# fy-vision/DiGA

Hardware: AMD Instinct MI355X
Metric: 768x768 19-class crops/sec (DiGA warm-up step) (higher is better)
Workload: dtype f32; 1 GPU; configs[1]: ResNet-101 DeepLabV2 DiGA warm-up (student + EMA teacher, KL distill), synthetic GTA5-shape 768x768, batch 8 per GPU; global_batch=8, parallelism=dp1

## Files before the change

### diga_amd/_lib.py

```python
import collections
import ctypes as C
import os

import torch

from diga_amd import config

_HERE = os.path.dirname(os.path.abspath(__file__))
LIB_PATH = os.environ.get("DIGA_LIB") or os.path.join(_HERE, "libdiga_hip.so")

if not os.path.exists(LIB_PATH):
    raise ImportError(
        f"{LIB_PATH} is missing: the DiGA hot path has no CPU fallback. "
        "Build the HIP extension first: python -m diga_amd.build")

lib = C.CDLL(LIB_PATH)

P = C.c_void_p
I64 = C.c_int64
F32 = C.c_float
INT = C.c_int
SZ = C.c_size_t

SIGNATURES = {
    "diga_version": (INT, []),
    "diga_last_error_string": (C.c_char_p, []),
    "diga_loss_workspace_bytes": (SZ, [I64]),
    "diga_ce2d_fwd_bwd": (INT, [P, P, P, P, P, SZ, I64, I64, I64, I64, F32, P]),
    "diga_ohem_ce_workspace_bytes": (SZ, [I64, I64, I64]),
    "diga_ohem_ce_fwd_bwd": (INT, [P, P, P, P, P, SZ, I64, I64, I64, I64, I64, F32, I64, F32, P]),
    "diga_distill_fwd_bwd": (INT, [P, P, P, P, P, SZ, I64, I64, I64, I64, F32, F32, P]),
    "diga_scale_inplace": (INT, [P, P, I64, P]),
    "diga_upsample_loss_workspace_bytes": (SZ, [I64, I64, I64, I64]),
    "diga_upsample_ce_distill_fwd_bwd": (INT, [P, P, P, P, P, P, SZ, I64, I64, I64, I64, I64, I64, F32, F32, F32, P]),
    "diga_upsample_ce_fwd_bwd": (INT, [P, P, P, P, P, SZ, I64, I64, I64, I64, I64, I64, F32, P]),
    "diga_upsample_bilinear_ac": (INT, [P, P, I64, I64, I64, I64, I64, P]),
    "diga_ema_update_flat": (INT, [P, P, I64, F32, F32, P]),
    "diga_ema_update_multi": (INT, [P, P, P, P, P, I64, I64, F32, F32, P]),
    "diga_sgd_momentum_multi": (INT, [P, P, P, P, P, P, P, P, I64, I64, F32, F32, INT, F32, P, P]),
    "diga_nonfinite_flag_f32": (INT, [P, I64, P, P]),
    "diga_label_hist256": (INT, [P, P, I64, I64, P]),
    "diga_classmix_paste": (INT, [P, P, P, P, P, P, P, I64, I64, I64, P]),
    "diga_centroid_softmax_weights": (INT, [P, P, P, P, I64, I64, I64, I64, P]),
    "diga_upsample_argmax_consensus": (INT, [P, P, P, P, I64, I64, I64, I64, I64, I64, P]),
    "diga_class_mean_workspace_bytes": (SZ, [I64, I64]),
    "diga_class_mean_vectors": (INT, [P, P, P, P, P, P, P, SZ, I64, I64, I64, I64, I64, I64, I64, P]),
    "diga_centroid_ema_apply": (INT, [P, P, P, P, I64, I64, I64, I64, F32, INT, INT, P]),
    "diga_confusion_matrix": (INT, [P, P, P, I64, I64, P]),
    "diga_two_scale_confusion": (INT, [P, I64, I64, P, I64, I64, P, P, P, I64, I64, I64, I64, P]),
    "diga_conv2d_nhwc_f32": (INT, [P, P, P, P] + [I64] * 17 + [P, INT, P]),
    "diga_conv2d_stats_floats": (SZ, [I64, I64, I64, I64]),
    "diga_conv2d_stats_chunk_rows": (INT, [I64] * 13 + [INT]),
    "diga_conv2d_epi_chunk_rows": (INT, [I64] * 13 + [INT]),
    "diga_split_bf16": (INT, [P, P, P, I64, P]),
    "diga_conv2d_nhwc_bf16x3": (INT, [P, P, P, P, P] + [I64] * 17 + [P, INT, P]),
    "diga_make_twin": (INT, [P, I64, P, I64, I64, P]),
    "diga_split_bf16_image_bytes": (SZ, [I64, I64, I64]),
    "diga_split_bf16_image": (INT, [P, P, I64, I64, I64, P]),
    "diga_conv2d_nhwc_twin": (INT, [P, P, P, P] + [I64] * 16 + [P, INT, P]),
    "diga_conv2d_nhwc_f32_opts": (INT, [P, P, P, P] + [I64] * 17 + [P, INT, P]),
    "diga_conv2d_nhwc_bf16x3_opts": (INT, [P, P, P, P, P] + [I64] * 17 + [P, INT, P]),
    "diga_conv2d_nhwc_twin_opts": (INT, [P, P, P, P] + [I64] * 16 + [P, INT, P]),
    "diga_conv2d_wgrad_workspace_bytes": (SZ, [I64] * 7),
    "diga_conv2d_wgrad_nhwc_f32": (INT, [P, P, P, P, SZ] + [I64] * 17 + [INT, P]),
    "diga_conv2d_wgrad_twin_workspace_bytes": (SZ, [I64] * 7),
    "diga_conv2d_wgrad_twin": (INT, [P, P, P, P, SZ] + [I64] * 15 + [P]),
    "diga_weight_transpose": (INT, [P, P, I64, I64, I64, P]),
    "diga_make_triplet": (INT, [P, I64, P, I64, I64, P]),
    "diga_split_bf16x6_image_bytes": (SZ, [I64, I64, I64]),
    "diga_split_bf16x6_image": (INT, [P, P, I64, I64, I64, P]),
    "diga_conv2d_nhwc_bf16x6": (INT, [P, P, P, P] + [I64] * 16 + [P, INT, P]),
    "diga_conv2d_nhwc_bf16x6_epi": (INT, [P, P, P] + [I64] * 16 + [P, INT, P]),
    "diga_conv2d_wgrad_bf16x6_workspace_bytes": (SZ, [I64] * 7),
    "diga_conv2d_wgrad_bf16x6": (INT, [P, P, P, P, SZ] + [I64] * 15 + [P]),
    "diga_im2col_nchw": (INT, [P, P] + [I64] * 11 + [P]),
    "diga_norm_workspace_bytes": (SZ, [I64, I64, I64]),
    "diga_bn_fwd": (INT, [P, I64, P, I64, P, I64, P, P, P, P, P, P, P, I64, I64, INT, INT, INT, P, F32, F32, P, SZ, P]),
    "diga_bn_fwd_partials": (INT, [P, I64, P, I64, P, I64, P, P, P, P, P, P, P, I64, I64, INT, INT, P, F32, F32, P, I64, P, SZ, P]),
    "diga_bn_fwd_records": (INT, [P, I64, P, I64, P, I64, P, P, P, P, P, P, P, I64, I64, INT, INT, P, F32, F32, P, P, I64, P, SZ, P]),
    "diga_bn_bwd": (INT, [P, I64, P, I64, P, I64, P, P, P, P, P, I64, P, I64, I64, I64, INT, INT, P, SZ, P]),
    "diga_bn_bwd_affine": (INT, [P, I64, P, I64, P, I64, P, P, P, P, P, I64, P, P, I64, I64, INT, P, SZ, P]),
    "diga_pyramid_sum_fwd": (INT, [P, I64, I64, P, P, I64, I64, P, I64, I64, P, I64, I64, I64, I64, P]),
    "diga_pyramid_sum_bwd": (INT, [P, I64, I64, P, I64, I64, I64, I64, P]),
    "diga_pyramid_sum_fwd3": (INT, [P, I64, I64, P, P, P, P, P, I64, I64, P]),
    "diga_pyramid_sum_bwd3": (INT, [P, I64, I64, P, P, P, I64, I64, P]),
    "diga_bn_bwd_partials": (INT, [P, I64, P, I64, P, P, P, P, I64, I64, I64, INT, P, I64, P, SZ, P]),
    "diga_conv2d_nhwc_f32_epi": (INT, [P, P, P] + [I64] * 17 + [P, INT, P]),
    "diga_conv2d_winograd_workspace_bytes": (SZ, [I64] * 7),
    "diga_conv2d_winograd_tile_table_bytes": (SZ, [I64] * 5),
    "diga_conv2d_winograd_tile_table": (INT, [P] + [I64] * 5 + [P]),
    "diga_conv2d_winograd_stats_records": (SZ, [I64] * 6),
    "diga_conv2d_winograd_stats_floats": (SZ, [I64] * 6),
    "diga_conv2d_winograd_f32": (INT, [P, P, P, P, P, SZ] + [I64] * 9 + [INT, P, P, INT, P]),
    "diga_conv2d_winograd_f32_opts": (INT, [P, P, P, P, P, SZ] + [I64] * 9 + [P, P, INT, P]),
    "diga_conv2d_winograd_f32_epi": (INT, [P, P, P, P, SZ] + [I64] * 9 + [INT, P, P, INT, P]),
    "diga_conv2d_wgrad_winograd_workspace_bytes": (SZ, [I64] * 7 + [INT]),
    "diga_conv2d_wgrad_winograd_f32": (INT, [P, P, P, P, P, SZ] + [I64] * 9 + [P, P]),
    "diga_conv2d_winograd_v_floats": (SZ, [I64] * 6),
    "diga_conv2d_winograd_f32_keep": (INT, [P, P, P, P, P, P, SZ] + [I64] * 9 + [P, P, INT, P]),
    "diga_conv2d_nhwc_bf16x3_epi": (INT, [P, P, P, P] + [I64] * 17 + [P, INT, P]),
    "diga_conv2d_nhwc_twin_epi": (INT, [P, P, P] + [I64] * 16 + [P, INT, P]),
    "diga_gn_fwd": (INT, [P, I64, P, I64, P, P, P, P, P, I64, I64, I64, I64, INT, F32, P, SZ, P]),
    "diga_gn_bwd": (INT, [P, I64, P, I64, P, I64, P, P, P, P, P, I64, P, P, I64, I64, I64, I64, P, SZ, P]),
    "diga_avgpool_nhwc": (INT, [P, I64, P, I64, I64, I64, P, SZ, P]),
    "diga_colsum_nhwc": (INT, [P, I64, P, I64, I64, P, SZ, P]),
    "diga_small_linear_fwd": (INT, [P, P, P, P, I64, I64, I64, INT, P]),
    "diga_small_linear_bwd": (INT, [P, P, P, P, P, P, P, P, I64, I64, I64, INT, P]),
    "diga_channel_affine": (INT, [P, I64, P, I64, P, P, I64, I64, I64, P]),
    "diga_channel_dot": (INT, [P, I64, P, I64, P, I64, I64, I64, P, SZ, P]),
    "diga_maxpool3x3s2_fwd": (INT, [P, P, P, I64, I64, I64, I64, I64, I64, P]),
    "diga_maxpool3x3s2_bwd": (INT, [P, P, P, I64, I64, I64, I64, I64, I64, P]),
    "diga_color_aug_view": (INT, [P, P, P, P, I64, I64, I64, F32, P, P, P]),
    "diga_mit_gemm_nt": (INT, [P, I64, P, I64, P, P, I64, INT, P, I64, P, I64, INT, F32, I64, I64, I64, P]),
    "diga_mit_gemm_tn_workspace_bytes": (SZ, [I64, I64, I64]),
    "diga_mit_gemm_tn": (INT, [P, I64, P, I64, P, P, F32, INT, P, SZ, I64, I64, I64, P]),
    "diga_mit_colsum_workspace_bytes": (SZ, [I64, I64]),
    "diga_mit_colsum": (INT, [P, I64, P, F32, INT, P, SZ, I64, I64, P]),
    "diga_mit_cast_transpose": (INT, [P, P, P, I64, I64, P]),
    "diga_mit_weight_prep_multi": (INT, [P, P, I64, I64, P]),
    "diga_mit_cast_scale": (INT, [P, P, I64, F32, P]),
    "diga_mit_row_scale": (INT, [P, P, P, I64, I64, I64, P]),
    "diga_mit_layernorm_fwd": (INT, [P, I64, P, P, P, P, I64, P, P, I64, I64, F32, P]),
    "diga_mit_layernorm_bwd_workspace_bytes": (SZ, [I64, I64]),
    "diga_mit_layernorm_bwd": (INT, [P, INT, I64, F32, P, I64, P, P, P, P, I64, P, P, I64, P, P, F32, INT, P, SZ, I64, I64, P]),
    "diga_mit_dwconv_gelu_fwd": (INT, [P, P, P, P, P, I64, I64, I64, I64, P]),
    "diga_mit_dwconv_bwd_workspace_bytes": (SZ, [I64, I64, I64]),
    "diga_mit_dwconv_gelu_bwd": (INT, [P, P, P, P, P, P, P, P, F32, INT, P, SZ, I64, I64, I64, I64, P]),
    "diga_mit_im2col": (INT, [P, INT, P] + [I64] * 11 + [P]),
    "diga_mit_col2im": (INT, [P, P, INT, F32] + [I64] * 11 + [P]),
    "diga_mit_attention_fwd": (INT, [P, I64, P, I64, P, I64, P, I64, I64, I64, I64, F32, P]),
    "diga_mit_attention_bwd_workspace_bytes": (SZ, [I64, I64, I64, I64]),
    "diga_mit_attention_bwd": (INT, [P, I64, P, I64, P, P, I64, P, P, P, P, SZ, I64, I64, I64, I64, F32, P]),
    "diga_prof_enable": (INT, [INT]),
    "diga_prof_reset": (INT, []),
    "diga_prof_query": (INT, [INT, P, P]),
    "diga_prof_query_work": (INT, [INT, P]),
}

class ConvOptions(C.Structure):
    _fields_ = [("reflect_pad", INT), ("upsample_shift", INT), ("activation", INT)]


class MitWeightPrep(C.Structure):
    _fields_ = [("src", P), ("out_a", P), ("out_b", P), ("Co", INT), ("Ci", INT), ("RS", INT), ("Kp", INT), ("mode", INT),
                ("tiles_k", INT)]


class BwdEpilogue(C.Structure):
    _fields_ = [("addend", P), ("addend_ld", I64), ("mask_y", P), ("mask_ld", I64), ("x", P), ("x_ld", I64),
                ("relu_ab", P), ("mean", P), ("invstd", P), ("partials", P), ("mask_bits", P), ("mask_bits_ld", I64)]


PROF_TAGS = ["ce2d", "distill", "upsample_loss", "ema", "sgd", "classmix_hist", "classmix_paste",
             "centroid_weights", "consensus", "class_means", "centroid_apply", "conv_fwd", "conv_bwd_data",
             "conv_bwd_weight", "norm", "elementwise", "mit_gemm", "mit_wgrad", "mit_attn_fwd", "mit_attn_bwd", "mit_norm",
             "mit_dwconv", "mit_misc"]


def prof_query(tag):
    n, ms = C.c_int64(0), C.c_double(0.0)
    call("diga_prof_query", PROF_TAGS.index(tag), C.byref(n), C.byref(ms))
    return n.value, ms.value

def prof_work(tag):
    w = C.c_double(0.0)
    call("diga_prof_query_work", PROF_TAGS.index(tag), C.byref(w))
    return w.value


for _name, (_res, _args) in SIGNATURES.items():
    _fn = getattr(lib, _name)
    _fn.restype = _res
    _fn.argtypes = _args


CONV_MATH_F32, CONV_MATH_BF16X3, CONV_MATH_BF16X6 = 0, 1, 2


def set_conv_math(mode, exact=None):
    mode = {"f32": 0, "bf16x3": 1, "bf16x6": 2}.get(mode, mode)
    if mode not in (CONV_MATH_F32, CONV_MATH_BF16X3, CONV_MATH_BF16X6):
        raise ValueError(f"conv math must be 0 / 'f32', 1 / 'bf16x3' or 2 / 'bf16x6', not {mode!r}")
    if exact is not None:
        if exact and mode != CONV_MATH_F32:
            raise ValueError("exact=True belongs to the fp32 arithmetic")
        config.active().winograd_max_tile = 2 if exact else config.active().winograd_default_max_tile
    config.active().conv_math = int(mode)


def get_conv_math():
    return config.active().conv_math


def last_error():
    return lib.diga_last_error_string().decode("utf-8", "replace")


def call(name, *args):
    rc = getattr(lib, name)(*args)
    if rc != 0:
        raise RuntimeError(f"{name} failed (code {rc}): {last_error()}")


def stream():
    return C.c_void_p(torch.cuda.current_stream().cuda_stream)


def ptr(t):
    return C.c_void_p(0) if t is None else C.c_void_p(t.data_ptr())


def require_gpu(*tensors):
    for t in tensors:
        if t is not None and not t.is_cuda:
            raise RuntimeError(
                "diga_amd ops run on the GPU only (HIP kernels, no CPU fallback); got a "
                f"{t.device} tensor")


def contiguous(t, dtype=None):
    if t is None:
        return None
    if dtype is not None and t.dtype != dtype:
        t = t.to(dtype)
    return t if t.is_contiguous() else t.contiguous()


_workspaces = {}

_consumed_flags = set()

# ... 81 lines not shown
```

### diga_amd/config.py

```python
import contextlib
import dataclasses
import os
from dataclasses import dataclass


def _flag(name, default):
    v = os.environ.get(name)
    if v is None:
        return default
    return v not in ("0", "", "false", "False")


@dataclass
class StepConfig:
    teacher_stream: bool = True
    teacher_offset: str = "layer1"
    wgrad_stream: bool = True
    wgrad_hold: int = 4
    wgrad_hold_batch: int = 4
    c4_overlap: int = 2
    c4_overlap_gloo: bool = False
    step_graph: bool = False
    graph_fork_teacher: bool = True
    graph_fork_wgrad: bool = True
    centroid_exchange: str = "allgather"
    conv_math: int = 0
    winograd: bool = True
    winograd_ratio: float = 0.62
    winograd_default_max_tile: int = 6
    winograd_max_tile: int = 6
    winograd_keep_v: bool = True
    winograd_stats: bool = True
    keep_v_max_gb: float = 8.0
    keep_v_min_device_gb: float = 160.0
    conv_twin: str = "3"
    twin_only: bool = True
    twin_conv3: str = "1"
    relu_bits: bool = True
    fuse_bwd: bool = True
    junction_chain: bool = True
    ddp_bucket_mb: int = 25
    ddp_grad_views: bool = True
    ddp_overlap: bool = True
    ddp_single_rank: bool = False
    mit_loss_scale: float = 1024.0

    @classmethod
    def from_env(cls):
        e = os.environ.get
        c = cls()
        c.teacher_stream = _flag("DIGA_TEACHER_STREAM", c.teacher_stream)
        c.teacher_offset = e("DIGA_TEACHER_OFFSET", c.teacher_offset)
        c.wgrad_stream = _flag("DIGA_WGRAD_STREAM", c.wgrad_stream)
        c.wgrad_hold = int(e("DIGA_WGRAD_HOLD", c.wgrad_hold))
        c.wgrad_hold_batch = int(e("DIGA_WGRAD_HOLD_BATCH", c.wgrad_hold_batch))
        c.c4_overlap = int(e("DIGA_C4_OVERLAP", c.c4_overlap))
        c.c4_overlap_gloo = _flag("DIGA_C4_OVERLAP_GLOO", c.c4_overlap_gloo)
        c.step_graph = _flag("DIGA_STEP_GRAPH", c.step_graph)
        c.graph_fork_teacher = _flag("DIGA_GRAPH_FORK_TEACHER", c.graph_fork_teacher)
        c.graph_fork_wgrad = _flag("DIGA_GRAPH_FORK_WGRAD", c.graph_fork_wgrad)
        c.centroid_exchange = e("DIGA_CENTROID_EXCHANGE", c.centroid_exchange)
        c.conv_math = {"bf16x3": 1, "1": 1, "bf16x6": 2, "2": 2}.get(e("DIGA_CONV_MATH", ""), 0)
        c.winograd = _flag("DIGA_CONV_WINOGRAD", c.winograd)
        c.winograd_ratio = float(e("DIGA_CONV_WINOGRAD_RATIO", c.winograd_ratio))
        c.winograd_default_max_tile = c.winograd_max_tile = int(e("DIGA_CONV_WINOGRAD_TILE", c.winograd_default_max_tile))
        c.winograd_keep_v = _flag("DIGA_WINOGRAD_KEEP_V", c.winograd_keep_v)
        c.winograd_stats = _flag("DIGA_WINOGRAD_STATS", c.winograd_stats)
        c.keep_v_max_gb = float(e("DIGA_WINOGRAD_KEEP_V_MAX_GB", c.keep_v_max_gb))
        c.keep_v_min_device_gb = float(e("DIGA_WINOGRAD_KEEP_V_MIN_DEVICE_GB", c.keep_v_min_device_gb))
        c.conv_twin = e("DIGA_CONV_TWIN", c.conv_twin)
        c.twin_only = _flag("DIGA_TWIN_ONLY", c.twin_only)
        c.twin_conv3 = e("DIGA_TWIN_CONV3", c.twin_conv3)
        c.relu_bits = _flag("DIGA_RELU_BITS", c.relu_bits)
        c.fuse_bwd = _flag("DIGA_FUSE_BWD", c.fuse_bwd)
        c.junction_chain = _flag("DIGA_JUNCTION_CHAIN", c.junction_chain)
        c.ddp_bucket_mb = int(e("DIGA_DDP_BUCKET_MB", c.ddp_bucket_mb))
        c.ddp_grad_views = _flag("DIGA_DDP_GRAD_VIEWS", c.ddp_grad_views)
        c.ddp_overlap = _flag("DIGA_DDP_OVERLAP", c.ddp_overlap)
        c.ddp_single_rank = _flag("DIGA_DDP_SINGLE_RANK", c.ddp_single_rank)
        c.mit_loss_scale = float(e("DIGA_MIT_LOSS_SCALE", c.mit_loss_scale))
        c.validate()
        return c

    def validate(self):
        if self.centroid_exchange not in ("allgather", "allreduce"):
            raise ValueError(f"centroid_exchange must be 'allgather' or 'allreduce', not {self.centroid_exchange!r}")
        if self.c4_overlap not in (0, 1, 2):
            raise ValueError(f"c4_overlap must be 0, 1 or 2, not {self.c4_overlap!r}")
        if self.wgrad_hold < 0:
            raise ValueError(f"wgrad_hold must be >= 0, not {self.wgrad_hold!r}")
        if self.conv_math not in (0, 1, 2):
            raise ValueError(f"conv_math must be 0 (fp32), 1 (split bf16) or 2 (bf16x6), not {self.conv_math!r}")
        if self.winograd_max_tile not in (2, 4, 6):
            raise ValueError(f"winograd_max_tile must be 2, 4 or 6, not {self.winograd_max_tile!r}")
        return self

    def replace(self, **fields):
        return dataclasses.replace(self, **fields).validate()

    def serial_streams(self):
        return self.replace(teacher_stream=False, wgrad_stream=False, c4_overlap=0)


DEFAULTS = StepConfig.from_env()
_stack = [DEFAULTS]


def active():
    return _stack[-1]


@contextlib.contextmanager
def use(cfg):
    _stack.append(cfg)
    try:
        yield cfg
    finally:
        _stack.pop()


@contextlib.contextmanager
def override(**fields):
    with use(active().replace(**fields)) as cfg:
        yield cfg
```

### diga_amd/csrc/conv.hip

```cpp
#include <stdlib.h>
#include <string.h>

#include <algorithm>
#include <atomic>

#include "common.h"

namespace diga {

using f32x16 = __attribute__((ext_vector_type(16))) float;
using f32x4nt = __attribute__((ext_vector_type(4))) float;

__device__ __forceinline__ void store4_stream(float* p, float x, float y, float z, float w) {
#if defined(DIGA_PROBE_NOSTORE)
    if (x == 1.2345e38f) *p = y + z + w;
#elif defined(DIGA_PROBE_PLAINSTORE)
    *reinterpret_cast<float4*>(p) = make_float4(x, y, z, w);
#else
    __builtin_nontemporal_store((f32x4nt){x, y, z, w}, reinterpret_cast<f32x4nt*>(p));
#endif
}

constexpr int kBK = 32;

// ... 2029 lines not shown
            wait_next(ahead);
            nx = nx == 2 ? 0 : nx + 1;
        }
        return;
    }

    const int wm = wv >> 1, wn = wv & 1;
    f32x16 acc[2][2];
#pragma unroll
    for (int i = 0; i < 2; ++i)
#pragma unroll
        for (int j = 0; j < 2; ++j)
#pragma unroll
            for (int e = 0; e < 16; ++e) acc[i][j][e] = 0.f;
    const int li = lane & 31, lh = lane >> 5;
    int offa[2], offb[2];
#pragma unroll
    for (int i = 0; i < 2; ++i) {
        offa[i] = lh * A_ROW + (((wm * 64 + i * 32 + li) * 4) ^ (lh << 7));
        offb[i] = A_BYTES + lh * B_ROW + (((wn * 64 + i * 32 + li) * 4) ^ (lh << 7));
    }

    __builtin_amdgcn_s_barrier();
    int cur = 0;
    for (int ks = 0; ks < ksteps; ++ks) {
        const unsigned char* St = smem_b + cur * STAGE;
        float av[2][2], bv[2][2];
        auto frag = [&](int kk, int set) {
#pragma unroll
            for (int i = 0; i < 2; ++i) av[set][i] = *reinterpret_cast<const float*>(St + offa[i] + kk * A_ROW);
#pragma unroll
            for (int j = 0; j < 2; ++j) bv[set][j] = *reinterpret_cast<const float*>(St + offb[j] + kk * B_ROW);
        };
        frag(0, 0);
#pragma unroll
        for (int kk = 0; kk < kBK; kk += 2) {
            const int set = (kk >> 1) & 1;
            if (kk + 2 < kBK) frag(kk + 2, set ^ 1);
            __builtin_amdgcn_sched_group_barrier(0x100, 4, 0);
#pragma unroll
            for (int i = 0; i < 2; ++i)
#pragma unroll
                for (int j = 0; j < 2; ++j)
                    acc[i][j] = __builtin_amdgcn_mfma_f32_32x32x2f32(av[set][i], bv[set][j], acc[i][j], 0, 0, 0);
            __builtin_amdgcn_sched_group_barrier(0x008, 4, 0);
        }
        asm volatile("s_waitcnt lgkmcnt(0)" ::: "memory");
        __builtin_amdgcn_s_barrier();
        cur = cur == 2 ? 0 : cur + 1;
    }

    float* out = a.slab + (int64_t)split * a.Cout * RS * a.Cin;
#pragma unroll
    for (int j = 0; j < 2; ++j) {
        const int c = c0 + wn * 64 + j * 32 + li;
#pragma unroll
        for (int i = 0; i < 2; ++i) {
#pragma unroll
            for (int e = 0; e < 16; ++e) {
                const int k = k0 + wm * 64 + i * 32 + (e & 3) + 8 * (e >> 2) + 4 * lh;
                out[((int64_t)k * RS + tap) * a.Cin + c] = acc[i][j][e];
            }
        }
    }
}

__global__ __launch_bounds__(256) void slab_reduce_kernel(const float* __restrict__ slab, float* __restrict__ dw,
                                                          int64_t n4, int splits) {
    const int64_t i = (int64_t)blockIdx.x * 256 + threadIdx.x;
    if (i >= n4) return;
    float4 s = reinterpret_cast<const float4*>(slab)[i];
    for (int k = 1; k < splits; ++k) {
        const float4 v = reinterpret_cast<const float4*>(slab)[(int64_t)k * n4 + i];
        s.x += v.x;
        s.y += v.y;
        s.z += v.z;
        s.w += v.w;
    }
    reinterpret_cast<float4*>(dw)[i] = s;
}

__global__ __launch_bounds__(256) void weight_transpose_kernel(const float* __restrict__ w, float* __restrict__ wt,
                                                               int K, int RS, int C) {
    __shared__ float tile[32][33];
    const int tap = blockIdx.z;
    const int k0 = blockIdx.y * 32, c0 = blockIdx.x * 32;
    const int tx = threadIdx.x & 31, ty = threadIdx.x >> 5;
#pragma unroll
    for (int i = 0; i < 4; ++i) {
        const int k = k0 + ty + 8 * i, c = c0 + tx;
        tile[ty + 8 * i][tx] = (k < K && c < C) ? w[((int64_t)k * RS + tap) * C + c] : 0.f;
    }
    __syncthreads();
#pragma unroll
    for (int i = 0; i < 4; ++i) {
        const int c = c0 + ty + 8 * i, k = k0 + tx;
        if (c < C && k < K) wt[((int64_t)c * RS + tap) * K + k] = tile[tx][ty + 8 * i];
    }
}

static int check_conv_common(const char* who, int64_t Cin, int64_t in_ld, int64_t out_ld, int64_t Cout,
                             const void* in, const void* w, const void* out) {
    DIGA_REQUIRE(Cin > 0 && Cin % 32 == 0, DIGA_EINVAL, "%s: Cin=%lld must be a multiple of 32", who, (long long)Cin);
    DIGA_REQUIRE(in_ld >= Cin && in_ld % 4 == 0 && out_ld >= Cout, DIGA_EINVAL, "%s: bad leading dimensions", who);
    DIGA_REQUIRE(aligned16(in) && aligned16(w), DIGA_EALIGN, "%s: pointers must be 16-byte aligned", who);
    (void)out;
    return DIGA_OK;
}

static void set_options(ConvArgs& a, const diga_conv_options_t* o) {
    a.pad_reflect = o ? o->reflect_pad : 0;
    a.up_shift = o ? o->upsample_shift : 0;
    a.act = o ? o->activation : 0;
}

static int check_options(const diga_conv_options_t* o, const char* who) {
    if (o == nullptr) return DIGA_OK;
    DIGA_REQUIRE(o->reflect_pad >= 0 && o->reflect_pad <= 1 && o->upsample_shift >= 0 && o->upsample_shift <= 2 && o->activation >= 0 &&
                     o->activation <= 1, DIGA_EINVAL, "%s: bad options (reflect_pad 0/1, upsample_shift 0..2, activation 0/1)", who);
    return DIGA_OK;
}

static int set_bwd_epilogue(ConvArgs& a, const diga_bwd_epilogue_t* e, const char* who) {
    a.e_add = a.e_masky = a.e_x = a.e_relu_ab = a.e_mean = a.e_invstd = nullptr;
    a.e_partials = nullptr;
    a.e_maskbits = nullptr;
    a.e_add_ld = a.e_masky_ld = a.e_x_ld = a.e_maskbits_ld = 0;
    if (e == nullptr) return DIGA_OK;
    DIGA_REQUIRE(e->addend || e->mask_y || e->mask_bits || e->x, DIGA_EINVAL, "%s: empty epilogue descriptor", who);
    DIGA_REQUIRE(a.Cout % 4 == 0 && a.out_ld % 4 == 0 && aligned16(a.out) && a.bias == nullptr && a.stats == nullptr, DIGA_EINVAL,
                 "%s: a backward epilogue needs Cout %% 4 == 0, out_ld %% 4 == 0, a 16-byte aligned output, no bias, no forward statistics", who);
    DIGA_REQUIRE(!e->addend || (aligned16(e->addend) && e->addend_ld >= a.Cout && e->addend_ld % 4 == 0), DIGA_EINVAL, "%s: bad addend", who);
    DIGA_REQUIRE(!e->mask_y || (aligned16(e->mask_y) && e->mask_ld >= a.Cout && e->mask_ld % 4 == 0), DIGA_EINVAL, "%s: bad mask_y", who);
    DIGA_REQUIRE(!e->x || (aligned16(e->x) && e->x_ld >= a.Cout && e->x_ld % 4 == 0), DIGA_EINVAL, "%s: bad x", who);
    DIGA_REQUIRE((e->mask_y != nullptr) + (e->relu_ab != nullptr) + (e->mask_bits != nullptr) <= 1, DIGA_EINVAL,
                 "%s: give one of mask_y, mask_bits, relu_ab", who);
    DIGA_REQUIRE(!e->mask_bits || e->mask_bits_ld * 8 >= a.Cout, DIGA_EINVAL, "%s: bad mask_bits", who);
    DIGA_REQUIRE(!e->relu_ab || (e->x && aligned16(e->relu_ab)), DIGA_EINVAL, "%s: relu_ab needs x", who);
    DIGA_REQUIRE(!e->partials || (e->x && e->mean && e->invstd && aligned16(e->mean) && aligned16(e->invstd)), DIGA_EINVAL,
                 "%s: partials need x, mean and invstd", who);
    a.e_add = e->addend; a.e_add_ld = (int)e->addend_ld;
    a.e_masky = e->mask_y; a.e_masky_ld = (int)e->mask_ld;
    a.e_maskbits = e->mask_bits; a.e_maskbits_ld = (int)e->mask_bits_ld;
    a.e_x = e->x; a.e_x_ld = (int)e->x_ld;
    a.e_relu_ab = e->relu_ab; a.e_mean = e->mean; a.e_invstd = e->invstd; a.e_partials = e->partials;
    return DIGA_OK;
}

struct GemmArgs {
    const float* A;
    const float* W;
    float* out;
    int M, K, Cout, tiles_m, tiles_n, wb_tiles;
    int64_t wb_stride;
    int64_t a_ld, out_ld;
    const float* bias;
    float* stats;
};

__global__ __launch_bounds__(768, 3) void gemm_f32_persistent_kernel(GemmArgs g) {
    constexpr int A_BYTES = 256 * 128, B_BYTES = 128 * 128, STAGE = A_BYTES + B_BYTES;
    extern __shared__ __align__(16) unsigned char smem_b[];
    const int lane = threadIdx.x & 63, wv = threadIdx.x >> 6;
    const bool loader = wv >= 8;
    const int total = g.tiles_m * g.tiles_n;
    const int xcd = blockIdx.x & 7, slot = blockIdx.x >> 3, nslots = gridDim.x >> 3;
    const int q = total >> 3, r = total & 7;
    const int start = xcd < r ? xcd * (q + 1) : r * (q + 1) + (xcd - r) * q, len = q + (xcd < r ? 1 : 0);
    const int nmine = slot < len ? (len - slot + nslots - 1) / nslots : 0;
    if (nmine == 0) return;
    const int ksteps = g.K / 32;
    const int total_steps = nmine * ksteps;
    const int64_t rowb = g.a_ld * 4, wrowb = (int64_t)g.K * 4;

    if (loader) {
        const int lw = wv - 8;
        const int lrow = lane >> 3;
        const unsigned char* pa[8];
        const unsigned char* pb[4];
        int l_it = 0, l_cc = 0, issued = 0;
        auto set_tile = [&](int it) {
            const int t = start + slot + nslots * it;
            const int tile_n = t % g.tiles_n, tile_m = t / g.tiles_n;
            const int row0 = tile_m * 256 + lw * 64 + lrow;
            const unsigned char* ab = reinterpret_cast<const unsigned char*>(g.A) + (int64_t)row0 * rowb;
            const unsigned char* wb = reinterpret_cast<const unsigned char*>(g.W + (g.wb_tiles > 0 ? (int64_t)(tile_m / g.wb_tiles) * g.wb_stride : 0)) +
                                      (int64_t)(tile_n * 128 + lw * 32 + lrow) * wrowb;
#pragma unroll
            for (int j = 0; j < 8; ++j)
                pa[j] = row0 + 8 * j < g.M ? ab + (int64_t)(8 * j) * rowb + (((lane & 7) ^ (((8 * j + lrow) >> 1) & 7)) << 4) : nullptr;
#pragma unroll
            for (int c = 0; c < 4; ++c) pb[c] = wb + (int64_t)(8 * c) * wrowb + (((lane & 7) ^ (((8 * c + lrow) >> 1) & 7)) << 4);
        };
        auto issue = [&](int buf) {
            unsigned char* stage = smem_b + buf * STAGE;
#pragma unroll
            for (int j = 0; j < 8; ++j) {
                const unsigned char* src = pa[j] != nullptr ? pa[j] + l_cc * 128 : g_zero16;
                __builtin_amdgcn_global_load_lds((const __attribute__((address_space(1))) void*)src,
                                                 (__attribute__((address_space(3))) void*)(stage + (lw * 64 + 8 * j) * 128), 16, 0, 0);
            }
#pragma unroll
            for (int c = 0; c < 4; ++c)
                __builtin_amdgcn_global_load_lds((const __attribute__((address_space(1))) void*)(pb[c] + l_cc * 128),
                                                 (__attribute__((address_space(3))) void*)(stage + A_BYTES + (lw * 32 + 8 * c) * 128), 16, 0, 0);
            ++issued;
            if (++l_cc == ksteps) {
                l_cc = 0;
                if (++l_it < nmine) set_tile(l_it);
            }
        };
        auto wait_next = [&](bool newest_in_flight) {
            if (newest_in_flight) asm volatile("s_waitcnt vmcnt(12)" ::: "memory");
            else asm volatile("s_waitcnt vmcnt(0)" ::: "memory");
            __builtin_amdgcn_s_barrier();
        };
        set_tile(0);
        issue(0);
        if (total_steps > 1) issue(1);
        wait_next(total_steps > 1);
        int nx = 2;
        for (int gs = 0; gs < total_steps; ++gs) {
            const bool ahead = gs + 2 < total_steps;
            if (ahead) issue(nx);
            wait_next(ahead);
            nx = nx == 2 ? 0 : nx + 1;
        }
        return;
    }

    const int wm = wv >> 1, wn = wv & 1;
    f32x16 acc[2][2];
#pragma unroll
    for (int i = 0; i < 2; ++i)
#pragma unroll
        for (int j = 0; j < 2; ++j)
#pragma unroll
            for (int e = 0; e < 16; ++e) acc[i][j][e] = 0.f;
    const int li = lane & 31, lh = lane >> 5;
    const int fsw = (li >> 1) & 7;
    const int F = li * 128 + ((lh ^ fsw) << 4);
    const int FA = F + wm * 64 * 128, FB = F + A_BYTES + wn * 64 * 128;
#define DIGA_FOFF(t) ((t) << 5)

    __builtin_amdgcn_s_barrier();
    int cur = 0, it = 0, ks_in_tile = 0;
    for (int gs = 0; gs < total_steps; ++gs) {
        const int sa = cur * STAGE + FA, sb = cur * STAGE + FB;
#define As_AT(t) (smem_b + (sa ^ DIGA_FOFF(t)))
#define Bs_AT(t) (smem_b + (sb ^ DIGA_FOFF(t)))
        float4 fa[2][2], fb[2][2];
        fa[0][0] = *reinterpret_cast<const float4*>(As_AT(0));
        fa[0][1] = *reinterpret_cast<const float4*>(As_AT(0) + 32 * 128);
        fb[0][0] = *reinterpret_cast<const float4*>(Bs_AT(0));
        fb[0][1] = *reinterpret_cast<const float4*>(Bs_AT(0) + 32 * 128);
        __builtin_amdgcn_sched_group_barrier(0x100, 4, 0);
#pragma unroll
        for (int t = 0; t < 4; ++t) {
            const int p = t & 1;
            if (t + 1 < 4) {
                fa[p ^ 1][0] = *reinterpret_cast<const float4*>(As_AT(t + 1));
                fa[p ^ 1][1] = *reinterpret_cast<const float4*>(As_AT(t + 1) + 32 * 128);
                fb[p ^ 1][0] = *reinterpret_cast<const float4*>(Bs_AT(t + 1));
                fb[p ^ 1][1] = *reinterpret_cast<const float4*>(Bs_AT(t + 1) + 32 * 128);
                __builtin_amdgcn_sched_group_barrier(0x100, 4, 0);
            }
#pragma unroll
            for (int e = 0; e < 4; ++e)
#pragma unroll
                for (int i = 0; i < 2; ++i)
#pragma unroll
                    for (int j = 0; j < 2; ++j) {
                        const float av = e == 0 ? fa[p][i].x : e == 1 ? fa[p][i].y : e == 2 ? fa[p][i].z : fa[p][i].w;
                        const float bv = e == 0 ? fb[p][j].x : e == 1 ? fb[p][j].y : e == 2 ? fb[p][j].z : fb[p][j].w;
                        acc[i][j] = __builtin_amdgcn_mfma_f32_32x32x2f32(av, bv, acc[i][j], 0, 0, 0);
                    }
            __builtin_amdgcn_sched_group_barrier(0x008, 16, 0);
        }
        asm volatile("s_waitcnt lgkmcnt(0)" ::: "memory");
        __builtin_amdgcn_s_barrier();
        cur = cur == 2 ? 0 : cur + 1;
        if (++ks_in_tile == ksteps) {
            const int t = start + slot + nslots * it;
            const int tile_n = t % g.tiles_n, tile_m = t / g.tiles_n;
            const int row_w = tile_m * 256 + wm * 64;
            const int col_w = tile_n * 128 + wn * 64 + li;
            const unsigned ob = (unsigned)(row_w + 4 * lh) * (unsigned)g.out_ld + (unsigned)col_w;
#define DIGA_O_AT(r, j) (g.out + (size_t)(ob + (unsigned)(r) * (unsigned)g.out_ld + (unsigned)((j) * 32)))
            const int rows_left = g.M - (row_w + 4 * lh);
#pragma unroll
            for (int j = 0; j < 2; ++j) {
                const float bv = g.bias != nullptr ? g.bias[col_w + j * 32] : 0.f;
                const float sh = __shfl(acc[0][j][0] + bv, li, 64);
                float sd = 0.f, sd2 = 0.f;
                if (row_w + 64 <= g.M) {
#pragma unroll
                    for (int i = 0; i < 2; ++i)
#pragma unroll
                        for (int e = 0; e < 16; ++e) {
                            const int r = i * 32 + (e & 3) + 8 * (e >> 2);
                            const float v = acc[i][j][e] + bv;
                            __builtin_nontemporal_store(v, DIGA_O_AT(r, j));
                            const float d = v - sh;
                            sd += d;
                            sd2 += d * d;
                            acc[i][j][e] = 0.f;
                        }
                } else {
#pragma unroll
                    for (int i = 0; i < 2; ++i)
#pragma unroll
                        for (int e = 0; e < 16; ++e) {
                            const int r = i * 32 + (e & 3) + 8 * (e >> 2);
                            const float v = acc[i][j][e] + bv;
                            if (r < rows_left) {
                                __builtin_nontemporal_store(v, DIGA_O_AT(r, j));
                                const float d = v - sh;
                                sd += d;
                                sd2 += d * d;
                            }
                            acc[i][j][e] = 0.f;
                        }
                }
                if (g.stats != nullptr && row_w < g.M) {
                    sd += __shfl_xor(sd, 32, 64);
                    sd2 += __shfl_xor(sd2, 32, 64);
                    if (lh == 0) {
                        float* sp = g.stats + (int64_t)(row_w >> 6) * 3 * g.Cout + col_w + j * 32;
                        sp[0] = sd;
                        sp[g.Cout] = sd2;
                        sp[2 * g.Cout] = sh;
                    }
                }
            }
            ks_in_tile = 0;
            ++it;
        }
    }
}

int gemm_batched_f32_dma(const float* A, int64_t rows_per_batch, int batches, int64_t K, const float* W, int64_t Cout,
                         float* out, hipStream_t st) {
    DIGA_REQUIRE(rows_per_batch > 0 && rows_per_batch % 256 == 0 && K % 32 == 0 && Cout > 0 && Cout % 4 == 0, DIGA_EINVAL,
                 "gemm_batched_f32_dma: rows %% 256, K %% 32, Cout %% 4 required");
    const int64_t M = rows_per_batch * batches;
    DIGA_REQUIRE(M / 256 < 32768 && M < (1ll << 31), DIGA_EINVAL, "gemm_batched_f32_dma: too many rows");
    ConvArgs a;
    a.in = A; a.wgt = W; a.wgt_hi = nullptr; a.wgt_lo = nullptr; a.wgt_img = nullptr; a.bias = nullptr; a.out = out; a.stats = nullptr;
    a.N = 1; a.Hi = (int)(M / 256); a.Wi = 256; a.Cin = (int)K; a.in_ld = (int)K;
    a.Ho = a.Hi; a.Wo = 256; a.Cout = (int)Cout; a.out_ld = (int)Cout;
    a.R = 1; a.S = 1; a.sy = 1; a.sx = 1; a.oy0 = 0; a.ox0 = 0; a.ody = 1; a.odx = 1;
    a.M = (int)M; a.tiles_m = (int)ceil_div(M, 128); a.tiles_n = (int)ceil_div(Cout, 128); a.all_inside = 1;
    a.pad_reflect = 0; a.up_shift = 0; a.act = 0;
    a.e_add = a.e_masky = a.e_x = a.e_relu_ab = a.e_mean = a.e_invstd = nullptr;
    a.e_partials = nullptr; a.e_maskbits = nullptr;
    a.e_add_ld = a.e_masky_ld = a.e_x_ld = a.e_maskbits_ld = 0;
    a.wb_tiles = (int)(rows_per_batch / 256);
    a.wb_stride = Cout * K;
    const unsigned grid = (unsigned)((M / 256) * a.tiles_n);
    const size_t sh = 3 * (256 + 128) * 128;
    if (Cout % 128 == 0 && grid >= 512 && M * Cout < (1ll << 32)) {
        GemmArgs g;
        g.A = A; g.W = W; g.out = out; g.M = (int)M; g.K = (int)K; g.Cout = (int)Cout;
        g.tiles_m = (int)(M / 256); g.tiles_n = a.tiles_n; g.wb_tiles = a.wb_tiles; g.wb_stride = a.wb_stride;
        g.a_ld = K; g.out_ld = Cout; g.bias = nullptr; g.stats = nullptr;
        (void)hipFuncSetAttribute((const void*)gemm_f32_persistent_kernel, hipFuncAttributeMaxDynamicSharedMemorySize, (int)sh);
        hipLaunchKernelGGL(gemm_f32_persistent_kernel, dim3(256), dim3(768), sh, st, g);
        return DIGA_OK;
    }
    (void)hipFuncSetAttribute((const void*)conv_fwd_dma_kernel<false>, hipFuncAttributeMaxDynamicSharedMemorySize, (int)sh);
    hipLaunchKernelGGL(conv_fwd_dma_kernel<false>, dim3(grid), dim3(768), sh, st, a);
    return DIGA_OK;
}

bool pointwise_persistent_ok(int64_t M, int64_t Hi, int64_t Wi, int64_t Cin, int64_t Ho, int64_t Wo, int64_t Cout, int64_t R,
                             int64_t S, int64_t sy, int64_t sx, int64_t oy0, int64_t ox0) {
    return R == 1 && S == 1 && sy == 1 && sx == 1 && oy0 == 0 && ox0 == 0 && Hi == Ho && Wi == Wo && Cin % 32 == 0 &&
           Cout % 128 == 0 && ceil_div(M, 256) * (Cout / 128) >= 512;
}

}

using namespace diga;

static int conv2d_f32_impl(const float* in, const float* wgt, const float* bias, float* out, int64_t N,
                                    int64_t Hi, int64_t Wi, int64_t Cin, int64_t in_ld, int64_t Ho, int64_t Wo,
                                    int64_t Cout, int64_t out_ld, int64_t R, int64_t S, int64_t stride_y,
                                    int64_t stride_x, int64_t off_y0, int64_t off_x0, int64_t off_dy, int64_t off_dx,
                                    float* stats_partial, int prof_tag, void* stream, const diga_bwd_epilogue_t* epi,
                                    const diga_conv_options_t* opts = nullptr) {
    DIGA_REQUIRE(in && wgt && out, DIGA_EINVAL, "conv2d: null pointer");
    DIGA_REQUIRE(N > 0 && Hi > 0 && Wi > 0 && Ho > 0 && Wo > 0 && Cout > 0 && R > 0 && S > 0, DIGA_EINVAL, "conv2d: bad shape");
    int rc = check_conv_common("conv2d", Cin, in_ld, out_ld, Cout, in, wgt, out);
    if (rc) return rc;
    DIGA_REQUIRE(N * Hi * Wi < (1ll << 31) && N * Ho * Wo < (1ll << 31), DIGA_EINVAL, "conv2d: too many pixels for 32-bit tile indices");
    ConvArgs a;
    a.in = in; a.wgt = wgt; a.wgt_hi = nullptr; a.wgt_lo = nullptr; a.bias = bias; a.out = out; a.stats = stats_partial;
    a.N = (int)N; a.Hi = (int)Hi; a.Wi = (int)Wi; a.Cin = (int)Cin; a.in_ld = (int)in_ld;
    a.Ho = (int)Ho; a.Wo = (int)Wo; a.Cout = (int)Cout; a.out_ld = (int)out_ld;
    a.R = (int)R; a.S = (int)S; a.sy = (int)stride_y; a.sx = (int)stride_x;
    a.oy0 = (int)off_y0; a.ox0 = (int)off_x0; a.ody = (int)off_dy; a.odx = (int)off_dx;
    a.M = (int)(N * Ho * Wo);
    a.all_inside = 0;
    a.tiles_m = (int)ceil_div(a.M, 128);
    rc = check_options(opts, "conv2d");
    if (rc) return rc;
    set_options(a, opts);
    rc = set_bwd_epilogue(a, epi, "conv2d");
    if (rc) return rc;
    hipStream_t st = (hipStream_t)stream;
    ProfScope prof(prof_tag == DIGA_PROF_CONV_BWD_DATA ? DIGA_PROF_CONV_BWD_DATA : DIGA_PROF_CONV_FWD, st,
                   2.0 * (double)a.M * (double)Cout * (double)(R * S) * (double)Cin);
#define DIGA_LAUNCH_K(KERNEL_, THREADS_, SH_)                                                                          \
    do {                                                                                                               \
        (void)hipFuncSetAttribute((const void*)KERNEL_, hipFuncAttributeMaxDynamicSharedMemorySize, (int)(SH_));        \
        hipLaunchKernelGGL(KERNEL_, dim3((unsigned)(a.tiles_m * a.tiles_n)), dim3(THREADS_), (SH_), st, a);             \
    } while (0)
#define DIGA_FWD_LAUNCH(TN_, BK_)                                                                                      \
    do {                                                                                                               \
        const size_t sh = (size_t)(2 * 128 * (BK_ + 4) + 2 * 64 * TN_ * (BK_ + 4)) * sizeof(float);                     \
        if (epi != nullptr) DIGA_LAUNCH_K((conv_fwd_kernel<TN_, 32, true>), 256, sh);                                   \
        else DIGA_LAUNCH_K((conv_fwd_kernel<TN_, BK_, false>), 256, sh);                                                \
    } while (0)
    if (pointwise_persistent_ok(N * Ho * Wo, Hi, Wi, Cin, Ho, Wo, Cout, R, S, stride_y, stride_x, off_y0, off_x0) &&
        epi == nullptr && !(opts && (opts->reflect_pad || opts->upsample_shift || opts->activation))) {
        DIGA_REQUIRE((int64_t)a.M * out_ld < (1ll << 32), DIGA_EINVAL, "conv2d_nhwc_f32: output beyond 2^32 elements (the pointwise kernel "
                     "addresses it with 32-bit element offsets)");
        GemmArgs g;
        g.A = in; g.W = wgt; g.out = out; g.M = a.M; g.K = (int)Cin; g.Cout = (int)Cout;
        g.tiles_m = (int)ceil_div(a.M, 256); g.tiles_n = (int)(Cout / 128); g.wb_tiles = 0; g.wb_stride = 0;
        g.a_ld = in_ld; g.out_ld = out_ld; g.bias = bias; g.stats = stats_partial;
        const size_t shp = 3 * (256 + 128) * 128;
        (void)hipFuncSetAttribute((const void*)gemm_f32_persistent_kernel, hipFuncAttributeMaxDynamicSharedMemorySize, (int)shp);
        hipLaunchKernelGGL(gemm_f32_persistent_kernel, dim3(256), dim3(768), shp, st, g);
        return launch_status("diga_conv2d_nhwc_f32");
    }
    if (a.M >= 256 && Cout >= 256 && R * S * Cin >= 256) {
        a.tiles_n = (int)ceil_div(Cout, 128);
        const unsigned grid = (unsigned)(ceil_div(a.M, 256) * a.tiles_n);
        const size_t sh = 3 * (256 + 128) * 128;
        if (epi != nullptr) {
            (void)hipFuncSetAttribute((const void*)conv_fwd_dma_kernel<true>, hipFuncAttributeMaxDynamicSharedMemorySize, (int)sh);
            hipLaunchKernelGGL(conv_fwd_dma_kernel<true>, dim3(grid), dim3(768), sh, st, a);
        } else {
            (void)hipFuncSetAttribute((const void*)conv_fwd_dma_kernel<false>, hipFuncAttributeMaxDynamicSharedMemorySize, (int)sh);
            hipLaunchKernelGGL(conv_fwd_dma_kernel<false>, dim3(grid), dim3(768), sh, st, a);
        }
    } else if (Cout > 64) {
        a.tiles_n = (int)ceil_div(Cout, 128);
        DIGA_FWD_LAUNCH(2, 32);
    } else {
        a.tiles_n = 1;
        DIGA_FWD_LAUNCH(1, 32);
    }
#undef DIGA_FWD_LAUNCH
    return launch_status("diga_conv2d_nhwc_f32");
}


extern "C" int diga_conv2d_nhwc_f32(const float* in, const float* wgt, const float* bias, float* out, int64_t N,
                                    int64_t Hi, int64_t Wi, int64_t Cin, int64_t in_ld, int64_t Ho, int64_t Wo,
                                    int64_t Cout, int64_t out_ld, int64_t R, int64_t S, int64_t stride_y,
                                    int64_t stride_x, int64_t off_y0, int64_t off_x0, int64_t off_dy, int64_t off_dx,
                                    float* stats_partial, int prof_tag, void* stream) {
    return conv2d_f32_impl(in, wgt, bias, out, N, Hi, Wi, Cin, in_ld, Ho, Wo, Cout, out_ld, R, S, stride_y, stride_x, off_y0, off_x0,
                           off_dy, off_dx, stats_partial, prof_tag, stream, nullptr);
}

extern "C" int diga_conv2d_nhwc_f32_epi(const float* in, const float* wgt, float* out, int64_t N, int64_t Hi, int64_t Wi,
                                        int64_t Cin, int64_t in_ld, int64_t Ho, int64_t Wo, int64_t Cout, int64_t out_ld,
                                        int64_t R, int64_t S, int64_t stride_y, int64_t stride_x, int64_t off_y0,
                                        int64_t off_x0, int64_t off_dy, int64_t off_dx, const diga_bwd_epilogue_t* epi,
                                        int prof_tag, void* stream) {
    DIGA_REQUIRE(epi != nullptr, DIGA_EINVAL, "conv2d_epi: null epilogue descriptor");
    return conv2d_f32_impl(in, wgt, nullptr, out, N, Hi, Wi, Cin, in_ld, Ho, Wo, Cout, out_ld, R, S, stride_y, stride_x, off_y0,
                           off_x0, off_dy, off_dx, nullptr, prof_tag, stream, epi);
}

extern "C" int diga_split_bf16(const float* x, uint16_t* hi, uint16_t* lo, int64_t n, void* stream) {
    DIGA_REQUIRE(x && hi && lo && n > 0 && n % 4 == 0, DIGA_EINVAL, "split_bf16: n must be a positive multiple of 4");
    DIGA_REQUIRE(aligned16(x) && ((uintptr_t)hi & 7u) == 0 && ((uintptr_t)lo & 7u) == 0, DIGA_EALIGN, "split_bf16: alignment");
    int64_t blocks = ceil_div(n / 4, 256);
    if (blocks > 4096) blocks = 4096;
    hipLaunchKernelGGL(split_bf16_kernel, dim3((unsigned)blocks), dim3(256), 0, (hipStream_t)stream, x, hi, lo, n / 4);
    return launch_status("diga_split_bf16");
}

static int conv2d_bf16x3_impl(const float* in, const uint16_t* wgt_hi, const uint16_t* wgt_lo, const float* bias,
                                       float* out, int64_t N, int64_t Hi, int64_t Wi, int64_t Cin, int64_t in_ld,
                                       int64_t Ho, int64_t Wo, int64_t Cout, int64_t out_ld, int64_t R, int64_t S,
                                       int64_t stride_y, int64_t stride_x, int64_t off_y0, int64_t off_x0, int64_t off_dy,
                                       int64_t off_dx, float* stats_partial, int prof_tag, void* stream,
                                       const diga_bwd_epilogue_t* epi, const diga_conv_options_t* opts = nullptr) {
    DIGA_REQUIRE(in && wgt_hi && wgt_lo && out, DIGA_EINVAL, "conv2d_bf16x3: null pointer");
    DIGA_REQUIRE(N > 0 && Hi > 0 && Wi > 0 && Ho > 0 && Wo > 0 && Cout > 0 && R > 0 && S > 0, DIGA_EINVAL, "conv2d_bf16x3: bad shape");
    int rc = check_conv_common("conv2d_bf16x3", Cin, in_ld, out_ld, Cout, in, in, out);
    if (rc) return rc;
    DIGA_REQUIRE(((uintptr_t)wgt_hi & 7u) == 0 && ((uintptr_t)wgt_lo & 7u) == 0, DIGA_EALIGN, "conv2d_bf16x3: weight alignment");
    DIGA_REQUIRE(N * Hi * Wi < (1ll << 31) && N * Ho * Wo < (1ll << 31), DIGA_EINVAL, "conv2d_bf16x3: too many pixels");
    ConvArgs a;
    a.in = in; a.wgt = nullptr; a.wgt_hi = wgt_hi; a.wgt_lo = wgt_lo; a.wgt_img = nullptr; a.bias = bias; a.out = out; a.stats = stats_partial;
    a.N = (int)N; a.Hi = (int)Hi; a.Wi = (int)Wi; a.Cin = (int)Cin; a.in_ld = (int)in_ld;
    a.Ho = (int)Ho; a.Wo = (int)Wo; a.Cout = (int)Cout; a.out_ld = (int)out_ld;
    a.R = (int)R; a.S = (int)S; a.sy = (int)stride_y; a.sx = (int)stride_x;
    a.oy0 = (int)off_y0; a.ox0 = (int)off_x0; a.ody = (int)off_dy; a.odx = (int)off_dx;
    a.M = (int)(N * Ho * Wo);
    a.tiles_m = (int)ceil_div(a.M, 128);
    {
        const int64_t y_lo = off_y0 + std::min<int64_t>(0, (R - 1) * off_dy), y_hi = (Ho - 1) * stride_y + off_y0 + std::max<int64_t>(0, (R - 1) * off_dy);
        const int64_t x_lo = off_x0 + std::min<int64_t>(0, (S - 1) * off_dx), x_hi = (Wo - 1) * stride_x + off_x0 + std::max<int64_t>(0, (S - 1) * off_dx);
        a.all_inside = y_lo >= 0 && y_hi < Hi && x_lo >= 0 && x_hi < Wi;
    }
    rc = check_options(opts, "conv2d_bf16x3");
    if (rc) return rc;
    set_options(a, opts);
    if (a.pad_reflect || a.up_shift) a.all_inside = 0;
    rc = set_bwd_epilogue(a, epi, "conv2d_bf16x3");
    if (rc) return rc;
    hipStream_t st = (hipStream_t)stream;
    ProfScope prof(prof_tag == DIGA_PROF_CONV_BWD_DATA ? DIGA_PROF_CONV_BWD_DATA : DIGA_PROF_CONV_FWD, st,
                   2.0 * (double)a.M * (double)Cout * (double)(R * S) * (double)Cin);
    const int tn = Cout > 64 ? 2 : 1;
    a.tiles_n = (int)ceil_div(Cout, 64 * tn);
    const bool fits32 = N * Hi * Wi * in_ld < (1ll << 31) && Cout * R * S * Cin < (1ll << 31);
    DIGA_REQUIRE(fits32 || !(a.pad_reflect || a.up_shift), DIGA_EINVAL,
                 "conv2d_bf16x3: reflect padding / fused upsampling are implemented by the 256-row kernel only");
    if (fits32) {
        a.tiles_m = (int)ceil_div(a.M, 256);
        const size_t loop = (size_t)2 * 256 * 64 + (size_t)2 * 64 * tn * 64, stage = (size_t)128 * (64 * tn + 4) * sizeof(float);
        const size_t sh = loop > stage ? loop : stage;
#ifdef DIGA_PROBE_STAMP
        if (tn == 2 && a.stats != nullptr) {
            (void)hipFuncSetAttribute((const void*)conv_fwd_x3w_kernel<2, true>, hipFuncAttributeMaxDynamicSharedMemorySize, (int)sh);
            hipLaunchKernelGGL((conv_fwd_x3w_kernel<2, true>), dim3((unsigned)(a.tiles_m * a.tiles_n)), dim3(256), sh, st, a);
        } else
#endif
        if (tn == 2) {
            if (epi != nullptr) DIGA_LAUNCH_K((conv_fwd_x3w_kernel<2, false, true>), 256, sh);
            else DIGA_LAUNCH_K((conv_fwd_x3w_kernel<2, false, false>), 256, sh);
        } else {
            if (epi != nullptr) DIGA_LAUNCH_K((conv_fwd_x3w_kernel<1, false, true>), 256, sh);
            else DIGA_LAUNCH_K((conv_fwd_x3w_kernel<1, false, false>), 256, sh);
        }
    } else if (tn == 2) {
        const size_t sh = (size_t)2 * (2 * 128 * kRowB + 2 * 128 * kRowB);
        if (epi != nullptr) DIGA_LAUNCH_K((conv_fwd_x3p_kernel<2, true>), 256, sh);
        else DIGA_LAUNCH_K((conv_fwd_x3p_kernel<2, false>), 256, sh);
    } else {
        const size_t sh = (size_t)2 * (2 * 128 * kRowB + 2 * 64 * kRowB);
        if (epi != nullptr) DIGA_LAUNCH_K((conv_fwd_x3p_kernel<1, true>), 256, sh);
        else DIGA_LAUNCH_K((conv_fwd_x3p_kernel<1, false>), 256, sh);
    }
    return launch_status("diga_conv2d_nhwc_bf16x3");
}

extern "C" int diga_conv2d_nhwc_bf16x3(const float* in, const uint16_t* wgt_hi, const uint16_t* wgt_lo, const float* bias,
                                       float* out, int64_t N, int64_t Hi, int64_t Wi, int64_t Cin, int64_t in_ld,
                                       int64_t Ho, int64_t Wo, int64_t Cout, int64_t out_ld, int64_t R, int64_t S,
                                       int64_t stride_y, int64_t stride_x, int64_t off_y0, int64_t off_x0, int64_t off_dy,
                                       int64_t off_dx, float* stats_partial, int prof_tag, void* stream) {
    return conv2d_bf16x3_impl(in, wgt_hi, wgt_lo, bias, out, N, Hi, Wi, Cin, in_ld, Ho, Wo, Cout, out_ld, R, S, stride_y, stride_x,
                              off_y0, off_x0, off_dy, off_dx, stats_partial, prof_tag, stream, nullptr);
}

extern "C" int diga_conv2d_nhwc_bf16x3_epi(const float* in, const uint16_t* wgt_hi, const uint16_t* wgt_lo, float* out, int64_t N,
                                           int64_t Hi, int64_t Wi, int64_t Cin, int64_t in_ld, int64_t Ho, int64_t Wo,
                                           int64_t Cout, int64_t out_ld, int64_t R, int64_t S, int64_t stride_y,
                                           int64_t stride_x, int64_t off_y0, int64_t off_x0, int64_t off_dy, int64_t off_dx,
                                           const diga_bwd_epilogue_t* epi, int prof_tag, void* stream) {
    DIGA_REQUIRE(epi != nullptr, DIGA_EINVAL, "conv2d_bf16x3_epi: null epilogue descriptor");
    return conv2d_bf16x3_impl(in, wgt_hi, wgt_lo, nullptr, out, N, Hi, Wi, Cin, in_ld, Ho, Wo, Cout, out_ld, R, S, stride_y, stride_x,
                              off_y0, off_x0, off_dy, off_dx, nullptr, prof_tag, stream, epi);
}

static int64_t image_bn(int64_t K) { return K > 64 ? 128 : 64; }

extern "C" int diga_make_twin(const float* x, int64_t ld, void* twin, int64_t M, int64_t C, void* stream) {
    DIGA_REQUIRE(x && twin && M > 0 && C > 0 && C % 8 == 0 && ld >= C && ld % 4 == 0, DIGA_EINVAL, "make_twin: C must be a multiple of 8");
    DIGA_REQUIRE(aligned16(x) && aligned16(twin), DIGA_EALIGN, "make_twin: pointers must be 16-byte aligned");
    int64_t blocks = ceil_div(M * (C / 8), 256);
    if (blocks > 16384) blocks = 16384;
    ProfScope prof(DIGA_PROF_ELEMENTWISE, (hipStream_t)stream, (double)M * C * 8.0);
    hipLaunchKernelGGL(make_twin_kernel, dim3((unsigned)blocks), dim3(256), 0, (hipStream_t)stream, x, ld, (unsigned char*)twin, M,
                       (int)(C / 8));
    return launch_status("diga_make_twin");
}

// ... 446 lines not shown
```

### diga_amd/csrc/norm.hip

```cpp
#include <initializer_list>

#include "common.h"

namespace diga {

constexpr int kNormThreads = 256;

using nf4 = __attribute__((ext_vector_type(4))) float;
using nu2 = __attribute__((ext_vector_type(2))) unsigned int;
__device__ __forceinline__ void st4s(float* p, float4 v) { __builtin_nontemporal_store((nf4){v.x, v.y, v.z, v.w}, reinterpret_cast<nf4*>(p)); }
__device__ __forceinline__ void st2s(unsigned char* p, uint2 v) { __builtin_nontemporal_store((nu2){v.x, v.y}, reinterpret_cast<nu2*>(p)); }
__device__ __forceinline__ float4 ld4s(const float* p) { const nf4 v = __builtin_nontemporal_load(reinterpret_cast<const nf4*>(p)); return make_float4(v.x, v.y, v.z, v.w); }

struct ColGeom {
    int64_t rows_per_seg;
    int nseg, C, chunk_rows, nchunk;
};

struct NoPrep {
    __device__ __forceinline__ void operator()(int) const {}
};

template <int NV, class F, class P = NoPrep>
__device__ __forceinline__ void chunk_walk(const ColGeom& g, int seg, int chunk, float* __restrict__ out, F&& f, P&& prep = NoPrep()) {
    __shared__ float red[kNormThreads][4];
    const int tq = g.C >> 2;
    const int64_t r0 = (int64_t)seg * g.rows_per_seg + (int64_t)chunk * g.chunk_rows;
    int64_t r1 = r0 + g.chunk_rows;
    const int64_t seg_end = (int64_t)(seg + 1) * g.rows_per_seg;
    if (r1 > seg_end) r1 = seg_end;
    if (tq >= kNormThreads) {
        for (int q = threadIdx.x; q < tq; q += kNormThreads) {
            float acc[NV][4];
#pragma unroll
            for (int v = 0; v < NV; ++v)
#pragma unroll
                for (int e = 0; e < 4; ++e) acc[v][e] = 0.f;
            prep(q * 4);
#pragma unroll 8
            for (int64_t r = r0; r < r1; ++r) f(r, r0, q * 4, acc);
#pragma unroll
            for (int v = 0; v < NV; ++v)
#pragma unroll
                for (int e = 0; e < 4; ++e) out[(int64_t)v * g.C + q * 4 + e] = acc[v][e];
        }
    } else {
        const int lanes = kNormThreads / tq;
        const int q = threadIdx.x % tq, rl = threadIdx.x / tq;
        float acc[NV][4];
#pragma unroll
        for (int v = 0; v < NV; ++v)
#pragma unroll
            for (int e = 0; e < 4; ++e) acc[v][e] = 0.f;
        if (rl < lanes) {
            prep(q * 4);
            int64_t r = r0 + rl;
            for (; r + 7 * (int64_t)lanes < r1; r += 8 * (int64_t)lanes) {
#pragma unroll
                for (int u = 0; u < 8; ++u) f(r + u * (int64_t)lanes, r0, q * 4, acc);
            }
            for (; r < r1; r += lanes) f(r, r0, q * 4, acc);
        }
#pragma unroll
        for (int v = 0; v < NV; ++v) {
            __syncthreads();
#pragma unroll
            for (int e = 0; e < 4; ++e) red[threadIdx.x][e] = acc[v][e];
            __syncthreads();
            if (threadIdx.x < tq) {
                float s[4] = {0.f, 0.f, 0.f, 0.f};
                for (int l = 0; l < lanes; ++l)
#pragma unroll
                    for (int e = 0; e < 4; ++e) s[e] += red[l * tq + threadIdx.x][e];
#pragma unroll
                for (int e = 0; e < 4; ++e) out[(int64_t)v * g.C + threadIdx.x * 4 + e] = s[e];
            }
        }
    }
}

__global__ __launch_bounds__(kNormThreads) void colstats_partial_kernel(const float* __restrict__ x, int64_t ld,
                                                                         ColGeom g, float* __restrict__ partial) {
    const int chunk = blockIdx.x, seg = blockIdx.y;
    float* out = partial + ((int64_t)seg * g.nchunk + chunk) * 3 * g.C;
    const int64_t r0 = (int64_t)seg * g.rows_per_seg + (int64_t)chunk * g.chunk_rows;
    float4 s = make_float4(0.f, 0.f, 0.f, 0.f);
    chunk_walk<2>(g, seg, chunk, out, [&](int64_t r, int64_t, int c, float (&acc)[2][4]) {
        const float4 v = *reinterpret_cast<const float4*>(x + r * ld + c);
        const float d0 = v.x - s.x, d1 = v.y - s.y, d2 = v.z - s.z, d3 = v.w - s.w;
        acc[0][0] += d0; acc[0][1] += d1; acc[0][2] += d2; acc[0][3] += d3;
        acc[1][0] += d0 * d0; acc[1][1] += d1 * d1; acc[1][2] += d2 * d2; acc[1][3] += d3 * d3;
    }, [&](int c) { s = *reinterpret_cast<const float4*>(x + r0 * ld + c); });
    for (int c = threadIdx.x; c < g.C; c += kNormThreads) out[2 * g.C + c] = x[r0 * ld + c];
}

__device__ __forceinline__ int64_t chunk_count(const ColGeom& g, int chunk) {
    const int64_t a = (int64_t)chunk * g.chunk_rows;
    int64_t b = a + g.chunk_rows;
    if (b > g.rows_per_seg) b = g.rows_per_seg;
    return b - a;
}

__device__ __forceinline__ void merge_channel(const float* __restrict__ partial, const ColGeom& g, int seg, int c,
                                              double& n, double& mean, double& m2) {
    n = 0.0; mean = 0.0; m2 = 0.0;
    for (int k = 0; k < g.nchunk; ++k) {
        const float* p = partial + ((int64_t)seg * g.nchunk + k) * 3 * g.C;
        const double nb = (double)chunk_count(g, k);
        const double sd = p[c], sd2 = p[g.C + c], sh = p[2 * g.C + c];
        const double mb = sh + sd / nb, m2b = sd2 - sd * sd / nb;
        const double tot = n + nb, delta = mb - mean;
        mean += delta * nb / tot;
        m2 += m2b + delta * delta * n * nb / tot;
        n = tot;
    }
}


__global__ void bn_eval_ab_kernel(const float* __restrict__ gamma, const float* __restrict__ beta,
                                  const float* __restrict__ running_mean, const float* __restrict__ running_var,
                                  float* __restrict__ save_mean, float* __restrict__ save_invstd, float* __restrict__ ab,
                                  int C, float eps) {
    const int c = blockIdx.x * blockDim.x + threadIdx.x;
    if (c >= C) return;
    const float invstd = 1.f / sqrtf(running_var[c] + eps);
    save_mean[c] = running_mean[c];
    save_invstd[c] = invstd;
    const float a = invstd * gamma[c];
    ab[c] = a;
    ab[C + c] = beta[c] - running_mean[c] * a;
}

__global__ void gn_finalize_kernel(const float* __restrict__ partial, ColGeom g, int G, const float* __restrict__ gamma,
                                   const float* __restrict__ beta, const float* __restrict__ chan_scale,
                                   float* __restrict__ save_mean, float* __restrict__ save_invstd, float* __restrict__ ab,
                                   float eps) {
    const int idx = blockIdx.x * blockDim.x + threadIdx.x;
    if (idx >= g.nseg * G) return;
    const int n_img = idx / G, grp = idx - n_img * G;
    const int cpg = g.C / G;
    double n = 0.0, mean = 0.0, m2 = 0.0;
    for (int j = 0; j < cpg; ++j) {
        double nb, mb, m2b;
        merge_channel(partial, g, n_img, grp * cpg + j, nb, mb, m2b);
        const double tot = n + nb, delta = mb - mean;
        mean += delta * nb / tot;
        m2 += m2b + delta * delta * n * nb / tot;
        n = tot;
    }
    const float var = (float)(m2 / n);
    const float invstd = 1.f / sqrtf(var + eps);
    const float mu = (float)mean;
    save_mean[idx] = mu;
    save_invstd[idx] = invstd;
    const int64_t NC = (int64_t)g.nseg * g.C;
    for (int j = 0; j < cpg; ++j) {
        const int c = grp * cpg + j;
        const float s = chan_scale ? chan_scale[(int64_t)n_img * g.C + c] : 1.f;
        const float a = invstd * gamma[c];
        ab[(int64_t)n_img * g.C + c] = a * s;
        ab[NC + (int64_t)n_img * g.C + c] = (beta[c] - mu * a) * s;
    }
}

__device__ __forceinline__ void norm_split4(const float4 v, uint2& hi, uint2& lo) {
    typedef __bf16 bf2 __attribute__((ext_vector_type(2)));
    typedef float f2 __attribute__((ext_vector_type(2)));
    hi.x = __builtin_bit_cast(uint32_t, __builtin_convertvector((f2){v.x, v.y}, bf2));
    hi.y = __builtin_bit_cast(uint32_t, __builtin_convertvector((f2){v.z, v.w}, bf2));
    const float h0 = __uint_as_float(hi.x << 16), h1 = __uint_as_float(hi.x & 0xffff0000u);
    const float h2 = __uint_as_float(hi.y << 16), h3 = __uint_as_float(hi.y & 0xffff0000u);
    lo.x = __builtin_bit_cast(uint32_t, __builtin_convertvector((f2){v.x - h0, v.y - h1}, bf2));
    lo.y = __builtin_bit_cast(uint32_t, __builtin_convertvector((f2){v.z - h2, v.w - h3}, bf2));
}

template <bool RES, bool RELU, bool BITS, bool TWIN, bool SEG>
__global__ __launch_bounds__(256) void affine_apply_kernel(const float* __restrict__ x, int64_t ld_x, float* __restrict__ y,
                                                           int64_t ld_y, const float* __restrict__ res, int64_t ld_r,
                                                           const float* __restrict__ a, const float* __restrict__ b,
                                                           int64_t ab_seg_stride, int64_t rows_per_seg, int64_t rows,
                                                           int C, unsigned char* __restrict__ relu_bits) {
    const int tq = C >> 2;
    const int tpr = tq < 256 ? tq : 256;
    const int rpb = 256 / tpr;
    const int q0 = threadIdx.x % tpr, rl = threadIdx.x / tpr;
    if (rl >= rpb) return;
    const int nrows = (int)rows, rps = (int)rows_per_seg;
    const int rstep = gridDim.x * rpb;
    for (int q = q0; q < tq; q += tpr) {
        const int c = q * 4;
        float4 av = *reinterpret_cast<const float4*>(a + c);
        float4 bv = b != nullptr ? *reinterpret_cast<const float4*>(b + c) : make_float4(0.f, 0.f, 0.f, 0.f);
        int cur_seg = 0;
        for (int r = blockIdx.x * rpb + rl; r < nrows; r += rstep) {
            if (SEG) {
                const int seg = r / rps;
                if (seg != cur_seg) {
                    cur_seg = seg;
                    av = *reinterpret_cast<const float4*>(a + (int64_t)seg * ab_seg_stride + c);
                    if (b != nullptr) bv = *reinterpret_cast<const float4*>(b + (int64_t)seg * ab_seg_stride + c);
                }
            }
            const float4 xv = ld4s(x + (int64_t)r * ld_x + c);
            float4 o;
            o.x = __builtin_fmaf(xv.x, av.x, bv.x); o.y = __builtin_fmaf(xv.y, av.y, bv.y);
            o.z = __builtin_fmaf(xv.z, av.z, bv.z); o.w = __builtin_fmaf(xv.w, av.w, bv.w);
            if (RES) {
                const float4 rv = ld4s(res + (int64_t)r * ld_r + c);
                o.x += rv.x; o.y += rv.y; o.z += rv.z; o.w += rv.w;
            }
            if (RELU) {
                if (BITS) {
                    unsigned v = ((o.x > 0.f ? 1u : 0u) | (o.y > 0.f ? 2u : 0u) | (o.z > 0.f ? 4u : 0u) | (o.w > 0.f ? 8u : 0u))
                                 << (4 * (threadIdx.x & 7));
                    v |= (unsigned)__builtin_amdgcn_update_dpp(0, (int)v, 0xB1, 0xf, 0xf, true);
                    v |= (unsigned)__builtin_amdgcn_update_dpp(0, (int)v, 0x4E, 0xf, 0xf, true);
                    v |= (unsigned)__builtin_amdgcn_update_dpp(0, (int)v, 0x141, 0xf, 0xf, true);
                    if ((threadIdx.x & 7) == 0)
                        *reinterpret_cast<unsigned*>(relu_bits + (int64_t)r * (C >> 3) + (c >> 3)) = v;
                }
                o.x = fmaxf(o.x, 0.f); o.y = fmaxf(o.y, 0.f); o.z = fmaxf(o.z, 0.f); o.w = fmaxf(o.w, 0.f);
            }
            if (TWIN) {
                uint2 hi, lo;
                norm_split4(o, hi, lo);
                unsigned char* tw = reinterpret_cast<unsigned char*>(y) + ((int64_t)r * (C >> 3) + (c >> 3)) * 32 + ((c >> 2) & 1) * 8;
                st2s(tw, hi);
                st2s(tw + 16, lo);
            } else {
                st4s(y + (int64_t)r * ld_y + c, o);
            }
        }
    }
}

template <bool RES, bool RELU, bool BITS, bool TWIN>
static void launch_affine_seg(dim3 grid, hipStream_t st, const float* x, int64_t ld_x, float* y, int64_t ld_y, const float* res, int64_t ld_r,
                              const float* a, const float* b, int64_t ab_seg_stride, int64_t rows_per_seg, int64_t rows, int C,
                              unsigned char* relu_bits) {
    if (ab_seg_stride != 0)
        hipLaunchKernelGGL((affine_apply_kernel<RES, RELU, BITS, TWIN, true>), grid, dim3(256), 0, st, x, ld_x, y, ld_y, res, ld_r, a, b, ab_seg_stride,
                           rows_per_seg, rows, C, relu_bits);
    else
        hipLaunchKernelGGL((affine_apply_kernel<RES, RELU, BITS, TWIN, false>), grid, dim3(256), 0, st, x, ld_x, y, ld_y, res, ld_r, a, b, ab_seg_stride,
                           rows_per_seg, rows, C, relu_bits);
}
static void launch_affine(dim3 grid, hipStream_t st, const float* x, int64_t ld_x, float* y, int64_t ld_y, const float* res, int64_t ld_r,
                          const float* a, const float* b, int64_t ab_seg_stride, int64_t rows_per_seg, int64_t rows, int C, int relu,
                          int twin_out, unsigned char* relu_bits = nullptr) {
#define DIGA_AFF(RES, RELU, BITS, TWIN) \
    launch_affine_seg<RES, RELU, BITS, TWIN>(grid, st, x, ld_x, y, ld_y, res, ld_r, a, b, ab_seg_stride, rows_per_seg, rows, C, relu_bits)
    const bool bits = relu && relu_bits != nullptr;
    if (res != nullptr) {
        if (relu) {
            if (bits) { if (twin_out) DIGA_AFF(true, true, true, true); else DIGA_AFF(true, true, true, false); }
            else { if (twin_out) DIGA_AFF(true, true, false, true); else DIGA_AFF(true, true, false, false); }
        } else { if (twin_out) DIGA_AFF(true, false, false, true); else DIGA_AFF(true, false, false, false); }
    } else {
        if (relu) {
            if (bits) { if (twin_out) DIGA_AFF(false, true, true, true); else DIGA_AFF(false, true, true, false); }
            else { if (twin_out) DIGA_AFF(false, true, false, true); else DIGA_AFF(false, true, false, false); }
        } else { if (twin_out) DIGA_AFF(false, false, false, true); else DIGA_AFF(false, false, false, false); }
    }
#undef DIGA_AFF
}

__global__ __launch_bounds__(kNormThreads) void bwd_partial_kernel(const float* __restrict__ dy, int64_t ld_dy,
                                                                    const float* __restrict__ x, int64_t ld_x,
                                                                    const float* __restrict__ y, int64_t ld_y,
                                                                    const float* __restrict__ mean,
                                                                    const float* __restrict__ invstd, int st_seg_stride,
                                                                    int cdiv, ColGeom g, float* __restrict__ partial,
                                                                    const float* __restrict__ relu_ab) {
    const int chunk = blockIdx.x, seg = blockIdx.y;
    float* out = partial + ((int64_t)seg * g.nchunk + chunk) * 2 * g.C;
    float mu[4] = {0.f, 0.f, 0.f, 0.f}, is[4] = {1.f, 1.f, 1.f, 1.f}, ra[4] = {0.f, 0.f, 0.f, 0.f}, rb[4] = {0.f, 0.f, 0.f, 0.f};
    chunk_walk<2>(g, seg, chunk, out, [&](int64_t r, int64_t, int c, float (&acc)[2][4]) {
        const float4 gv = *reinterpret_cast<const float4*>(dy + r * ld_dy + c);
        const float4 xv = *reinterpret_cast<const float4*>(x + r * ld_x + c);
        float gg[4] = {gv.x, gv.y, gv.z, gv.w};
        const float xx[4] = {xv.x, xv.y, xv.z, xv.w};
        if (y != nullptr) {
            const float4 yv = *reinterpret_cast<const float4*>(y + r * ld_y + c);
            const float yy[4] = {yv.x, yv.y, yv.z, yv.w};
#pragma unroll
            for (int e = 0; e < 4; ++e) gg[e] = yy[e] > 0.f ? gg[e] : 0.f;
        } else if (relu_ab != nullptr) {
#pragma unroll
            for (int e = 0; e < 4; ++e) gg[e] = __builtin_fmaf(xx[e], ra[e], rb[e]) > 0.f ? gg[e] : 0.f;
        }
#pragma unroll
        for (int e = 0; e < 4; ++e) {
            const float xh = (xx[e] - mu[e]) * is[e];
            acc[0][e] += gg[e];
            acc[1][e] += gg[e] * xh;
        }
    }, [&](int c) {
#pragma unroll
        for (int e = 0; e < 4; ++e) {
            const int si = seg * st_seg_stride + (c + e) / cdiv;
            mu[e] = mean != nullptr ? mean[si] : 0.f;
            is[e] = mean != nullptr ? invstd[si] : 1.f;
            ra[e] = relu_ab != nullptr ? relu_ab[c + e] : 0.f;
            rb[e] = relu_ab != nullptr ? relu_ab[g.C + c + e] : 0.f;
        }
    });
}


__global__ void gn_bwd_finalize_kernel(const float* __restrict__ partial, ColGeom g, int G, const float* __restrict__ gamma,
                                       const float* __restrict__ chan_scale, const float* __restrict__ invstd,
                                       float* __restrict__ kk, float* __restrict__ chan_sums ) {
    const int idx = blockIdx.x * blockDim.x + threadIdx.x;
    if (idx >= g.nseg * G) return;
    const int n_img = idx / G, grp = idx - n_img * G;
    const int cpg = g.C / G;
    const int64_t NC = (int64_t)g.nseg * g.C;
    double c1 = 0.0, c2 = 0.0;
    for (int j = 0; j < cpg; ++j) {
        const int c = grp * cpg + j;
        double s1 = 0.0, s2 = 0.0;
        for (int k = 0; k < g.nchunk; ++k) {
            const float* p = partial + ((int64_t)n_img * g.nchunk + k) * 2 * g.C;
            s1 += (double)p[c];
            s2 += (double)p[g.C + c];
        }
        const double sc = chan_scale ? (double)chan_scale[(int64_t)n_img * g.C + c] : 1.0;
        s1 *= sc;
        s2 *= sc;
        chan_sums[(int64_t)n_img * g.C + c] = (float)s1;
        chan_sums[NC + (int64_t)n_img * g.C + c] = (float)s2;
        c1 += (double)gamma[c] * s1;
        c2 += (double)gamma[c] * s2;
    }
    const double cnt = (double)g.rows_per_seg * cpg;
    const float is = invstd[idx];
    for (int j = 0; j < cpg; ++j) {
        const int c = grp * cpg + j;
        const float sc = chan_scale ? chan_scale[(int64_t)n_img * g.C + c] : 1.f;
        kk[(int64_t)n_img * g.C + c] = sc * gamma[c] * is;
        kk[NC + (int64_t)n_img * g.C + c] = (float)(is * (c1 / cnt));
        kk[2 * NC + (int64_t)n_img * g.C + c] = (float)(is * (c2 / cnt));
    }
}

__global__ void gn_param_grad_kernel(const float* __restrict__ chan_sums, int N, int C, float* __restrict__ dgamma,
                                     float* __restrict__ dbeta) {
    const int c = blockIdx.x * blockDim.x + threadIdx.x;
    if (c >= C) return;
    float b = 0.f, gm = 0.f;
    for (int n = 0; n < N; ++n) {
        b += chan_sums[(int64_t)n * C + c];
        gm += chan_sums[(int64_t)N * C + (int64_t)n * C + c];
    }
    dbeta[c] = b;
    dgamma[c] = gm;
}

template <int MASK, bool DRES, bool TWIN, bool SEG>
__global__ __launch_bounds__(256) void bwd_apply_kernel(const float* __restrict__ dy, int64_t ld_dy,
                                                        const float* __restrict__ x, int64_t ld_x,
                                                        const float* __restrict__ y, int64_t ld_y,
                                                        const float* __restrict__ mean, const float* __restrict__ invstd,
                                                        int st_seg_stride, int cdiv, const float* __restrict__ kk,
                                                        int64_t kk_seg_stride, int64_t kk_plane, float* __restrict__ dx,
                                                        int64_t ld_dx, float* __restrict__ dres, int64_t ld_dr,
                                                        int64_t rows_per_seg, int64_t rows, int C,
                                                        const float* __restrict__ relu_ab) {
    const int tq = C >> 2;
    const int tpr = tq < 256 ? tq : 256;
    const int rpb = 256 / tpr;
    const int q0 = threadIdx.x % tpr, rl = threadIdx.x / tpr;
    if (rl >= rpb) return;
    const int nrows = (int)rows, rps = (int)rows_per_seg;
    const int rstep = gridDim.x * rpb;
    for (int q = q0; q < tq; q += tpr) {
        const int c = q * 4;
        float k1a[4], k2a[4], k3a[4], mu[4], is[4];
        float ra[4] = {0.f, 0.f, 0.f, 0.f}, rb[4] = {0.f, 0.f, 0.f, 0.f};
        if (MASK == 2) {
#pragma unroll
            for (int e = 0; e < 4; ++e) {
                ra[e] = relu_ab[c + e];
                rb[e] = relu_ab[C + c + e];
            }
        }
        auto load_coeff = [&](int seg) {
            const float* kb = kk + (int64_t)seg * kk_seg_stride + c;
            const float4 k1 = *reinterpret_cast<const float4*>(kb);
            const float4 k2 = *reinterpret_cast<const float4*>(kb + kk_plane);
            const float4 k3 = *reinterpret_cast<const float4*>(kb + 2 * kk_plane);
            k1a[0] = k1.x; k1a[1] = k1.y; k1a[2] = k1.z; k1a[3] = k1.w;
            k2a[0] = k2.x; k2a[1] = k2.y; k2a[2] = k2.z; k2a[3] = k2.w;
            k3a[0] = k3.x; k3a[1] = k3.y; k3a[2] = k3.z; k3a[3] = k3.w;
#pragma unroll
            for (int e = 0; e < 4; ++e) {
                const int si = seg * st_seg_stride + (c + e) / cdiv;
                mu[e] = mean[si];
                is[e] = invstd[si];
            }
        };
        load_coeff(0);
        int cur_seg = 0;
        for (int r = blockIdx.x * rpb + rl; r < nrows; r += rstep) {
            if (SEG) {
                const int seg = r / rps;
                if (seg != cur_seg) {
                    cur_seg = seg;
                    load_coeff(seg);
                }
            }
            const float4 gv = ld4s(dy + (int64_t)r * ld_dy + c);
            const float4 xv = ld4s(x + (int64_t)r * ld_x + c);
            float gg[4] = {gv.x, gv.y, gv.z, gv.w};
            const float xx[4] = {xv.x, xv.y, xv.z, xv.w};
            if (MASK == 1) {
                const float4 yv = ld4s(y + (int64_t)r * ld_y + c);
// ... 397 lines not shown
            s1 += (double)p[c];
            s2 += (double)p[g.C + c];
        }
    for (int o = cpg; o < 64; o <<= 1) {
        s1 += __shfl_xor(s1, o, 64);
        s2 += __shfl_xor(s2, o, 64);
    }
    const double sc = chan_scale ? (double)chan_scale[(int64_t)n_img * g.C + c] : 1.0;
    s1 *= sc;
    s2 *= sc;
    const int64_t NC = (int64_t)g.nseg * g.C;
    if (lane < cpg) {
        chan_sums[(int64_t)n_img * g.C + c] = (float)s1;
        chan_sums[NC + (int64_t)n_img * g.C + c] = (float)s2;
    }
    double c1 = lane < cpg ? (double)gamma[c] * s1 : 0.0;
    double c2 = lane < cpg ? (double)gamma[c] * s2 : 0.0;
    c1 = wave_sum_f64(c1);
    c2 = wave_sum_f64(c2);
    const double cnt = (double)g.rows_per_seg * cpg;
    const float is = invstd[idx];
    if (lane < cpg) {
        kk[(int64_t)n_img * g.C + c] = (float)sc * gamma[c] * is;
        kk[NC + (int64_t)n_img * g.C + c] = (float)(is * (c1 / cnt));
        kk[2 * NC + (int64_t)n_img * g.C + c] = (float)(is * (c2 / cnt));
    }
}

static ColGeom make_geom(int64_t rows_per_seg, int64_t nseg, int64_t C) {
    ColGeom g;
    g.rows_per_seg = rows_per_seg;
    g.nseg = (int)nseg;
    g.C = (int)C;
    int64_t want = ceil_div(512, nseg);
    int64_t chunk = ceil_div(rows_per_seg, want);
    if (chunk < 64) chunk = 64;
    if (chunk > rows_per_seg) chunk = rows_per_seg;
    g.chunk_rows = (int)chunk;
    g.nchunk = (int)ceil_div(rows_per_seg, chunk);
    return g;
}

static unsigned ew_blocks(int64_t work) {
    int64_t b = ceil_div(work, 256);
    if (b > 8192) b = 8192;
    if (b < 1) b = 1;
    return (unsigned)b;
}

static int check_norm(const char* who, int64_t C, std::initializer_list<int64_t> lds, std::initializer_list<const void*> ptrs) {
    DIGA_REQUIRE(C > 0 && C % 4 == 0, DIGA_EINVAL, "%s: C=%lld must be a positive multiple of 4", who, (long long)C);
    for (int64_t ld : lds) DIGA_REQUIRE(ld >= C && ld % 4 == 0, DIGA_EINVAL, "%s: leading dimension %lld invalid", who, (long long)ld);
    for (const void* p : ptrs) DIGA_REQUIRE(p == nullptr || aligned16(p), DIGA_EALIGN, "%s: pointers must be 16-byte aligned", who);
    return DIGA_OK;
}

__device__ __forceinline__ float act_apply(float v, int act) { return act == 1 ? fmaxf(v, 0.f) : act == 2 ? 1.f / (1.f + expf(-v)) : v; }

__global__ __launch_bounds__(256) void small_linear_fwd_kernel(const float* __restrict__ x, const float* __restrict__ w,
                                                               const float* __restrict__ b, float* __restrict__ y, int N, int K, int O,
                                                               int act) {
    const int wave = (int)(((int64_t)blockIdx.x * 256 + threadIdx.x) >> 6), lane = threadIdx.x & 63;
    if (wave >= N * O) return;
    const int n = wave / O, o = wave - n * O;
    const float* xr = x + (int64_t)n * K;
    const float* wr = w + (int64_t)o * K;
    float acc = 0.f;
    for (int k = lane; k < K; k += 64) acc = __builtin_fmaf(xr[k], wr[k], acc);
    acc = wave_sum(acc);
    if (lane == 0) y[(int64_t)n * O + o] = act_apply(acc + (b != nullptr ? b[o] : 0.f), act);
}

__global__ __launch_bounds__(256) void small_linear_dz_kernel(const float* __restrict__ dy, const float* __restrict__ y,
                                                              float* __restrict__ dz, float* __restrict__ db, int N, int O, int act) {
    const int o = blockIdx.x * 256 + threadIdx.x;
    if (o >= O) return;
    float s = 0.f;
    for (int n = 0; n < N; ++n) {
        const float yv = y[(int64_t)n * O + o], g = dy[(int64_t)n * O + o];
        const float d = act == 1 ? (yv > 0.f ? g : 0.f) : act == 2 ? g * yv * (1.f - yv) : g;
        dz[(int64_t)n * O + o] = d;
        s += d;
    }
    if (db != nullptr) db[o] = s;
}

__global__ __launch_bounds__(256) void small_linear_dw_kernel(const float* __restrict__ dz, const float* __restrict__ x,
                                                              float* __restrict__ dw, int N, int K, int O) {
    const int64_t idx = (int64_t)blockIdx.x * 256 + threadIdx.x;
    if (idx >= (int64_t)O * K) return;
    const int o = (int)(idx / K), k = (int)(idx - (int64_t)o * K);
    float s = 0.f;
    for (int n = 0; n < N; ++n) s = __builtin_fmaf(dz[(int64_t)n * O + o], x[(int64_t)n * K + k], s);
    dw[idx] = s;
}

__global__ __launch_bounds__(256) void small_linear_dx_kernel(const float* __restrict__ dz, const float* __restrict__ w,
                                                              float* __restrict__ dx, int N, int K, int O) {
    const int64_t idx = (int64_t)blockIdx.x * 256 + threadIdx.x;
    if (idx >= (int64_t)N * K) return;
    const int n = (int)(idx / K), k = (int)(idx - (int64_t)n * K);
    float s = 0.f;
    for (int o = 0; o < O; ++o) s = __builtin_fmaf(dz[(int64_t)n * O + o], w[(int64_t)o * K + k], s);
    dx[idx] = s;
}

}

using namespace diga;

extern "C" size_t diga_norm_workspace_bytes(int64_t rows_per_seg, int64_t nseg, int64_t C) {
    if (rows_per_seg <= 0 || nseg <= 0 || C <= 0) return 0;
    const ColGeom g = make_geom(rows_per_seg, nseg, C);
    return ((size_t)nseg * g.nchunk * 3 * C + (size_t)5 * nseg * C + 64) * sizeof(float);
}

extern "C" int diga_bn_fwd(const float* x, int64_t ld_x, float* y, int64_t ld_y, const float* residual, int64_t ld_r,
                           const float* gamma, const float* beta, float* running_mean, float* running_var,
                           float* save_mean, float* save_invstd, float* save_ab, int64_t M, int64_t C, int training,
                           int relu, int y_twin, unsigned char* relu_bits, float momentum, float eps, void* workspace,
                           size_t workspace_bytes, void* stream) {
    DIGA_REQUIRE(!relu_bits || (relu && C % 32 == 0), DIGA_EINVAL, "bn_fwd: relu_bits needs relu and C % 32 == 0");
    DIGA_REQUIRE(!y_twin || (C % 8 == 0 && ld_y == C), DIGA_EINVAL, "bn_fwd: twin output needs C % 8 == 0 and a dense y");
    DIGA_REQUIRE(x && gamma && beta && save_mean && save_invstd && workspace && M > 0, DIGA_EINVAL, "bn_fwd: bad argument");
    DIGA_REQUIRE(y || (save_ab && !y_twin), DIGA_EINVAL, "bn_fwd: y = null (statistics and coefficients only; residual / relu_bits are then the consumer's) needs save_ab");
    DIGA_REQUIRE(training || (running_mean && running_var), DIGA_EINVAL, "bn_fwd: eval mode needs running statistics");
    int rc = check_norm("bn_fwd", C, {ld_x, y ? ld_y : C, residual ? ld_r : C}, {x, y ? (const void*)y : (const void*)x, residual});
    if (rc) return rc;
    DIGA_REQUIRE(workspace_bytes >= diga_norm_workspace_bytes(M, 1, C), DIGA_EWORKSPACE, "bn_fwd: workspace too small");
    hipStream_t st = (hipStream_t)stream;
    ProfScope prof(DIGA_PROF_NORM, st, (double)M * C * (8.0 + (training ? 4.0 : 0.0) + (residual ? 4.0 : 0.0)));
    const ColGeom g = make_geom(M, 1, C);
    float* partial = (float*)workspace;
    float* ab = save_ab != nullptr ? save_ab : partial + (size_t)g.nchunk * 3 * C;
    if (training) {
        hipLaunchKernelGGL(colstats_partial_kernel, dim3(g.nchunk, 1), dim3(kNormThreads), 0, st, x, ld_x, g, partial);
        hipLaunchKernelGGL(bn_finalize2_kernel, dim3((unsigned)ceil_div(C, kFinCh)), dim3(256), 0, st, partial, g, gamma, beta,
                           running_mean, running_var, save_mean, save_invstd, ab, momentum, eps);
    } else {
        hipLaunchKernelGGL(bn_eval_ab_kernel, dim3((unsigned)ceil_div(C, 128)), dim3(128), 0, st, gamma, beta, running_mean,
                           running_var, save_mean, save_invstd, ab, (int)C, eps);
    }
    if (y != nullptr)
        launch_affine(dim3(ew_blocks(M * C / 4)), st, x, ld_x, y, ld_y, residual, ld_r, ab,
                           ab + C, (int64_t)0, M, M, (int)C, relu, y_twin, relu_bits);
    return launch_status("diga_bn_fwd");
}

static int bn_fwd_from_partials(const char* who, const float* x, int64_t ld_x, float* y, int64_t ld_y, const float* residual,
                                int64_t ld_r, const float* gamma, const float* beta, float* running_mean,
                                float* running_var, float* save_mean, float* save_invstd, float* save_ab, int64_t M,
                                int64_t C, int relu, int y_twin, unsigned char* relu_bits, float momentum, float eps,
                                const float* partial, int64_t chunk_rows, const float* counts, int64_t n_records,
                                void* workspace, size_t workspace_bytes, void* stream) {
    DIGA_REQUIRE(!relu_bits || (relu && C % 32 == 0), DIGA_EINVAL, "%s: relu_bits needs relu and C %% 32 == 0", who);
    DIGA_REQUIRE(x && gamma && beta && save_mean && save_invstd && partial && workspace && M > 0, DIGA_EINVAL, "%s: bad argument", who);
    DIGA_REQUIRE(counts ? (n_records > 0 && n_records < (1 << 30)) : chunk_rows > 0, DIGA_EINVAL, "%s: bad chunk_rows / record count", who);
    DIGA_REQUIRE(y || (save_ab && !y_twin), DIGA_EINVAL, "%s: y = null (statistics and coefficients only) needs save_ab", who);
    int rc = check_norm(who, C, {ld_x, y ? ld_y : C, residual ? ld_r : C}, {x, y ? (const void*)y : (const void*)x, residual});
    if (rc) return rc;
    hipStream_t st = (hipStream_t)stream;
    ProfScope prof(DIGA_PROF_NORM, st, (double)M * C * (8.0 + (residual ? 4.0 : 0.0)));
    ColGeom g;
    g.rows_per_seg = M;
    g.nseg = 1;
    g.C = (int)C;
    g.chunk_rows = counts ? 1 : (int)chunk_rows;
    g.nchunk = counts ? (int)n_records : (int)ceil_div(M, chunk_rows);
    const int group = g.nchunk > 128 ? (int)ceil_div(g.nchunk, 96) : 1;
    const int ngroup = (int)ceil_div(g.nchunk, group);
    const size_t need = ((group > 1 ? (size_t)ngroup * 3 * C + (counts ? ngroup : 0) : 0) + (size_t)2 * C) * sizeof(float);
    DIGA_REQUIRE(workspace_bytes >= need, DIGA_EWORKSPACE, "%s: workspace too small (%zu < %zu)", who, workspace_bytes, need);
    float* ab = save_ab != nullptr ? save_ab : (float*)workspace;
    if (group > 1) {
        float* merged = (float*)workspace + 2 * C;
        float* mcounts = counts ? merged + (size_t)ngroup * 3 * C : nullptr;
        hipLaunchKernelGGL(merge_partials_kernel, dim3(ngroup, (unsigned)ceil_div(C, 64)), dim3(256), 0, st, partial, g, group,
                           merged, counts, mcounts);
        partial = merged;
        counts = mcounts;
        g.chunk_rows = counts ? 1 : (int)(chunk_rows * group);
        g.nchunk = ngroup;
    }
    hipLaunchKernelGGL(bn_finalize2_kernel, dim3((unsigned)ceil_div(C, kFinCh)), dim3(256), 0, st, partial, g, gamma, beta,
                       running_mean, running_var, save_mean, save_invstd, ab, momentum, eps, counts);
    if (y != nullptr)
        launch_affine(dim3(ew_blocks(M * C / 4)), st, x, ld_x, y, ld_y, residual, ld_r, ab,
                           ab + C, (int64_t)0, M, M, (int)C, relu, y_twin, relu_bits);
    return launch_status(who);
}

extern "C" int diga_bn_fwd_partials(const float* x, int64_t ld_x, float* y, int64_t ld_y, const float* residual,
                                    int64_t ld_r, const float* gamma, const float* beta, float* running_mean,
                                    float* running_var, float* save_mean, float* save_invstd, float* save_ab, int64_t M,
                                    int64_t C, int relu, int y_twin, unsigned char* relu_bits, float momentum, float eps,
                                    const float* partial, int64_t chunk_rows,
                                    void* workspace, size_t workspace_bytes, void* stream) {
    return bn_fwd_from_partials("diga_bn_fwd_partials", x, ld_x, y, ld_y, residual, ld_r, gamma, beta, running_mean, running_var, save_mean,
                                save_invstd, save_ab, M, C, relu, y_twin, relu_bits, momentum, eps, partial, chunk_rows, nullptr, 0,
                                workspace, workspace_bytes, stream);
}

extern "C" int diga_bn_fwd_records(const float* x, int64_t ld_x, float* y, int64_t ld_y, const float* residual,
                                   int64_t ld_r, const float* gamma, const float* beta, float* running_mean,
                                   float* running_var, float* save_mean, float* save_invstd, float* save_ab, int64_t M,
                                   int64_t C, int relu, int y_twin, unsigned char* relu_bits, float momentum, float eps,
                                   const float* partial, const float* counts, int64_t n_records,
                                   void* workspace, size_t workspace_bytes, void* stream) {
    DIGA_REQUIRE(counts != nullptr, DIGA_EINVAL, "diga_bn_fwd_records: null counts");
    return bn_fwd_from_partials("diga_bn_fwd_records", x, ld_x, y, ld_y, residual, ld_r, gamma, beta, running_mean, running_var, save_mean,
                                save_invstd, save_ab, M, C, relu, y_twin, relu_bits, momentum, eps, partial, 0, counts, n_records,
                                workspace, workspace_bytes, stream);
}

static int bn_bwd_impl(const float* dy, int64_t ld_dy, const float* x, int64_t ld_x, const float* y, int64_t ld_y,
                           const float* relu_ab, const float* gamma, const float* save_mean, const float* save_invstd,
                           float* dx, int64_t ld_dx,
                           float* dres, int64_t ld_dr, int64_t M, int64_t C, int training, int dx_twin, void* workspace,
                           size_t workspace_bytes, void* stream, float* dgamma, float* dbeta) {
    DIGA_REQUIRE(!dx_twin || (C % 8 == 0 && ld_dx == C), DIGA_EINVAL, "bn_bwd: twin output needs C % 8 == 0 and a dense dx");
    DIGA_REQUIRE(dy && x && gamma && save_mean && save_invstd && dx && workspace && M > 0, DIGA_EINVAL, "bn_bwd: bad argument");
    int rc = check_norm("bn_bwd", C, {ld_dy, ld_x, y ? ld_y : C, ld_dx, dres ? ld_dr : C}, {dy, x, y, dx, dres});
    if (rc) return rc;
    DIGA_REQUIRE(workspace_bytes >= diga_norm_workspace_bytes(M, 1, C), DIGA_EWORKSPACE, "bn_bwd: workspace too small");
    hipStream_t st = (hipStream_t)stream;
    ProfScope prof(DIGA_PROF_NORM, st,
                   (double)M * C * ((training ? 8.0 + (y ? 4.0 : 0.0) : 0.0) + 12.0 + (y ? 4.0 : 0.0) + (dres ? 4.0 : 0.0)));
    const ColGeom g = make_geom(M, 1, C);
    float* partial = (float*)workspace;
    float* kk = partial + (size_t)g.nchunk * 3 * C;
    DIGA_REQUIRE(!(y && relu_ab), DIGA_EINVAL, "bn_bwd: pass y or relu_ab, not both");
    if (training || dgamma)
        hipLaunchKernelGGL(bwd_partial_kernel, dim3(g.nchunk, 1), dim3(kNormThreads), 0, st, dy, ld_dy, x, ld_x, y, ld_y,
                           save_mean, save_invstd, 0, 1, g, partial, relu_ab);
    hipLaunchKernelGGL(bn_bwd_finalize2_kernel, dim3((unsigned)ceil_div(C, kFinCh)), dim3(256), 0, st, partial, g, gamma,
                       save_invstd, kk, training, dgamma, dbeta);
    launch_bwd_apply(dim3(ew_blocks(M * C / 4)), st, dy, ld_dy, x, ld_x, y, ld_y, save_mean,
                       save_invstd, 0, 1, kk, (int64_t)0, (int64_t)C, dx, ld_dx, dres, ld_dr, M, M, (int)C, relu_ab, dx_twin);
    return launch_status(dgamma ? "diga_bn_bwd_affine" : "diga_bn_bwd");
}

extern "C" int diga_bn_bwd(const float* dy, int64_t ld_dy, const float* x, int64_t ld_x, const float* y, int64_t ld_y,
                           const float* relu_ab, const float* gamma, const float* save_mean, const float* save_invstd,
                           float* dx, int64_t ld_dx,
                           float* dres, int64_t ld_dr, int64_t M, int64_t C, int training, int dx_twin, void* workspace,
                           size_t workspace_bytes, void* stream) {
    return bn_bwd_impl(dy, ld_dy, x, ld_x, y, ld_y, relu_ab, gamma, save_mean, save_invstd, dx, ld_dx, dres, ld_dr, M, C, training,
                       dx_twin, workspace, workspace_bytes, stream, nullptr, nullptr);
}

extern "C" int diga_bn_bwd_affine(const float* dy, int64_t ld_dy, const float* x, int64_t ld_x, const float* y, int64_t ld_y,
                                  const float* relu_ab, const float* gamma, const float* save_mean, const float* save_invstd,
                                  float* dx, int64_t ld_dx, float* dgamma, float* dbeta, int64_t M, int64_t C, int training,
                                  void* workspace, size_t workspace_bytes, void* stream) {
    DIGA_REQUIRE(dgamma && dbeta, DIGA_EINVAL, "bn_bwd_affine: dgamma and dbeta are required");
    return bn_bwd_impl(dy, ld_dy, x, ld_x, y, ld_y, relu_ab, gamma, save_mean, save_invstd, dx, ld_dx, nullptr, 0, M, C, training ? 1 : 0, 0,
                       workspace, workspace_bytes, stream, dgamma, dbeta);
}

extern "C" int diga_bn_bwd_partials(const float* g, int64_t ld_g, const float* x, int64_t ld_x, const float* gamma,
                                    const float* save_mean, const float* save_invstd, float* dx, int64_t ld_dx, int64_t M,
                                    int64_t C, int dx_twin, const float* partial, int64_t chunk_rows, void* workspace,
                                    size_t workspace_bytes, void* stream) {
    DIGA_REQUIRE(!dx_twin || (C % 8 == 0 && ld_dx == C), DIGA_EINVAL, "bn_bwd_partials: twin output needs C % 8 == 0 and a dense dx");
    DIGA_REQUIRE(g && x && gamma && save_mean && save_invstd && dx && partial && workspace && M > 0 && chunk_rows > 0, DIGA_EINVAL,
                 "bn_bwd_partials: bad argument");
    int rc = check_norm("bn_bwd_partials", C, {ld_g, ld_x, ld_dx}, {g, x, dx});
    if (rc) return rc;
    DIGA_REQUIRE(workspace_bytes >= (size_t)(3 + 64) * C * sizeof(float), DIGA_EWORKSPACE, "bn_bwd_partials: workspace too small");
    hipStream_t st = (hipStream_t)stream;
    ProfScope prof(DIGA_PROF_NORM, st, (double)M * C * 12.0);
    ColGeom geo;
    geo.rows_per_seg = M;
    geo.nseg = 1;
    geo.C = (int)C;
    geo.chunk_rows = (int)chunk_rows;
    geo.nchunk = (int)ceil_div(M, chunk_rows);
    float* kk = (float*)workspace;
    if (geo.nchunk > 64) {
        constexpr int kParts = 32;
        float* folded = kk + 3 * C;
        hipLaunchKernelGGL(colsum_fold_kernel, dim3((unsigned)ceil_div(2 * C, 64), kParts), dim3(256), 0, st, partial, geo.nchunk,
                           (int)(2 * C), kParts, folded);
        partial = folded;
        geo.nchunk = kParts;
        geo.chunk_rows = (int)ceil_div(M, kParts);
    }
    hipLaunchKernelGGL(bn_bwd_finalize2_kernel, dim3((unsigned)ceil_div(C, kFinCh)), dim3(256), 0, st, partial, geo, gamma,
                       save_invstd, kk, 1);
    launch_bwd_apply(dim3(ew_blocks(M * C / 4)), st, g, ld_g, x, ld_x, (const float*)nullptr,
                       (int64_t)0, save_mean, save_invstd, 0, 1, kk, (int64_t)0, (int64_t)C, dx, ld_dx, (float*)nullptr,
                       (int64_t)0, M, M, (int)C, (const float*)nullptr, dx_twin);
    return launch_status("diga_bn_bwd_partials");
}

extern "C" int diga_gn_fwd(const float* x, int64_t ld_x, float* y, int64_t ld_y, const float* gamma, const float* beta,
                           const float* chan_scale, float* save_mean, float* save_invstd, int64_t N, int64_t HW, int64_t C,
                           int64_t G, int relu, float eps, void* workspace, size_t workspace_bytes, void* stream) {
    DIGA_REQUIRE(x && y && gamma && beta && save_mean && save_invstd && workspace && N > 0 && HW > 0, DIGA_EINVAL, "gn_fwd: bad argument");
    DIGA_REQUIRE(G > 0 && C % G == 0, DIGA_EINVAL, "gn_fwd: C must be divisible by the group count");
    int rc = check_norm("gn_fwd", C, {ld_x, ld_y}, {x, y});
    if (rc) return rc;
    DIGA_REQUIRE(workspace_bytes >= diga_norm_workspace_bytes(HW, N, C), DIGA_EWORKSPACE, "gn_fwd: workspace too small");
    hipStream_t st = (hipStream_t)stream;
    ProfScope prof(DIGA_PROF_NORM, st, (double)N * HW * C * 12.0);
    const ColGeom g = make_geom(HW, N, C);
    float* partial = (float*)workspace;
    float* ab = partial + (size_t)N * g.nchunk * 3 * C;
    hipLaunchKernelGGL(colstats_partial_kernel, dim3(g.nchunk, (unsigned)N), dim3(kNormThreads), 0, st, x, ld_x, g, partial);
    const int cpg_f = (int)(C / G);
    if (cpg_f <= 64 && (cpg_f & (cpg_f - 1)) == 0)
        hipLaunchKernelGGL(gn_finalize2_kernel, dim3((unsigned)ceil_div(N * G, 4)), dim3(256), 0, st, partial, g, (int)G, gamma,
                           beta, chan_scale, save_mean, save_invstd, ab, eps);
    else
        hipLaunchKernelGGL(gn_finalize_kernel, dim3((unsigned)ceil_div(N * G, 64)), dim3(64), 0, st, partial, g, (int)G, gamma,
                           beta, chan_scale, save_mean, save_invstd, ab, eps);
    launch_affine(dim3(ew_blocks(N * HW * C / 4)), st, x, ld_x, y, ld_y,
                       (const float*)nullptr, (int64_t)0, ab, ab + N * C, C, HW, N * HW, (int)C, relu, 0);
    return launch_status("diga_gn_fwd");
}

extern "C" int diga_gn_bwd(const float* dy, int64_t ld_dy, const float* x, int64_t ld_x, const float* y, int64_t ld_y,
                           const float* gamma, const float* chan_scale, const float* save_mean, const float* save_invstd,
                           float* dx, int64_t ld_dx, float* dgamma, float* dbeta, int64_t N, int64_t HW, int64_t C,
                           int64_t G, void* workspace, size_t workspace_bytes, void* stream) {
    DIGA_REQUIRE(dy && x && gamma && save_mean && save_invstd && dx && dgamma && dbeta && workspace && N > 0 && HW > 0,
                 DIGA_EINVAL, "gn_bwd: bad argument");
    DIGA_REQUIRE(G > 0 && C % G == 0, DIGA_EINVAL, "gn_bwd: C must be divisible by the group count");
    int rc = check_norm("gn_bwd", C, {ld_dy, ld_x, y ? ld_y : C, ld_dx}, {dy, x, y, dx});
    if (rc) return rc;
    DIGA_REQUIRE(workspace_bytes >= diga_norm_workspace_bytes(HW, N, C), DIGA_EWORKSPACE, "gn_bwd: workspace too small");
    hipStream_t st = (hipStream_t)stream;
    ProfScope prof(DIGA_PROF_NORM, st, (double)N * HW * C * (20.0 + (y ? 8.0 : 0.0)));
    const ColGeom g = make_geom(HW, N, C);
    const int cpg = (int)(C / G);
    float* partial = (float*)workspace;
    float* kk = partial + (size_t)N * g.nchunk * 3 * C;
    float* chan_sums = kk + (size_t)3 * N * C;
    hipLaunchKernelGGL(bwd_partial_kernel, dim3(g.nchunk, (unsigned)N), dim3(kNormThreads), 0, st, dy, ld_dy, x, ld_x, y, ld_y,
                       save_mean, save_invstd, (int)G, cpg, g, partial, (const float*)nullptr);
    if (cpg <= 64 && (cpg & (cpg - 1)) == 0)
        hipLaunchKernelGGL(gn_bwd_finalize2_kernel, dim3((unsigned)ceil_div(N * G, 4)), dim3(256), 0, st, partial, g, (int)G,
                           gamma, chan_scale, save_invstd, kk, chan_sums);
    else
        hipLaunchKernelGGL(gn_bwd_finalize_kernel, dim3((unsigned)ceil_div(N * G, 64)), dim3(64), 0, st, partial, g, (int)G,
                           gamma, chan_scale, save_invstd, kk, chan_sums);
    hipLaunchKernelGGL(gn_param_grad_kernel, dim3((unsigned)ceil_div(C, 128)), dim3(128), 0, st, chan_sums, (int)N, (int)C,
                       dgamma, dbeta);
    launch_bwd_apply(dim3(ew_blocks(N * HW * C / 4)), st, dy, ld_dy, x, ld_x, y, ld_y,
                       save_mean, save_invstd, (int)G, cpg, kk, C, N * C, dx, ld_dx, (float*)nullptr, (int64_t)0, HW, N * HW,
                       (int)C, (const float*)nullptr, 0);
    return launch_status("diga_gn_bwd");
}
// ... 167 lines not shown
```

### diga_amd/csrc/winograd.hip

```cpp
#include "common.h"

namespace diga {

int gemm_batched_f32_dma(const float* A, int64_t rows_per_batch, int batches, int64_t K, const float* W, int64_t Cout,
                         float* out, hipStream_t st);
size_t wgrad_batched_slab_bytes(int64_t rows, int batches, int64_t Cout, int64_t Cin);
int wgrad_batched_f32_dma(const float* Z, const float* V, float* dU, float* slab, int64_t rows, int batches, int64_t Cout,
                          int64_t Cin, hipStream_t st);

namespace wino {

struct WinoGeom {
    int N, H, W, d;
    int m;
    int tys, txs;
    int64_t T, Tp;
};

int phase_tiles(int len, int d, int m) {
    int s = 0;
    for (int a = 0; a < d; ++a) {
        const int n = len > a ? (len - a + d - 1) / d : 0;
        s += (n + m - 1) / m;
    }
    return s;
}

WinoGeom make_wino(int64_t N, int64_t H, int64_t W, int64_t d, int64_t m) {
    WinoGeom g;
    g.N = (int)N; g.H = (int)H; g.W = (int)W; g.d = (int)d; g.m = (int)m;
    g.tys = phase_tiles((int)H, (int)d, (int)m);
    g.txs = phase_tiles((int)W, (int)d, (int)m);
    g.T = N * g.tys * g.txs;
    g.Tp = ceil_div(g.T, 256) * 256;
    return g;
}
static inline int products(int64_t m) { return (int)((m + 2) * (m + 2)); }
static inline bool tile_ok(int64_t m) { return m == 2 || m == 4 || m == 6; }

__global__ __launch_bounds__(256) void wino_tiles_kernel(int4* __restrict__ tab, WinoGeom g) {
    const int64_t t = (int64_t)blockIdx.x * 256 + threadIdx.x;
    if (t >= g.Tp) return;
    if (t >= g.T) {
        tab[t] = make_int4(-1, 0, 0, 0);
        return;
    }
    const int timg = g.tys * g.txs;
    const int n = (int)(t / timg), r = (int)(t - (int64_t)n * timg);
    constexpr int kBand = 1;
    const int band = r / (kBand * g.txs), rem = r - band * kBand * g.txs;
    const int rows_in_band = min(kBand, g.tys - kBand * band);
    int Cc = rem / rows_in_band, R = kBand * band + (rem - Cc * rows_in_band);
    int a = 0, b = 0;
    for (; a < g.d; ++a) {
        const int cnt = g.H > a ? (g.H - a + g.d - 1) / g.d : 0;
        const int tl = (cnt + g.m - 1) / g.m;
        if (R < tl) break;
        R -= tl;
    }
    for (; b < g.d; ++b) {
        const int cnt = g.W > b ? (g.W - b + g.d - 1) / g.d : 0;
        const int tl = (cnt + g.m - 1) / g.m;
        if (Cc < tl) break;
        Cc -= tl;
    }
    tab[t] = make_int4(n, a + g.m * R * g.d, b + g.m * Cc * g.d, 0);
}

using f32x4nt = __attribute__((ext_vector_type(4))) float;
__device__ __forceinline__ void nt_store4(float* p, float4 v) {
    __builtin_nontemporal_store((f32x4nt){v.x, v.y, v.z, v.w}, reinterpret_cast<f32x4nt*>(p));
}
__device__ __forceinline__ float4 nt_load4(const float* p) {
    const f32x4nt v = __builtin_nontemporal_load(reinterpret_cast<const f32x4nt*>(p));
    return make_float4(v.x, v.y, v.z, v.w);
}
__device__ __forceinline__ float4 f4add(float4 a, float4 b) { return make_float4(a.x + b.x, a.y + b.y, a.z + b.z, a.w + b.w); }
__device__ __forceinline__ float4 f4sub(float4 a, float4 b) { return make_float4(a.x - b.x, a.y - b.y, a.z - b.z, a.w - b.w); }
__device__ __forceinline__ float4 f4half(float4 a) { return make_float4(0.5f * a.x, 0.5f * a.y, 0.5f * a.z, 0.5f * a.w); }

__global__ __launch_bounds__(256) void wino_weight_kernel(const float* __restrict__ w, float* __restrict__ U, int Cout, int Cin,
                                                          int flip) {
    const int64_t idx = (int64_t)blockIdx.x * 256 + threadIdx.x;
    const int c4n = Cin / 4;
    if (idx >= (int64_t)Cout * c4n) return;
    const int co = (int)(idx / c4n), c = (int)(idx - (int64_t)co * c4n) * 4;
    float4 g[3][3];
#pragma unroll
    for (int r = 0; r < 3; ++r)
#pragma unroll
        for (int s = 0; s < 3; ++s) {
            const int rr = flip ? 2 - r : r, ss = flip ? 2 - s : s;
            g[r][s] = *reinterpret_cast<const float4*>(w + ((int64_t)co * 9 + rr * 3 + ss) * Cin + c);
        }
    float4 t[4][3];
#pragma unroll
    for (int s = 0; s < 3; ++s) {
        const float4 sum = f4add(g[0][s], g[2][s]);
        t[0][s] = g[0][s];
        t[1][s] = f4half(f4add(sum, g[1][s]));
        t[2][s] = f4half(f4sub(sum, g[1][s]));
        t[3][s] = g[2][s];
    }
    const int64_t plane = (int64_t)Cout * Cin;
    float* o = U + (int64_t)co * Cin + c;
#pragma unroll
    for (int i = 0; i < 4; ++i) {
        const float4 sum = f4add(t[i][0], t[i][2]);
        *reinterpret_cast<float4*>(o + (4 * i + 0) * plane) = t[i][0];
        *reinterpret_cast<float4*>(o + (4 * i + 1) * plane) = f4half(f4add(sum, t[i][1]));
        *reinterpret_cast<float4*>(o + (4 * i + 2) * plane) = f4half(f4sub(sum, t[i][1]));
        *reinterpret_cast<float4*>(o + (4 * i + 3) * plane) = t[i][2];
    }
}

__global__ __launch_bounds__(256) void wino_input_kernel(const float* __restrict__ x, int64_t ld, const int4* __restrict__ tab,
                                                         float* __restrict__ V, int64_t Tp, int C, int H, int W, int d) {
    const int c4n = C / 4;
    const int64_t idx = (int64_t)blockIdx.x * 256 + threadIdx.x;
    if (idx >= Tp * c4n) return;
    const int64_t t = idx / c4n;
    const int c = (int)(idx - t * c4n) * 4;
    const int4 e = tab[t];
    const float4 z = make_float4(0.f, 0.f, 0.f, 0.f);
    const int img = max(e.x, 0);
    float4 p[4][4];
#pragma unroll
    for (int i = 0; i < 4; ++i) {
        const int y = e.y + (i - 1) * d;
        const bool yok = e.x >= 0 && (unsigned)y < (unsigned)H;
        const int yc = min(max(y, 0), H - 1);
#pragma unroll
        for (int j = 0; j < 4; ++j) {
            const int xx = e.z + (j - 1) * d;
            const bool ok = yok && (unsigned)xx < (unsigned)W;
            const float4 v = *reinterpret_cast<const float4*>(x + ((int64_t)(img * H + yc) * W + min(max(xx, 0), W - 1)) * ld + c);
            p[i][j] = ok ? v : z;
        }
    }
    float4 m[4][4];
#pragma unroll
    for (int j = 0; j < 4; ++j) {
        m[0][j] = f4sub(p[0][j], p[2][j]);
        m[1][j] = f4add(p[1][j], p[2][j]);
        m[2][j] = f4sub(p[2][j], p[1][j]);
        m[3][j] = f4sub(p[1][j], p[3][j]);
    }
    float* o = V + t * C + c;
    const int64_t plane = Tp * C;
#pragma unroll
    for (int i = 0; i < 4; ++i) {
        nt_store4(o + (4 * i + 0) * plane, f4sub(m[i][0], m[i][2]));
        nt_store4(o + (4 * i + 1) * plane, f4add(m[i][1], m[i][2]));
        nt_store4(o + (4 * i + 2) * plane, f4sub(m[i][2], m[i][1]));
        nt_store4(o + (4 * i + 3) * plane, f4sub(m[i][1], m[i][3]));
    }
}

// ... 670 lines not shown
}
struct WinoStatsPlan {
    int tpb, CG, TL;
    int64_t blocks, records;
};
template <int M>
static WinoStatsPlan stats_plan_m(const WinoGeom& g, int64_t Cout) {
    using VT = typename Vec<M>::Out;
    constexpr int VW = sizeof(VT) / 4;
    WinoStatsPlan p;
    const int64_t groups = Cout / VW;
    p.CG = groups >= 256 ? 256 : groups >= 128 ? 128 : 64;
    p.TL = 256 / p.CG;
    p.tpb = 4 * p.TL;
    p.blocks = ceil_div(g.T, p.tpb);
    p.records = p.blocks * p.TL;
    return p;
}
static WinoStatsPlan stats_plan(const WinoGeom& g, int64_t Cout) {
    return g.m == 6 ? stats_plan_m<6>(g, Cout) : stats_plan_m<4>(g, Cout);
}
template <int M>
static void launch_output_stats_m(const float* Mb, const int4* tab, const float* bias, float* out, int64_t out_ld, const WinoGeom& g,
                                  int64_t Cout, float* stats, hipStream_t st) {
    using VT = typename Vec<M>::Out;
    constexpr int VW = sizeof(VT) / 4;
    const WinoStatsPlan p = stats_plan_m<M>(g, Cout);
    float* counts = stats + p.records * 3 * Cout;
    hipLaunchKernelGGL((winoM_output_stats_kernel<M, VT>), dim3((unsigned)p.blocks, (unsigned)ceil_div(Cout, (int64_t)p.CG * VW)), dim3(256), 0, st,
                       Mb, tab, bias, out, out_ld, g.T, g.Tp, (int)Cout, g.H, g.W, g.d, p.tpb, p.CG, stats, counts);
}

constexpr int kEpiTileLanes = 2;
template <int M, bool ADD, int MASK>
static void launch_output_epi2_sums(const float* Mb, const int4* tab, float* out, int64_t out_ld, const WinoGeom& g, int64_t Cout, int64_t G,
                                    int tpb, const WinoEpi& ep, hipStream_t st) {
    using VT = typename Vec<M>::Out;
    constexpr int VW = sizeof(VT) / 4;
    constexpr int TL = kEpiTileLanes;
    const dim3 grid((unsigned)G, (unsigned)ceil_div(Cout, (256 / TL) * VW));
    if (ep.partials != nullptr)
        hipLaunchKernelGGL((winoM_output_epi2_kernel<M, VT, TL, ADD, MASK, true>), grid, dim3(256), 0, st, Mb, tab, out, out_ld, g.T, g.Tp,
                           (int)Cout, g.H, g.W, g.d, tpb, ep);
    else
        hipLaunchKernelGGL((winoM_output_epi2_kernel<M, VT, TL, ADD, MASK, false>), grid, dim3(256), 0, st, Mb, tab, out, out_ld, g.T, g.Tp,
                           (int)Cout, g.H, g.W, g.d, tpb, ep);
}
template <int M, bool ADD>
static void launch_output_epi2_mask(const float* Mb, const int4* tab, float* out, int64_t out_ld, const WinoGeom& g, int64_t Cout, int64_t G,
                                    int tpb, const WinoEpi& ep, hipStream_t st) {
    if (ep.masky != nullptr) launch_output_epi2_sums<M, ADD, 1>(Mb, tab, out, out_ld, g, Cout, G, tpb, ep, st);
    else if (ep.maskbits != nullptr) launch_output_epi2_sums<M, ADD, 2>(Mb, tab, out, out_ld, g, Cout, G, tpb, ep, st);
    else if (ep.relu_ab != nullptr) launch_output_epi2_sums<M, ADD, 3>(Mb, tab, out, out_ld, g, Cout, G, tpb, ep, st);
    else launch_output_epi2_sums<M, ADD, 0>(Mb, tab, out, out_ld, g, Cout, G, tpb, ep, st);
}
template <int M>
static void launch_output_epi2_m(const float* Mb, const int4* tab, float* out, int64_t out_ld, const WinoGeom& g, int64_t Cout, int64_t G,
                                 int tpb, const WinoEpi& ep, hipStream_t st) {
    if (ep.add != nullptr) launch_output_epi2_mask<M, true>(Mb, tab, out, out_ld, g, Cout, G, tpb, ep, st);
    else launch_output_epi2_mask<M, false>(Mb, tab, out, out_ld, g, Cout, G, tpb, ep, st);
}

template <int M>
static void launch_dy_m(const float* dy, int64_t dy_ld, const int4* tab, float* Z, const WinoGeom& g, int64_t Cout, hipStream_t st) {
    using VT = typename Vec<M>::Dy;
    constexpr int VW = sizeof(VT) / 4;
    hipLaunchKernelGGL((winoM_dy_kernel<M, VT>), dim3((unsigned)ceil_div(g.Tp * (Cout / VW), 256)), dim3(256), 0, st, dy, dy_ld, tab, Z, g.Tp,
                       (int)Cout, g.H, g.W, g.d);
}
template <int M>
static void launch_dw_m(const float* dU, float* dw, int64_t Cout, int64_t Cin, hipStream_t st) {
    hipLaunchKernelGGL((winoM_dw_kernel<M, float2>), dim3((unsigned)ceil_div(Cout * (Cin / 2), 256)), dim3(256), 0, st, dU, dw, (int)Cout, (int)Cin);
}

struct WinoWgradLayout {
    size_t tab, V, Z, dU, slab, total;
};
WinoWgradLayout wino_wgrad_layout(const WinoGeom& g, int64_t Cin, int64_t Cout, bool with_v) {
    WinoWgradLayout l;
    size_t o = 0;
    l.tab = o; o += (size_t)g.Tp * sizeof(int4);
    l.V = o; o += with_v ? (size_t)products(g.m) * g.Tp * Cin * sizeof(float) : 0;
    l.Z = o; o += (size_t)products(g.m) * g.Tp * Cout * sizeof(float);
    l.dU = o; o += (size_t)products(g.m) * Cout * Cin * sizeof(float);
    l.slab = o; o += wgrad_batched_slab_bytes(g.Tp, products(g.m), Cout, Cin);
    l.total = o + 64;
    return l;
}

struct WinoLayout {
    size_t tab, U, V, M, total;
};
WinoLayout wino_layout(const WinoGeom& g, int64_t Cin, int64_t Cout) {
    WinoLayout l;
    size_t o = 0;
    l.tab = o; o += (size_t)g.Tp * sizeof(int4);
    l.U = o; o += (size_t)products(g.m) * Cout * Cin * sizeof(float);
    l.V = o; o += (size_t)products(g.m) * g.Tp * Cin * sizeof(float);
    l.M = o; o += (size_t)products(g.m) * g.Tp * Cout * sizeof(float);
    l.total = o + 64;
    return l;
}

}
}

using namespace diga;
using namespace diga::wino;

extern "C" size_t diga_conv2d_winograd_workspace_bytes(int64_t N, int64_t H, int64_t W, int64_t Cin, int64_t Cout, int64_t dilation, int64_t tile) {
    if (N <= 0 || H <= 0 || W <= 0 || Cin <= 0 || Cout <= 0 || dilation <= 0 || !tile_ok(tile)) return 0;
    return wino_layout(make_wino(N, H, W, dilation, tile), Cin, Cout).total;
}

static int winograd_impl(const float* in, const float* wgt, const float* bias, float* out, void* workspace,
                         size_t workspace_bytes, int64_t N, int64_t H, int64_t W, int64_t Cin, int64_t in_ld,
                         int64_t Cout, int64_t out_ld, int64_t dilation, int64_t tile, int flip, const diga_bwd_epilogue_t* epi, int prof_tag,
                         void* stream, float* v_keep = nullptr, float* stats = nullptr,
                         const void* tile_table = nullptr, int reflect = 0) {
    DIGA_REQUIRE(!reflect || (tile != 2 && !flip && !epi && dilation < H && dilation < W), DIGA_EINVAL,
                 "conv2d_winograd: reflection padding comes with the forward of 4x4 / 6x6 tiles (pad < H, W)");
    DIGA_REQUIRE(in && wgt && out && workspace, DIGA_EINVAL, "conv2d_winograd: null pointer");
    DIGA_REQUIRE(N > 0 && H > 0 && W > 0 && dilation > 0 && dilation < 4096, DIGA_EINVAL, "conv2d_winograd: bad shape");
    DIGA_REQUIRE(tile_ok(tile), DIGA_EINVAL, "conv2d_winograd: tile must be 2, 4 or 6 (F(2x2,3x3) / F(4x4,3x3) / F(6x6,3x3))");
    DIGA_REQUIRE(Cin % 32 == 0 && Cout % 4 == 0 && Cout > 64 && in_ld >= Cin && in_ld % 4 == 0 && out_ld >= Cout && out_ld % 4 == 0,
                 DIGA_EINVAL, "conv2d_winograd: Cin %% 32, Cout %% 4 (> 64) and leading dimensions %% 4 required");
    DIGA_REQUIRE(aligned16(in) && aligned16(wgt) && aligned16(out) && aligned16(workspace) && (!bias || aligned16(bias)), DIGA_EALIGN,
                 "conv2d_winograd: pointers must be 16-byte aligned");
    DIGA_REQUIRE(N * H * W < (1ll << 31), DIGA_EINVAL, "conv2d_winograd: too many pixels");
    const WinoGeom g = make_wino(N, H, W, dilation, tile);
    const int P = products(tile);
    DIGA_REQUIRE(P * g.Tp / 256 < 32768, DIGA_EINVAL, "conv2d_winograd: too many tiles for one launch");
    const WinoLayout l = wino_layout(g, Cin, Cout);
    DIGA_REQUIRE(workspace_bytes >= l.total, DIGA_EWORKSPACE, "conv2d_winograd: workspace too small (%zu < %zu)", workspace_bytes, l.total);
    DIGA_REQUIRE(!stats || (epi == nullptr && tile != 2 && aligned16(stats)), DIGA_EINVAL,
                 "conv2d_winograd: statistics come with the forward output transform of 4x4 / 6x6 tiles (16-byte aligned buffer)");
    DIGA_REQUIRE(!tile_table || aligned16(tile_table), DIGA_EALIGN, "conv2d_winograd: tile_table must be 16-byte aligned");
    char* ws = static_cast<char*>(workspace);
    const int4* tab = tile_table != nullptr ? static_cast<const int4*>(tile_table) : reinterpret_cast<const int4*>(ws + l.tab);
    float* U = reinterpret_cast<float*>(ws + l.U);
    float* V = v_keep != nullptr ? v_keep : reinterpret_cast<float*>(ws + l.V);
    float* Mb = reinterpret_cast<float*>(ws + l.M);
    hipStream_t st = (hipStream_t)stream;
    ProfScope prof(prof_tag == DIGA_PROF_CONV_BWD_DATA ? DIGA_PROF_CONV_BWD_DATA : DIGA_PROF_CONV_FWD, st,
                   2.0 * (double)(N * H * W) * (double)Cout * 9.0 * (double)Cin);
    if (tile_table == nullptr)
        hipLaunchKernelGGL(wino_tiles_kernel, dim3((unsigned)ceil_div(g.Tp, 256)), dim3(256), 0, st, reinterpret_cast<int4*>(ws + l.tab), g);
    if (tile == 6) launch_weight_m<6>(wgt, U, Cout, Cin, flip, st);
    else if (tile == 4) launch_weight_m<4>(wgt, U, Cout, Cin, flip, st);
    else
        hipLaunchKernelGGL(wino_weight_kernel, dim3((unsigned)ceil_div(Cout * (Cin / 4), 256)), dim3(256), 0, st, wgt, U, (int)Cout, (int)Cin,
                           flip);
    launch_input(tile, in, in_ld, tab, V, g.Tp, Cin, H, W, dilation, st, reflect);
    int rc = gemm_batched_f32_dma(V, g.Tp, P, Cin, U, Cout, Mb, st);
    if (rc) return rc;
    if (epi == nullptr && stats != nullptr) {
        if (tile == 6) launch_output_stats_m<6>(Mb, tab, bias, out, out_ld, g, Cout, stats, st);
        else launch_output_stats_m<4>(Mb, tab, bias, out, out_ld, g, Cout, stats, st);
    } else if (epi == nullptr) {
        if (tile == 6) launch_output_m<6>(Mb, tab, bias, out, out_ld, g, Cout, st);
        else if (tile == 4) launch_output_m<4>(Mb, tab, bias, out, out_ld, g, Cout, st);
        else
            hipLaunchKernelGGL(wino_output_kernel, dim3((unsigned)ceil_div(g.T * (Cout / 4), 256)), dim3(256), 0, st, Mb, tab, bias, out,
                               out_ld, g.T, g.Tp, (int)Cout, (int)H, (int)W, (int)dilation);
    } else {
        WinoEpi ep;
        ep.add = epi->addend; ep.add_ld = epi->addend_ld;
        ep.masky = epi->mask_y; ep.masky_ld = epi->mask_ld;
        ep.maskbits = epi->mask_bits; ep.maskbits_ld = epi->mask_bits_ld;
        ep.x = epi->x; ep.x_ld = epi->x_ld;
        ep.relu_ab = epi->relu_ab; ep.mean = epi->mean; ep.invstd = epi->invstd; ep.partials = epi->partials;
        const int64_t G = ceil_div(N * H * W, 128);
        const int tpb = (int)ceil_div(g.T, G);
        if (tile == 6) launch_output_epi2_m<6>(Mb, tab, out, out_ld, g, Cout, G, tpb, ep, st);
        else if (tile == 4) launch_output_epi2_m<4>(Mb, tab, out, out_ld, g, Cout, G, tpb, ep, st);
        else
            hipLaunchKernelGGL(wino_output_epi_kernel, dim3((unsigned)G, (unsigned)ceil_div(Cout, 256)), dim3(256), 0, st, Mb, tab, out,
                               out_ld, g.T, g.Tp, (int)Cout, (int)H, (int)W, (int)dilation, tpb, ep);
    }
    return launch_status("diga_conv2d_winograd_f32");
}

extern "C" size_t diga_conv2d_winograd_tile_table_bytes(int64_t N, int64_t H, int64_t W, int64_t dilation, int64_t tile) {
    if (N <= 0 || H <= 0 || W <= 0 || dilation <= 0 || !tile_ok(tile)) return 0;
    return (size_t)make_wino(N, H, W, dilation, tile).Tp * sizeof(int4);
}

extern "C" int diga_conv2d_winograd_tile_table(void* table, int64_t N, int64_t H, int64_t W, int64_t dilation, int64_t tile, void* stream) {
    DIGA_REQUIRE(table && aligned16(table), DIGA_EINVAL, "conv2d_winograd_tile_table: null / unaligned table");
    DIGA_REQUIRE(N > 0 && H > 0 && W > 0 && dilation > 0 && dilation < 4096 && tile_ok(tile) && N * H * W < (1ll << 31), DIGA_EINVAL,
                 "conv2d_winograd_tile_table: bad shape / tile");
    const WinoGeom g = make_wino(N, H, W, dilation, tile);
    hipLaunchKernelGGL(wino_tiles_kernel, dim3((unsigned)ceil_div(g.Tp, 256)), dim3(256), 0, (hipStream_t)stream, static_cast<int4*>(table), g);
    return launch_status("diga_conv2d_winograd_tile_table");
}

extern "C" size_t diga_conv2d_winograd_stats_records(int64_t N, int64_t H, int64_t W, int64_t Cout, int64_t dilation, int64_t tile) {
    if (N <= 0 || H <= 0 || W <= 0 || Cout <= 0 || dilation <= 0 || (tile != 4 && tile != 6)) return 0;
    return (size_t)stats_plan(make_wino(N, H, W, dilation, tile), Cout).records;
}

extern "C" size_t diga_conv2d_winograd_stats_floats(int64_t N, int64_t H, int64_t W, int64_t Cout, int64_t dilation, int64_t tile) {
    const size_t r = diga_conv2d_winograd_stats_records(N, H, W, Cout, dilation, tile);
    return r * 3 * (size_t)Cout + r;
}

extern "C" int diga_conv2d_winograd_f32(const float* in, const float* wgt, const float* bias, float* out, void* workspace,
                                        size_t workspace_bytes, int64_t N, int64_t H, int64_t W, int64_t Cin, int64_t in_ld,
                                        int64_t Cout, int64_t out_ld, int64_t dilation, int64_t tile, int flip, float* stats_partial,
                                        const void* tile_table, int prof_tag, void* stream) {
    return winograd_impl(in, wgt, bias, out, workspace, workspace_bytes, N, H, W, Cin, in_ld, Cout, out_ld, dilation, tile, flip, nullptr,
                         prof_tag, stream, nullptr, stats_partial, tile_table);
}

extern "C" int diga_conv2d_winograd_f32_opts(const float* in, const float* wgt, const float* bias, float* out, void* workspace,
                                             size_t workspace_bytes, int64_t N, int64_t H, int64_t W, int64_t Cin, int64_t in_ld,
                                             int64_t Cout, int64_t out_ld, int64_t dilation, int64_t tile, const diga_conv_options_t* opts,
                                             const void* tile_table, int prof_tag, void* stream) {
    DIGA_REQUIRE(opts != nullptr, DIGA_EINVAL, "conv2d_winograd_opts: null options");
    DIGA_REQUIRE(opts->upsample_shift == 0 && opts->activation == 0, DIGA_EINVAL,
                 "conv2d_winograd_opts: only reflect_pad is folded on the Winograd path (upsampling / tanh: the direct `_opts` kernels)");
    return winograd_impl(in, wgt, bias, out, workspace, workspace_bytes, N, H, W, Cin, in_ld, Cout, out_ld, dilation, tile, 0, nullptr,
                         prof_tag, stream, nullptr, nullptr, tile_table, opts->reflect_pad ? 1 : 0);
}

extern "C" size_t diga_conv2d_winograd_v_floats(int64_t N, int64_t H, int64_t W, int64_t Cin, int64_t dilation, int64_t tile) {
    if (N <= 0 || H <= 0 || W <= 0 || Cin <= 0 || dilation <= 0 || !tile_ok(tile)) return 0;
    return (size_t)products(tile) * make_wino(N, H, W, dilation, tile).Tp * Cin;
}

extern "C" int diga_conv2d_winograd_f32_keep(const float* in, const float* wgt, const float* bias, float* out, float* v_keep,
                                             void* workspace, size_t workspace_bytes, int64_t N, int64_t H, int64_t W, int64_t Cin,
                                             int64_t in_ld, int64_t Cout, int64_t out_ld, int64_t dilation, int64_t tile,
                                             float* stats_partial, const void* tile_table, int prof_tag, void* stream) {
    DIGA_REQUIRE(v_keep != nullptr && aligned16(v_keep), DIGA_EINVAL, "conv2d_winograd_keep: v_keep must be a 16-byte aligned buffer");
    return winograd_impl(in, wgt, bias, out, workspace, workspace_bytes, N, H, W, Cin, in_ld, Cout, out_ld, dilation, tile, 0, nullptr,
                         prof_tag, stream, v_keep, stats_partial, tile_table);
}

extern "C" int diga_conv2d_winograd_f32_epi(const float* in, const float* wgt, float* out, void* workspace, size_t workspace_bytes,
                                            int64_t N, int64_t H, int64_t W, int64_t Cin, int64_t in_ld, int64_t Cout,
                                            int64_t out_ld, int64_t dilation, int64_t tile, int flip, const diga_bwd_epilogue_t* e,
                                            const void* tile_table, int prof_tag, void* stream) {
    DIGA_REQUIRE(e != nullptr, DIGA_EINVAL, "conv2d_winograd_epi: null epilogue descriptor");
    DIGA_REQUIRE(e->addend || e->mask_y || e->mask_bits || e->x, DIGA_EINVAL, "conv2d_winograd_epi: empty epilogue descriptor");
    DIGA_REQUIRE(!e->addend || (aligned16(e->addend) && e->addend_ld >= Cout && e->addend_ld % 4 == 0), DIGA_EINVAL, "conv2d_winograd_epi: bad addend");
    DIGA_REQUIRE(!e->mask_y || (aligned16(e->mask_y) && e->mask_ld >= Cout && e->mask_ld % 4 == 0), DIGA_EINVAL, "conv2d_winograd_epi: bad mask_y");
    DIGA_REQUIRE(!e->x || (aligned16(e->x) && e->x_ld >= Cout && e->x_ld % 4 == 0), DIGA_EINVAL, "conv2d_winograd_epi: bad x");
    DIGA_REQUIRE((e->mask_y != nullptr) + (e->relu_ab != nullptr) + (e->mask_bits != nullptr) <= 1, DIGA_EINVAL,
                 "conv2d_winograd_epi: give one of mask_y, mask_bits, relu_ab");
    DIGA_REQUIRE(!e->mask_bits || e->mask_bits_ld * 8 >= Cout, DIGA_EINVAL, "conv2d_winograd_epi: bad mask_bits");
    DIGA_REQUIRE(!e->relu_ab || (e->x && aligned16(e->relu_ab)), DIGA_EINVAL, "conv2d_winograd_epi: relu_ab needs x");
    DIGA_REQUIRE(!e->partials || (e->x && e->mean && e->invstd && aligned16(e->mean) && aligned16(e->invstd)), DIGA_EINVAL,
                 "conv2d_winograd_epi: partials need x, mean and invstd");
    return winograd_impl(in, wgt, nullptr, out, workspace, workspace_bytes, N, H, W, Cin, in_ld, Cout, out_ld, dilation, tile, flip, e, prof_tag,
                         stream, nullptr, nullptr, tile_table);
}

extern "C" size_t diga_conv2d_wgrad_winograd_workspace_bytes(int64_t N, int64_t H, int64_t W, int64_t Cin, int64_t Cout,
                                                             int64_t dilation, int64_t tile, int v_kept) {
    if (N <= 0 || H <= 0 || W <= 0 || Cin <= 0 || Cout <= 0 || dilation <= 0 || Cout % 256 != 0 || Cin % 128 != 0 || !tile_ok(tile)) return 0;
    return wino_wgrad_layout(make_wino(N, H, W, dilation, tile), Cin, Cout, v_kept == 0).total;
}

static int wgrad_winograd_impl(const float* dy, const float* x, const float* v_kept, float* dw, void* workspace,
                               size_t workspace_bytes, int64_t N, int64_t H, int64_t W, int64_t Cin, int64_t x_ld,
                               int64_t Cout, int64_t dy_ld, int64_t dilation, int64_t tile, const void* tile_table, void* stream) {
    DIGA_REQUIRE(!tile_table || aligned16(tile_table), DIGA_EALIGN, "conv2d_wgrad_winograd: tile_table must be 16-byte aligned");
    DIGA_REQUIRE(dy && (x || v_kept) && dw && workspace, DIGA_EINVAL, "conv2d_wgrad_winograd: null pointer");
    DIGA_REQUIRE(!v_kept || aligned16(v_kept), DIGA_EALIGN, "conv2d_wgrad_winograd: v_kept must be 16-byte aligned");
    DIGA_REQUIRE(N > 0 && H > 0 && W > 0 && dilation > 0 && dilation < 4096 && N * H * W < (1ll << 31) && tile_ok(tile),
                 DIGA_EINVAL, "conv2d_wgrad_winograd: bad shape / tile");
    DIGA_REQUIRE(Cout % 256 == 0 && Cin % 128 == 0 && x_ld >= Cin && x_ld % 4 == 0 && dy_ld >= Cout && dy_ld % 4 == 0, DIGA_EINVAL,
                 "conv2d_wgrad_winograd: Cout %% 256, Cin %% 128 and leading dimensions %% 4 required");
    DIGA_REQUIRE(aligned16(dy) && (!x || aligned16(x)) && aligned16(dw) && aligned16(workspace), DIGA_EALIGN,
                 "conv2d_wgrad_winograd: pointers must be 16-byte aligned");
    const WinoGeom g = make_wino(N, H, W, dilation, tile);
    const WinoWgradLayout l = wino_wgrad_layout(g, Cin, Cout, v_kept == nullptr);
    DIGA_REQUIRE(workspace_bytes >= l.total, DIGA_EWORKSPACE, "conv2d_wgrad_winograd: workspace too small (%zu < %zu)", workspace_bytes,
                 l.total);
    char* ws = static_cast<char*>(workspace);
    const int4* tab = tile_table != nullptr ? static_cast<const int4*>(tile_table) : reinterpret_cast<const int4*>(ws + l.tab);
    const float* V = v_kept != nullptr ? v_kept : reinterpret_cast<float*>(ws + l.V);
    float* Z = reinterpret_cast<float*>(ws + l.Z);
    float* dU = reinterpret_cast<float*>(ws + l.dU);
    float* slab = reinterpret_cast<float*>(ws + l.slab);
    hipStream_t st = (hipStream_t)stream;
    ProfScope prof(DIGA_PROF_CONV_BWD_WEIGHT, st, 2.0 * (double)(N * H * W) * (double)Cout * 9.0 * (double)Cin);
    if (tile_table == nullptr)
        hipLaunchKernelGGL(wino_tiles_kernel, dim3((unsigned)ceil_div(g.Tp, 256)), dim3(256), 0, st, reinterpret_cast<int4*>(ws + l.tab), g);
    if (v_kept == nullptr)
        launch_input(tile, x, x_ld, tab, reinterpret_cast<float*>(ws + l.V), g.Tp, Cin, H, W, dilation, st);
    if (tile == 6) launch_dy_m<6>(dy, dy_ld, tab, Z, g, Cout, st);
    else if (tile == 4) launch_dy_m<4>(dy, dy_ld, tab, Z, g, Cout, st);
    else
        hipLaunchKernelGGL(wino_dy_kernel, dim3((unsigned)ceil_div(g.Tp * (Cout / 4), 256)), dim3(256), 0, st, dy, dy_ld, tab, Z, g.Tp,
                           (int)Cout, (int)H, (int)W, (int)dilation);
    int rc = wgrad_batched_f32_dma(Z, V, dU, slab, g.Tp, products(tile), Cout, Cin, st);
    if (rc) return rc;
    if (tile == 6) launch_dw_m<6>(dU, dw, Cout, Cin, st);
    else if (tile == 4) launch_dw_m<4>(dU, dw, Cout, Cin, st);
    else
        hipLaunchKernelGGL(wino_dw_kernel, dim3((unsigned)ceil_div(Cout * (Cin / 4), 256)), dim3(256), 0, st, dU, dw, (int)Cout, (int)Cin);
    return launch_status("diga_conv2d_wgrad_winograd_f32");
}

extern "C" int diga_conv2d_wgrad_winograd_f32(const float* dy, const float* x, const float* v_kept, float* dw, void* workspace,
// ... 7 lines not shown
```

### diga_amd/model/norm.py

```python
import torch
import torch.nn as nn

from diga_amd import _lib, config


def nhwc(x):
    t = x.permute(0, 2, 3, 1)
    if t.dtype != torch.float32:
        t = t.float()
    return t if t.is_contiguous() else t.contiguous()


def rows_ld(t):
    n, h, w, c = t.shape
    ld = t.stride(2)
    if t.stride(3) == 1 and ld >= c and t.stride(1) == w * ld and t.stride(0) == h * w * ld and ld % 4 == 0 \
            and t.data_ptr() % 16 == 0:
        return ld
    return None


def as_rows(t):
    ld = rows_ld(t)
    if ld is None:
        t = t.contiguous()
        ld = t.shape[3]
    return t, ld


def alias_slice(buf, lo, hi):
    n, h, w, c = buf.shape
    return torch.empty(0, dtype=buf.dtype, device=buf.device).set_(
        buf.untyped_storage(), buf.storage_offset() + lo, (n, h, w, hi - lo), (h * w * c, w * c, c, 1))


def _ws(rows_per_seg, nseg, c, device):
    return _lib.workspace(_lib.lib.diga_norm_workspace_bytes(rows_per_seg, nseg, c), device, "norm")


class _BnFn(torch.autograd.Function):

    @staticmethod
    def forward(ctx, x, residual, weight, bias, running_mean, running_var, training, relu, momentum, eps,
                partials=None, twin_out=False, dx_twin=False, box=None, res_box=None):
        _lib.require_gpu(x)
        xn = nhwc(x.detach())
        n, h, w, c = xn.shape
        m = n * h * w
        rn = None if residual is None else nhwc(residual.detach())
        y = torch.empty_like(xn)
        save_mean = torch.empty(c, dtype=torch.float32, device=xn.device)
        save_invstd = torch.empty_like(save_mean)
        save_ab = torch.empty(2 * c, dtype=torch.float32, device=xn.device) if (relu and residual is None) else None
        ws = _ws(m, 1, c, xn.device)
        bits = None
        if (box is not None and relu and residual is not None and c % 32 == 0 and _relu_bits_enabled()):
            bits = torch.empty((m, c // 8), dtype=torch.uint8, device=xn.device)
        if partials is not None and training and isinstance(partials[1], tuple):
            recs = int(partials[1][1])
            wsr = _lib.workspace(max(_lib.lib.diga_norm_workspace_bytes(m, 1, c), (96 * 3 * c + 2 * c + 128) * 4), xn.device, "norm_rec")
            _lib.call("diga_bn_fwd_records", _lib.ptr(xn), c, _lib.ptr(y), c, _lib.ptr(rn), c, _lib.ptr(weight),
                      _lib.ptr(bias), _lib.ptr(running_mean), _lib.ptr(running_var), _lib.ptr(save_mean),
                      _lib.ptr(save_invstd), _lib.ptr(save_ab), m, c, 1 if relu else 0, 1 if twin_out else 0,
                      _lib.ptr(bits), float(momentum), float(eps), _lib.ptr(partials[0]),
                      _lib.C.c_void_p(partials[0].data_ptr() + recs * 3 * c * 4), recs, _lib.ptr(wsr), wsr.numel(), _lib.stream())
        elif partials is not None and training:
            _lib.call("diga_bn_fwd_partials", _lib.ptr(xn), c, _lib.ptr(y), c, _lib.ptr(rn), c, _lib.ptr(weight),
                      _lib.ptr(bias), _lib.ptr(running_mean), _lib.ptr(running_var), _lib.ptr(save_mean),
                      _lib.ptr(save_invstd), _lib.ptr(save_ab), m, c, 1 if relu else 0, 1 if twin_out else 0,
                      _lib.ptr(bits),
                      float(momentum), float(eps), _lib.ptr(partials[0]), int(partials[1]), _lib.ptr(ws), ws.numel(),
                      _lib.stream())
        else:
            _lib.call("diga_bn_fwd", _lib.ptr(xn), c, _lib.ptr(y), c, _lib.ptr(rn), c, _lib.ptr(weight), _lib.ptr(bias),
                      _lib.ptr(running_mean), _lib.ptr(running_var), _lib.ptr(save_mean), _lib.ptr(save_invstd),
                      _lib.ptr(save_ab), m, c, 1 if training else 0, 1 if relu else 0, 1 if twin_out else 0,
                      _lib.ptr(bits),
                      float(momentum), float(eps), _lib.ptr(ws), ws.numel(), _lib.stream())
        ctx.save_for_backward(xn, y if (relu and save_ab is None) else None, weight, save_mean, save_invstd, save_ab)
        ctx.flags = (training, residual is not None)
        ctx.dx_twin = bool(dx_twin and c % 8 == 0)
        ctx.box, ctx.res_box = box, res_box
        if box is not None:
            box.update(x=xn, mean=save_mean, invstd=save_invstd, relu_ab=save_ab, has_res=residual is not None, rows=m, C=c,
                       mask_bits=bits)
        return y.permute(0, 3, 1, 2)

    @staticmethod
    def backward(ctx, gy):
        xn, y, weight, save_mean, save_invstd, save_ab = ctx.saved_tensors
        training, has_res = ctx.flags
        n, h, w, c = xn.shape
        m = n * h * w
        g, ld_g = as_rows(gy.permute(0, 2, 3, 1))
        dx = torch.empty_like(xn)
        dgamma = dbeta = None
        if ctx.needs_input_grad[2] or ctx.needs_input_grad[3]:
            if has_res or ctx.box is not None:
                raise RuntimeError("DigaTrainableBatchNorm2d: no residual input / fused backward epilogue with a trainable affine pair")
            dgamma, dbeta = torch.empty(c, dtype=torch.float32, device=xn.device), torch.empty(c, dtype=torch.float32, device=xn.device)
            ws = _ws(m, 1, c, xn.device)
            _lib.call("diga_bn_bwd_affine", _lib.ptr(g), ld_g, _lib.ptr(xn), c, _lib.ptr(y), c, _lib.ptr(save_ab), _lib.ptr(weight),
                      _lib.ptr(save_mean), _lib.ptr(save_invstd), _lib.ptr(dx), c, _lib.ptr(dgamma), _lib.ptr(dbeta), m, c,
                      1 if training else 0, _lib.ptr(ws), ws.numel(), _lib.stream())
            return (dx.permute(0, 3, 1, 2), None, dgamma if ctx.needs_input_grad[2] else None, dbeta if ctx.needs_input_grad[3] else None,
                    None, None, None, None, None, None, None, None, None, None, None)
        pre = ctx.box.pop("premasked", None) if ctx.box is not None else None
        if pre is not None and pre[0] == g.data_ptr() and pre[2]._version == pre[4] and ld_g == c and training:
            ws = _lib.workspace(67 * c * 4, xn.device, "norm_kk")
            _lib.call("diga_bn_bwd_partials", _lib.ptr(g), ld_g, _lib.ptr(xn), c, _lib.ptr(weight), _lib.ptr(save_mean),
                      _lib.ptr(save_invstd), _lib.ptr(dx), c, m, c, 1 if ctx.dx_twin else 0, _lib.ptr(pre[1]), int(pre[5]),
                      _lib.ptr(ws), ws.numel(), _lib.stream())
            dres = g if has_res else None
        else:
            dres = torch.empty_like(xn) if has_res else None
            ws = _ws(m, 1, c, xn.device)
            _lib.call("diga_bn_bwd", _lib.ptr(g), ld_g, _lib.ptr(xn), c, _lib.ptr(y), c, _lib.ptr(save_ab), _lib.ptr(weight),
                      _lib.ptr(save_mean), _lib.ptr(save_invstd), _lib.ptr(dx), c, _lib.ptr(dres), c, m, c,
                      1 if training else 0, 1 if ctx.dx_twin else 0, _lib.ptr(ws), ws.numel(), _lib.stream())
        if dres is not None and ctx.res_box is not None and not ctx.res_box.get("consumed"):
            ctx.res_box["dres"] = dres
            dres = None
        return (dx.permute(0, 3, 1, 2), None if dres is None else dres.permute(0, 3, 1, 2),
                dgamma, dbeta, None, None, None, None, None, None, None, None, None, None, None)


class DigaBatchNorm2d(nn.BatchNorm2d):

    def forward(self, x, residual=None, relu=False, twin_out=False, dx_twin=False):
        if self.weight.requires_grad or self.bias.requires_grad:
            raise RuntimeError("DigaBatchNorm2d implements the frozen-affine BN of the DiGA path; "
                               "set requires_grad=False on weight and bias")
        training = self.training or self.running_mean is None
        if getattr(self, "_nbt_external", False):
            self._nbt_external = False
        elif self.training and self.num_batches_tracked is not None:
            self.num_batches_tracked.add_(1)
        twin_out = bool(twin_out and relu and residual is None and x.shape[1] % 8 == 0)
        box = res_box = None
        if training and relu and torch.is_grad_enabled() and x.requires_grad and fuse_backward_enabled():
            box = {}
            if residual is not None:
                rb = getattr(residual, "_diga_bn_box", None)
                if rb is not None and rb.get("consumer_ready") and "res_claimed" not in rb:
                    rb["res_claimed"] = True
                    res_box = rb
        y = _BnFn.apply(x, residual, self.weight, self.bias, self.running_mean, self.running_var, training, relu,
                        self.momentum, self.eps, getattr(x, "_diga_bn_partials", None), twin_out, bool(dx_twin), box, res_box)
        if twin_out:
            y._diga_is_twin = True
        if box is not None:
            y._diga_bn_box = box
        return y


class DigaTrainableBatchNorm2d(DigaBatchNorm2d):

    def forward(self, x, relu=False):
        training = self.training or self.running_mean is None
        if getattr(self, "_nbt_external", False):
            self._nbt_external = False
        elif self.training and self.num_batches_tracked is not None:
            self.num_batches_tracked.add_(1)
        return _BnFn.apply(x, None, self.weight, self.bias, self.running_mean, self.running_var, training, relu, self.momentum, self.eps,
                           getattr(x, "_diga_bn_partials", None), False, False, None, None)


def bump_batches_tracked(model):
    bns = [m for m in model.modules() if isinstance(m, DigaBatchNorm2d) and m.num_batches_tracked is not None]
    if not bns:
        return
    flat = getattr(model, "_nbt_flat", None)
    ok = (flat is not None and len(bns) == flat.numel() and flat.device == bns[0].num_batches_tracked.device
          and all(b.num_batches_tracked.data_ptr() == flat.data_ptr() + 8 * i for i, b in enumerate(bns)))
    if not ok:
        flat = torch.stack([b.num_batches_tracked.detach().reshape(()) for b in bns]).contiguous()
        for i, b in enumerate(bns):
            b.num_batches_tracked = flat[i]
        object.__setattr__(model, "_nbt_flat", flat)
        object.__setattr__(model, "_nbt_inc", None)
    state = tuple(b.training for b in bns)
    inc = getattr(model, "_nbt_inc", None)
    if inc is None or inc[0] != state:
        inc = (state, torch.tensor([1 if t else 0 for t in state], dtype=torch.int64).to(flat.device))
        object.__setattr__(model, "_nbt_inc", inc)
    for b in bns:
        b._nbt_external = True
    if all(state):
        flat.add_(1)
    else:
        flat.add_(inc[1])


def _relu_bits_enabled():
    return config.active().relu_bits


def fuse_backward_enabled():
    return config.active().fuse_bwd


class _GnFn(torch.autograd.Function):
    @staticmethod
    def forward(ctx, x, weight, bias, groups, eps, relu, chan_scale, out):
        _lib.require_gpu(x)
        xn = nhwc(x.detach())
        n, h, w, c = xn.shape
        y = torch.empty_like(xn) if out is None else out
        y_, ld_y = (y, c) if out is None else (out, rows_ld(out))
        if ld_y is None:
            raise ValueError("GroupNorm output slice must be a channel slice of a contiguous NHWC tensor")
        save_mean = torch.empty(n * groups, dtype=torch.float32, device=xn.device)
        save_invstd = torch.empty_like(save_mean)
        cs = None if chan_scale is None else chan_scale.detach().float().contiguous()
        ws = _ws(h * w, n, c, xn.device)
        _lib.call("diga_gn_fwd", _lib.ptr(xn), c, _lib.ptr(y_), ld_y, _lib.ptr(weight.detach()), _lib.ptr(bias.detach()),
                  _lib.ptr(cs), _lib.ptr(save_mean), _lib.ptr(save_invstd), n, h * w, c, groups, 1 if relu else 0,
                  float(eps), _lib.ptr(ws), ws.numel(), _lib.stream())
        ctx.save_for_backward(xn, y_ if relu else None, weight, cs, save_mean, save_invstd)
        ctx.groups = groups
        return y_.permute(0, 3, 1, 2)

    @staticmethod
    def backward(ctx, gy):
        xn, y, weight, cs, save_mean, save_invstd = ctx.saved_tensors
        n, h, w, c = xn.shape
        g, ld_g = as_rows(gy.permute(0, 2, 3, 1))
        ld_y = rows_ld(y) if y is not None else c
        dx = torch.empty_like(xn)
        dgamma = torch.empty(c, dtype=torch.float32, device=xn.device)
        dbeta = torch.empty_like(dgamma)
        ws = _ws(h * w, n, c, xn.device)
        _lib.call("diga_gn_bwd", _lib.ptr(g), ld_g, _lib.ptr(xn), c, _lib.ptr(y), ld_y, _lib.ptr(weight.detach()),
                  _lib.ptr(cs), _lib.ptr(save_mean), _lib.ptr(save_invstd), _lib.ptr(dx), c, _lib.ptr(dgamma),
                  _lib.ptr(dbeta), n, h * w, c, ctx.groups, _lib.ptr(ws), ws.numel(), _lib.stream())
        return dx.permute(0, 3, 1, 2), dgamma, dbeta, None, None, None, None, None


class DigaGroupNorm(nn.GroupNorm):

    def forward(self, x, relu=False, chan_scale=None, out=None):
        return _GnFn.apply(x, self.weight, self.bias, self.num_groups, self.eps, relu, chan_scale, out)


class _AssembleFn(torch.autograd.Function):

    @staticmethod
    def forward(ctx, buf, width, *slices):
        ctx.width = width
        ctx.k = len(slices)
        return buf.permute(0, 3, 1, 2)

    @staticmethod
    def backward(ctx, g):
        gn = g.permute(0, 2, 3, 1)
        if not gn.is_contiguous():
            gn = gn.contiguous()
        outs = [alias_slice(gn, i * ctx.width, (i + 1) * ctx.width).permute(0, 3, 1, 2) for i in range(ctx.k)]
        return (None, None, *outs)


def assemble(buf, width, slices):
    return _AssembleFn.apply(buf, width, *slices)


class _AvgPoolFn(torch.autograd.Function):
    @staticmethod
    def forward(ctx, x):
        xn = nhwc(x.detach())
        n, h, w, c = xn.shape
        out = torch.empty((n, c), dtype=torch.float32, device=xn.device)
        ws = _ws(h * w, n, c, xn.device)
        _lib.call("diga_avgpool_nhwc", _lib.ptr(xn), c, _lib.ptr(out), n, h * w, c, _lib.ptr(ws), ws.numel(), _lib.stream())
        ctx.shape = (n, h, w, c)
        return out

    @staticmethod
    def backward(ctx, g):
        n, h, w, c = ctx.shape
        return (g / float(h * w))[:, :, None, None].expand(n, c, h, w)


class _ChannelGateFn(torch.autograd.Function):
    @staticmethod
    def forward(ctx, x, gate):
        xn = nhwc(x.detach())
        n, h, w, c = xn.shape
        gt = gate.detach().float().contiguous()
        y = torch.empty_like(xn)
        _lib.call("diga_channel_affine", _lib.ptr(xn), c, _lib.ptr(y), c, _lib.ptr(gt), None, n, h * w, c, _lib.stream())
        ctx.save_for_backward(xn, gt)
        return y.permute(0, 3, 1, 2)

    @staticmethod
    def backward(ctx, gy):
        xn, gt = ctx.saved_tensors
        n, h, w, c = xn.shape
        g, ld_g = as_rows(gy.permute(0, 2, 3, 1))
        dx = torch.empty_like(xn)
        _lib.call("diga_channel_affine", _lib.ptr(g), ld_g, _lib.ptr(dx), c, _lib.ptr(gt), None, n, h * w, c, _lib.stream())
        dgate = torch.empty((n, c), dtype=torch.float32, device=xn.device)
        ws = _ws(h * w, n, c, xn.device)
        _lib.call("diga_channel_dot", _lib.ptr(g), ld_g, _lib.ptr(xn), c, _lib.ptr(dgate), n, h * w, c, _lib.ptr(ws),
                  ws.numel(), _lib.stream())
        return dx.permute(0, 3, 1, 2), dgate


class _SmallLinearFn(torch.autograd.Function):

    @staticmethod
    def forward(ctx, x, weight, bias, act):
        _lib.require_gpu(x, weight)
        xc, wc = x.detach().float().contiguous(), weight.detach().float().contiguous()
        bc = None if bias is None else bias.detach().float().contiguous()
        n, k = xc.shape
        o = wc.shape[0]
        y = torch.empty((n, o), dtype=torch.float32, device=xc.device)
        _lib.call("diga_small_linear_fwd", _lib.ptr(xc), _lib.ptr(wc), _lib.ptr(bc), _lib.ptr(y), n, k, o, act, _lib.stream())
        ctx.save_for_backward(xc, wc, y)
        ctx.act, ctx.has_bias = act, bias is not None
        return y

    @staticmethod
    def backward(ctx, gy):
        xc, wc, y = ctx.saved_tensors
        n, k = xc.shape
        o = wc.shape[0]
        g = gy.float().contiguous()
        dz = torch.empty_like(y)
        dx = torch.empty_like(xc) if ctx.needs_input_grad[0] else None
        dw = torch.empty_like(wc) if ctx.needs_input_grad[1] else None
        db = torch.empty(o, dtype=torch.float32, device=xc.device) if (ctx.has_bias and ctx.needs_input_grad[2]) else None
        _lib.call("diga_small_linear_bwd", _lib.ptr(xc), _lib.ptr(wc), _lib.ptr(y), _lib.ptr(g), _lib.ptr(dz), _lib.ptr(dx), _lib.ptr(dw),
                  _lib.ptr(db), n, k, o, ctx.act, _lib.stream())
        return dx, dw, db, None


def small_linear(x, linear, act):
    return _SmallLinearFn.apply(x, linear.weight, linear.bias, act)


def global_avg_pool(x):
    return _AvgPoolFn.apply(x)


def channel_gate(x, gate):
    return _ChannelGateFn.apply(x, gate)


class _MaxPoolFn(torch.autograd.Function):
# ... 37 lines not shown
```

### diga_amd/model/seg_model_noaux.py

```python
from dataclasses import dataclass
from typing import Tuple

import torch
import torch.nn as nn

from diga_amd import config
from diga_amd.model import norm as dn
from diga_amd.model.conv import DigaConv2d, takes_twin_only_input


@dataclass(frozen=True)
class Arch:
    layers: Tuple[int, ...] = (3, 4, 23, 3)
    planes: Tuple[int, ...] = (64, 128, 256, 512)
    strides: Tuple[int, ...] = (1, 2, 1, 1)
    dilations: Tuple[int, ...] = (1, 1, 2, 4)
    stem: int = 64
    expansion: int = 4
    aspp_dilations: Tuple[int, ...] = (6, 12, 18, 24)
    aspp_width: int = 256
    gn_groups: int = 32
    se_reduction: int = 16
    n_classes: int = 19
    droprate: float = 0.1


RESNET101 = Arch()
TINY = Arch(layers=(1, 1, 2, 1), planes=(16, 32, 64, 128), stem=16)


def _frozen_bn(channels):
    bn = dn.DigaBatchNorm2d(channels, affine=True)
    for p in bn.parameters():
        p.requires_grad = False
    return bn


class Bottleneck(nn.Module):
    expansion = 4

    def __init__(self, inplanes, planes, stride=1, dilation=1, downsample=None):
        super().__init__()
        self.conv1 = DigaConv2d(inplanes, planes, 1, stride=stride, bias=False)
        self.bn1 = _frozen_bn(planes)
        self.conv2 = DigaConv2d(planes, planes, 3, stride=1, padding=dilation, dilation=dilation, bias=False)
        self.bn2 = _frozen_bn(planes)
        self.conv3 = DigaConv2d(planes, planes * self.expansion, 1, bias=False)
        self.bn3 = _frozen_bn(planes * self.expansion)
        self.relu = nn.ReLU(inplace=True)
        self.downsample = downsample
        self.stride = stride
        for conv in (self.conv1, self.conv2, self.conv3) + ((downsample[0],) if downsample is not None else ()):
            conv.emit_bn_stats = True

    def forward(self, x):
        grad = torch.is_grad_enabled()
        chain = None
        if self.downsample is not None:
            box = getattr(x, "_diga_bn_box", None)
            if (grad and x.requires_grad and dn.fuse_backward_enabled() and tuple(self.conv1.stride) == (1, 1)
                    and tuple(self.downsample[0].stride) == (1, 1) and config.active().junction_chain):
                chain = {"remaining": 2, "acc": None, "box": box}
            elif box is not None:
                x._diga_bn_box = None
        tw2 = takes_twin_only_input(self.conv2)
        c3 = config.active().twin_conv3
        tw3 = (grad or c3 != "2") and c3 != "0" and takes_twin_only_input(self.conv3, pointwise_ok=True)
        y1 = self.conv1(x, chain=chain)
        y = self.bn1(y1, relu=True, twin_out=tw2)
        y = self.bn2(self.conv2(y, twin_grad=tw2 and grad), relu=True, twin_out=tw3, dx_twin=tw2 and grad)
        if self.downsample is None:
            skip = x
        elif chain is not None:
            skip = self.downsample[1](self.downsample[0](x, chain=chain))
        else:
            skip = self.downsample(x)
        return self.bn3(self.conv3(y, twin_grad=tw3), residual=skip, relu=True, dx_twin=tw3)


class SEBlock(nn.Module):
    def __init__(self, inplanes, r=16):
        super().__init__()
        self.global_pool = nn.AdaptiveAvgPool2d((1, 1))
        self.se = nn.Sequential(nn.Linear(inplanes, inplanes // r), nn.ReLU(inplace=True),
                                nn.Linear(inplanes // r, inplanes), nn.Sigmoid())

    def forward(self, x):
        hidden = dn.small_linear(dn.global_avg_pool(x), self.se[0], 1)
        for hook in self.se[1]._forward_hooks.values():
            hook(self.se[1], (hidden,), hidden)
        return dn.channel_gate(x, dn.small_linear(hidden, self.se[2], 2))


class Classifier_Module2(nn.Module):

    def __init__(self, inplanes, dilation_series, padding_series, num_classes, droprate=0.1, use_se=True,
                 width=256, groups=32, se_reduction=16):
        super().__init__()
        self.width = width

        def branch(k, d, p):
            return nn.Sequential(DigaConv2d(inplanes, width, k, stride=1, padding=p, dilation=d, bias=True),
                                 dn.DigaGroupNorm(groups, width), nn.ReLU(inplace=True))

        self.conv2d_list = nn.ModuleList([branch(1, 1, 0)] +
                                         [branch(3, d, p) for d, p in zip(dilation_series, padding_series)])
        for seq in self.conv2d_list:
            seq[0].share_twin = True
        cat = width * (len(dilation_series) + 1)
        tail = [DigaConv2d(cat, width, 3, stride=1, padding=1, bias=True), dn.DigaGroupNorm(groups, width)]
        self.bottleneck = nn.Sequential(*([SEBlock(cat, se_reduction)] if use_se else []), *tail)
        self.head = nn.Sequential(nn.Dropout2d(droprate), DigaConv2d(width, num_classes, 1, bias=False))
        nn.init.zeros_(self.bottleneck[-2].bias)

    def _drop_scale(self, n, c, device):
        drop = self.head[0]
        if not drop.training or drop.p <= 0.0:
            return None
        keep = (torch.rand((n, c), device=device) >= drop.p).to(torch.float32)
        return keep / (1.0 - drop.p)

    def forward(self, x, get_feat=True):
        n, _, h, w = x.shape
        nb = len(self.conv2d_list)
        buf = torch.empty((n, h, w, self.width * nb), dtype=torch.float32, device=x.device)
        slices = []
        chain = None
        if torch.is_grad_enabled() and x.requires_grad and dn.fuse_backward_enabled():
            chain = {"remaining": nb, "acc": None, "box": getattr(x, "_diga_bn_box", None)}
        for b, (conv, gn, _) in enumerate(self.conv2d_list):
            dst = dn.alias_slice(buf, b * self.width, (b + 1) * self.width)
            slices.append(gn(conv(x, chain=chain), relu=True, out=dst))
        y = dn.assemble(buf, self.width, slices)
        mods = list(self.bottleneck)
        if len(mods) == 3:
            y = mods[0](y)
        y = mods[-2](y)
        feat = mods[-1](y, chan_scale=self._drop_scale(n, self.width, x.device))
        out = self.head[1](feat)
        return {'feat': feat, 'out': out} if get_feat else out


class ResNetMulti(nn.Module):
    def __init__(self, block, layers, num_classes, bn_clr=False, arch=RESNET101):
        super().__init__()
        self.bn_clr = bn_clr
        self.inplanes = arch.stem
        self.conv1 = DigaConv2d(3, arch.stem, 7, stride=2, padding=3, bias=False)
        self.bn1 = _frozen_bn(arch.stem)
        self.conv1.emit_bn_stats = True
        self.relu = nn.ReLU(inplace=True)
        self.maxpool = dn.DigaMaxPool3x3s2()
        stages = [self._make_layer(block, arch.planes[i], layers[i], arch.strides[i], arch.dilations[i])
                  for i in range(4)]
        self.layer1, self.layer2, self.layer3, self.layer4 = stages
        self.layer5 = Classifier_Module2(self.inplanes, list(arch.aspp_dilations), list(arch.aspp_dilations),
                                         num_classes, arch.droprate, True, arch.aspp_width, arch.gn_groups,
                                         arch.se_reduction)
        if bn_clr:
            self.bn_pretrain = dn.DigaBatchNorm2d(self.inplanes, affine=True)
            for p in self.bn_pretrain.parameters():
                p.requires_grad = False
        for m in self.modules():
            if isinstance(m, nn.Conv2d):
                m.weight.data.normal_(0, 0.01)
            elif isinstance(m, nn.BatchNorm2d):
                m.weight.data.fill_(1)
                m.bias.data.zero_()

    def _make_layer(self, block, planes, blocks, stride=1, dilation=1):
        down = None
        if stride != 1 or self.inplanes != planes * block.expansion or dilation in (2, 4):
            down = nn.Sequential(DigaConv2d(self.inplanes, planes * block.expansion, 1, stride=stride, bias=False),
                                 _frozen_bn(planes * block.expansion))
        seq = [block(self.inplanes, planes, stride, dilation=dilation, downsample=down)]
        self.inplanes = planes * block.expansion
        seq += [block(self.inplanes, planes, dilation=dilation) for _ in range(1, blocks)]
        return nn.Sequential(*seq)

    def stem(self, x):
        return self.maxpool(self.bn1(self.conv1(x), relu=True))

    def forward(self, x):
        if self.training:
            dn.bump_batches_tracked(self)
        x = self.layer4(self.layer3(self.layer2(self.layer1(self.stem(x)))))
        if self.bn_clr:
            x = self.bn_pretrain(x)
        return self.layer5(x)


def DeeplabMulti(pretrained=True, num_classes=19, initialization=None, bn_clr=False, arch=RESNET101):
    model = ResNetMulti(Bottleneck, list(arch.layers), num_classes, bn_clr=bn_clr, arch=arch)
    if pretrained and initialization is not None:
        saved = torch.load(initialization, map_location="cpu")
        saved = saved.get('state_dict', saved)
        own = model.state_dict()
        own.update({k: v for k, v in saved.items() if k in own and v.shape == own[k].shape})
        model.load_state_dict(own)
    return model
```

### include/diga_hip.h

```cpp
#ifndef DIGA_HIP_H
#define DIGA_HIP_H

#include <stddef.h>
#include <stdint.h>

#ifdef __cplusplus
extern "C" {
#endif
#if defined(__GNUC__)
#pragma GCC visibility push(default)
#endif

#define DIGA_ABI_VERSION 1

#define DIGA_OK 0
#define DIGA_EINVAL (-1)
#define DIGA_EALIGN (-2)
#define DIGA_EWORKSPACE (-3)

#define DIGA_IGNORE_LABEL 255

int diga_version(void);
const char* diga_last_error_string(void);

// ... 91 lines not shown
                         int64_t off_dy, int64_t off_dx, float* stats_partial, int prof_tag, void* stream);

size_t diga_conv2d_stats_floats(int64_t N, int64_t Ho, int64_t Wo, int64_t Cout);
int diga_conv2d_stats_chunk_rows(int64_t N, int64_t Hi, int64_t Wi, int64_t Cin, int64_t Ho, int64_t Wo, int64_t Cout, int64_t R,
                                 int64_t S, int64_t stride_y, int64_t stride_x, int64_t off_y0, int64_t off_x0, int math);
int diga_conv2d_epi_chunk_rows(int64_t N, int64_t Hi, int64_t Wi, int64_t Cin, int64_t Ho, int64_t Wo, int64_t Cout, int64_t R,
                               int64_t S, int64_t stride_y, int64_t stride_x, int64_t off_y0, int64_t off_x0, int math);

typedef struct {
    const float* addend;
    int64_t addend_ld;
    const float* mask_y;
    int64_t mask_ld;
    const float* x;
    int64_t x_ld;
    const float* relu_ab;
    const float* mean;
    const float* invstd;
    float* partials;
    const unsigned char* mask_bits;
    int64_t mask_bits_ld;
} diga_bwd_epilogue_t;

int diga_conv2d_nhwc_f32_epi(const float* in, const float* wgt, float* out, int64_t N, int64_t Hi, int64_t Wi, int64_t Cin,
                             int64_t in_ld, int64_t Ho, int64_t Wo, int64_t Cout, int64_t out_ld, int64_t R, int64_t S,
                             int64_t stride_y, int64_t stride_x, int64_t off_y0, int64_t off_x0, int64_t off_dy,
                             int64_t off_dx, const diga_bwd_epilogue_t* epi, int prof_tag, void* stream);
int diga_conv2d_nhwc_bf16x3_epi(const float* in, const uint16_t* wgt_hi, const uint16_t* wgt_lo, float* out, int64_t N,
                                int64_t Hi, int64_t Wi, int64_t Cin, int64_t in_ld, int64_t Ho, int64_t Wo, int64_t Cout,
                                int64_t out_ld, int64_t R, int64_t S, int64_t stride_y, int64_t stride_x, int64_t off_y0,
                                int64_t off_x0, int64_t off_dy, int64_t off_dx, const diga_bwd_epilogue_t* epi, int prof_tag,
                                void* stream);
int diga_conv2d_nhwc_twin_epi(const void* in_twin, const void* wgt_img, float* out, int64_t N, int64_t Hi, int64_t Wi,
                              int64_t Cin, int64_t Ho, int64_t Wo, int64_t Cout, int64_t out_ld, int64_t R, int64_t S,
                              int64_t stride_y, int64_t stride_x, int64_t off_y0, int64_t off_x0, int64_t off_dy,
                              int64_t off_dx, const diga_bwd_epilogue_t* epi, int prof_tag, void* stream);

typedef struct diga_conv_options {
    int reflect_pad;
    int upsample_shift;
    int activation;
} diga_conv_options_t;

#define DIGA_CONV_MATH_F32 0
#define DIGA_CONV_MATH_BF16X3 1
#define DIGA_CONV_MATH_BF16X6 2

int diga_split_bf16(const float* x, uint16_t* hi, uint16_t* lo, int64_t n, void* stream);
int diga_conv2d_nhwc_bf16x3(const float* in, const uint16_t* wgt_hi, const uint16_t* wgt_lo, const float* bias, float* out,
                            int64_t N, int64_t Hi, int64_t Wi, int64_t Cin, int64_t in_ld,
                            int64_t Ho, int64_t Wo, int64_t Cout, int64_t out_ld, int64_t R, int64_t S,
                            int64_t stride_y, int64_t stride_x, int64_t off_y0, int64_t off_x0,
                            int64_t off_dy, int64_t off_dx, float* stats_partial, int prof_tag, void* stream);

int diga_make_twin(const float* x, int64_t ld, void* twin, int64_t M, int64_t C, void* stream);
size_t diga_split_bf16_image_bytes(int64_t Cout, int64_t RS, int64_t Cin);
int diga_split_bf16_image(const float* w, void* img, int64_t Cout, int64_t RS, int64_t Cin, void* stream);
int diga_conv2d_nhwc_twin(const void* in_twin, const void* wgt_img, const float* bias, float* out, int64_t N, int64_t Hi,
                          int64_t Wi, int64_t Cin, int64_t Ho, int64_t Wo, int64_t Cout, int64_t out_ld, int64_t R, int64_t S,
                          int64_t stride_y, int64_t stride_x, int64_t off_y0, int64_t off_x0, int64_t off_dy, int64_t off_dx,
                          float* stats_partial, int prof_tag, void* stream);

size_t diga_conv2d_winograd_workspace_bytes(int64_t N, int64_t H, int64_t W, int64_t Cin, int64_t Cout, int64_t dilation, int64_t tile);
size_t diga_conv2d_winograd_tile_table_bytes(int64_t N, int64_t H, int64_t W, int64_t dilation, int64_t tile);
int diga_conv2d_winograd_tile_table(void* table, int64_t N, int64_t H, int64_t W, int64_t dilation, int64_t tile, void* stream);
size_t diga_conv2d_winograd_stats_records(int64_t N, int64_t H, int64_t W, int64_t Cout, int64_t dilation, int64_t tile);
size_t diga_conv2d_winograd_stats_floats(int64_t N, int64_t H, int64_t W, int64_t Cout, int64_t dilation, int64_t tile);
int diga_conv2d_winograd_f32(const float* in, const float* wgt, const float* bias, float* out, void* workspace,
                             size_t workspace_bytes, int64_t N, int64_t H, int64_t W, int64_t Cin, int64_t in_ld, int64_t Cout,
                             int64_t out_ld, int64_t dilation, int64_t tile, int flip, float* stats_partial, const void* tile_table,
                             int prof_tag, void* stream);
int diga_conv2d_winograd_f32_opts(const float* in, const float* wgt, const float* bias, float* out, void* workspace,
                                  size_t workspace_bytes, int64_t N, int64_t H, int64_t W, int64_t Cin, int64_t in_ld, int64_t Cout,
                                  int64_t out_ld, int64_t dilation, int64_t tile, const diga_conv_options_t* opts, const void* tile_table,
                                  int prof_tag, void* stream);
int diga_conv2d_winograd_f32_epi(const float* in, const float* wgt, float* out, void* workspace, size_t workspace_bytes, int64_t N,
                                 int64_t H, int64_t W, int64_t Cin, int64_t in_ld, int64_t Cout, int64_t out_ld, int64_t dilation,
                                 int64_t tile, int flip, const diga_bwd_epilogue_t* epi, const void* tile_table, int prof_tag,
                                 void* stream);
size_t diga_conv2d_wgrad_winograd_workspace_bytes(int64_t N, int64_t H, int64_t W, int64_t Cin, int64_t Cout, int64_t dilation,
                                                  int64_t tile, int v_kept );
int diga_conv2d_wgrad_winograd_f32(const float* dy, const float* x, const float* v_kept, float* dw, void* workspace,
                                   size_t workspace_bytes, int64_t N, int64_t H, int64_t W, int64_t Cin, int64_t x_ld, int64_t Cout,
                                   int64_t dy_ld, int64_t dilation, int64_t tile, const void* tile_table, void* stream);
size_t diga_conv2d_winograd_v_floats(int64_t N, int64_t H, int64_t W, int64_t Cin, int64_t dilation, int64_t tile);
int diga_conv2d_winograd_f32_keep(const float* in, const float* wgt, const float* bias, float* out, float* v_keep, void* workspace,
                                  size_t workspace_bytes, int64_t N, int64_t H, int64_t W, int64_t Cin, int64_t in_ld, int64_t Cout,
                                  int64_t out_ld, int64_t dilation, int64_t tile, float* stats_partial, const void* tile_table, int prof_tag,
                                  void* stream);

int diga_conv2d_nhwc_f32_opts(const float* in, const float* wgt, const float* bias, float* out, int64_t N, int64_t Hi, int64_t Wi,
                              int64_t Cin, int64_t in_ld, int64_t Ho, int64_t Wo, int64_t Cout, int64_t out_ld, int64_t R, int64_t S,
                              int64_t stride_y, int64_t stride_x, int64_t off_y0, int64_t off_x0, int64_t off_dy, int64_t off_dx,
                              const diga_conv_options_t* opts, int prof_tag, void* stream);
int diga_conv2d_nhwc_bf16x3_opts(const float* in, const uint16_t* wgt_hi, const uint16_t* wgt_lo, const float* bias, float* out,
                                 int64_t N, int64_t Hi, int64_t Wi, int64_t Cin, int64_t in_ld, int64_t Ho, int64_t Wo, int64_t Cout,
                                 int64_t out_ld, int64_t R, int64_t S, int64_t stride_y, int64_t stride_x, int64_t off_y0,
                                 int64_t off_x0, int64_t off_dy, int64_t off_dx, const diga_conv_options_t* opts, int prof_tag,
                                 void* stream);
int diga_conv2d_nhwc_twin_opts(const void* in_twin, const void* wgt_img, const float* bias, float* out, int64_t N, int64_t Hi,
                               int64_t Wi, int64_t Cin, int64_t Ho, int64_t Wo, int64_t Cout, int64_t out_ld, int64_t R, int64_t S,
                               int64_t stride_y, int64_t stride_x, int64_t off_y0, int64_t off_x0, int64_t off_dy, int64_t off_dx,
                               const diga_conv_options_t* opts, int prof_tag, void* stream);

size_t diga_conv2d_wgrad_workspace_bytes(int64_t N, int64_t Ho, int64_t Wo, int64_t Cout, int64_t Cin,
                                         int64_t R, int64_t S);
int diga_conv2d_wgrad_nhwc_f32(const float* dy, const float* x, float* dw, void* workspace, size_t workspace_bytes,
                               int64_t N, int64_t Hi, int64_t Wi, int64_t Cin, int64_t x_ld,
                               int64_t Ho, int64_t Wo, int64_t Cout, int64_t dy_ld, int64_t R, int64_t S,
                               int64_t stride_y, int64_t stride_x, int64_t off_y0, int64_t off_x0,
                               int64_t off_dy, int64_t off_dx, int math, void* stream);

size_t diga_conv2d_wgrad_twin_workspace_bytes(int64_t N, int64_t Ho, int64_t Wo, int64_t Cout, int64_t Cin, int64_t R, int64_t S);
int diga_conv2d_wgrad_twin(const void* dy_twin, const void* x_twin, float* dw, void* workspace, size_t workspace_bytes,
                           int64_t N, int64_t Hi, int64_t Wi, int64_t Cin, int64_t Ho, int64_t Wo, int64_t Cout, int64_t R,
                           int64_t S, int64_t stride_y, int64_t stride_x, int64_t off_y0, int64_t off_x0, int64_t off_dy,
                           int64_t off_dx, void* stream);

int diga_make_triplet(const float* x, int64_t ld, void* triplet, int64_t M, int64_t C, void* stream);
size_t diga_split_bf16x6_image_bytes(int64_t Cout, int64_t RS, int64_t Cin);
int diga_split_bf16x6_image(const float* w, void* img, int64_t Cout, int64_t RS, int64_t Cin, void* stream);
int diga_conv2d_nhwc_bf16x6(const void* in_triplet, const void* wgt_img, const float* bias, float* out, int64_t N, int64_t Hi,
                            int64_t Wi, int64_t Cin, int64_t Ho, int64_t Wo, int64_t Cout, int64_t out_ld, int64_t R, int64_t S,
                            int64_t stride_y, int64_t stride_x, int64_t off_y0, int64_t off_x0, int64_t off_dy, int64_t off_dx,
                            float* stats_partial, int prof_tag, void* stream);
int diga_conv2d_nhwc_bf16x6_epi(const void* in_triplet, const void* wgt_img, float* out, int64_t N, int64_t Hi, int64_t Wi,
                                int64_t Cin, int64_t Ho, int64_t Wo, int64_t Cout, int64_t out_ld, int64_t R, int64_t S,
                                int64_t stride_y, int64_t stride_x, int64_t off_y0, int64_t off_x0, int64_t off_dy, int64_t off_dx,
                                const diga_bwd_epilogue_t* epi, int prof_tag, void* stream);
size_t diga_conv2d_wgrad_bf16x6_workspace_bytes(int64_t N, int64_t Ho, int64_t Wo, int64_t Cout, int64_t Cin, int64_t R, int64_t S);
int diga_conv2d_wgrad_bf16x6(const void* dy_triplet, const void* x_triplet, float* dw, void* workspace, size_t workspace_bytes,
                             int64_t N, int64_t Hi, int64_t Wi, int64_t Cin, int64_t Ho, int64_t Wo, int64_t Cout, int64_t R,
                             int64_t S, int64_t stride_y, int64_t stride_x, int64_t off_y0, int64_t off_x0, int64_t off_dy,
                             int64_t off_dx, void* stream);

int diga_im2col_nchw(const float* x, float* out, int64_t N, int64_t C, int64_t H, int64_t W, int64_t R, int64_t S,
                     int64_t stride, int64_t pad, int64_t Ho, int64_t Wo, int64_t Kpad, void* stream);

int diga_weight_transpose(const float* w, float* wt, int64_t K, int64_t RS, int64_t C, void* stream);

size_t diga_norm_workspace_bytes(int64_t rows_per_segment, int64_t n_segments, int64_t C);

int diga_bn_fwd(const float* x, int64_t ld_x, float* y, int64_t ld_y, const float* residual, int64_t ld_r,
                const float* gamma, const float* beta, float* running_mean, float* running_var,
                float* save_mean, float* save_invstd, float* save_ab, int64_t M, int64_t C, int training, int relu,
                int y_twin, unsigned char* relu_bits, float momentum, float eps, void* workspace, size_t workspace_bytes,
                void* stream);

int diga_bn_fwd_partials(const float* x, int64_t ld_x, float* y, int64_t ld_y, const float* residual, int64_t ld_r,
                         const float* gamma, const float* beta, float* running_mean, float* running_var,
                         float* save_mean, float* save_invstd, float* save_ab, int64_t M, int64_t C, int relu,
                         int y_twin, unsigned char* relu_bits, float momentum, float eps, const float* partial,
                         int64_t chunk_rows, void* workspace, size_t workspace_bytes, void* stream);

int diga_bn_fwd_records(const float* x, int64_t ld_x, float* y, int64_t ld_y, const float* residual, int64_t ld_r,
                        const float* gamma, const float* beta, float* running_mean, float* running_var,
                        float* save_mean, float* save_invstd, float* save_ab, int64_t M, int64_t C, int relu,
                        int y_twin, unsigned char* relu_bits, float momentum, float eps, const float* partial,
                        const float* counts, int64_t n_records, void* workspace, size_t workspace_bytes, void* stream);

int diga_bn_bwd(const float* dy, int64_t ld_dy, const float* x, int64_t ld_x, const float* y, int64_t ld_y,
                const float* relu_ab, const float* gamma, const float* save_mean, const float* save_invstd, float* dx,
                int64_t ld_dx, float* dres, int64_t ld_dr, int64_t M, int64_t C, int training, int dx_twin, void* workspace,
                size_t workspace_bytes, void* stream);

int diga_bn_bwd_affine(const float* dy, int64_t ld_dy, const float* x, int64_t ld_x, const float* y, int64_t ld_y,
                       const float* relu_ab, const float* gamma, const float* save_mean, const float* save_invstd, float* dx,
                       int64_t ld_dx, float* dgamma, float* dbeta, int64_t M, int64_t C, int training, void* workspace,
                       size_t workspace_bytes, void* stream);

int diga_bn_bwd_partials(const float* g, int64_t ld_g, const float* x, int64_t ld_x, const float* gamma,
                         const float* save_mean, const float* save_invstd, float* dx, int64_t ld_dx, int64_t M, int64_t C,
                         int dx_twin, const float* partial, int64_t chunk_rows, void* workspace, size_t workspace_bytes,
                         void* stream);

int diga_gn_fwd(const float* x, int64_t ld_x, float* y, int64_t ld_y, const float* gamma, const float* beta,
                const float* chan_scale, float* save_mean, float* save_invstd, int64_t N, int64_t HW, int64_t C,
                int64_t G, int relu, float eps, void* workspace, size_t workspace_bytes, void* stream);
int diga_gn_bwd(const float* dy, int64_t ld_dy, const float* x, int64_t ld_x, const float* y, int64_t ld_y,
                const float* gamma, const float* chan_scale, const float* save_mean, const float* save_invstd,
                float* dx, int64_t ld_dx, float* dgamma, float* dbeta, int64_t N, int64_t HW, int64_t C, int64_t G,
                void* workspace, size_t workspace_bytes, void* stream);

int diga_avgpool_nhwc(const float* x, int64_t ld_x, float* out, int64_t N, int64_t HW, int64_t C, void* workspace,
                      size_t workspace_bytes, void* stream);
int diga_channel_affine(const float* x, int64_t ld_x, float* y, int64_t ld_y, const float* a, const float* b,
                        int64_t N, int64_t HW, int64_t C, void* stream);
int diga_small_linear_fwd(const float* x, const float* w, const float* b, float* y, int64_t N, int64_t K, int64_t O, int act, void* stream);
int diga_small_linear_bwd(const float* x, const float* w, const float* y, const float* dy, float* dz, float* dx, float* dw, float* db,
                          int64_t N, int64_t K, int64_t O, int act, void* stream);
int diga_colsum_nhwc(const float* x, int64_t ld_x, float* out, int64_t M, int64_t C, void* workspace, size_t workspace_bytes,
                     void* stream);
int diga_channel_dot(const float* dy, int64_t ld_dy, const float* x, int64_t ld_x, float* out, int64_t N, int64_t HW,
                     int64_t C, void* workspace, size_t workspace_bytes, void* stream);

int diga_pyramid_sum_fwd(float* dst, int64_t H, int64_t W, const float* bias, const float* s0, int64_t h0, int64_t w0,
                         const float* s1, int64_t h1, int64_t w1, const float* s2, int64_t h2, int64_t w2, int64_t N, int64_t C,
                         void* stream);
int diga_pyramid_sum_bwd(const float* dout, int64_t H, int64_t W, float* ds, int64_t h, int64_t w, int64_t N, int64_t C, void* stream);
int diga_pyramid_sum_fwd3(float* dst, int64_t H, int64_t W, const float* bias, const float* s2, const float* s4, const float* s8,
                          float* stats, int64_t N, int64_t C, void* stream);
int diga_pyramid_sum_bwd3(const float* dout, int64_t H, int64_t W, float* ds2, float* ds4, float* ds8, int64_t N, int64_t C, void* stream);

int diga_maxpool3x3s2_fwd(const float* x, float* y, uint8_t* idx, int64_t N, int64_t H, int64_t W, int64_t C,
                          int64_t Ho, int64_t Wo, void* stream);
int diga_maxpool3x3s2_bwd(const float* dy, const uint8_t* idx, float* dx, int64_t N, int64_t H, int64_t W, int64_t C,
                          int64_t Ho, int64_t Wo, void* stream);

int diga_color_aug_view(const float* x, float* out, const float* params, const int32_t* order_host, int64_t B, int64_t H,
                        int64_t W, float beta, const float* mean_host, const float* std_host, void* stream);

enum {
    DIGA_PROF_CE2D = 0,
    DIGA_PROF_DISTILL,
    DIGA_PROF_UPSAMPLE_LOSS,
    DIGA_PROF_EMA,
    DIGA_PROF_SGD,
    DIGA_PROF_CLASSMIX_HIST,
    DIGA_PROF_CLASSMIX_PASTE,
    DIGA_PROF_CENTROID_WEIGHTS,
    DIGA_PROF_CONSENSUS,
    DIGA_PROF_CLASS_MEANS,
    DIGA_PROF_CENTROID_APPLY,
    DIGA_PROF_CONV_FWD,
    DIGA_PROF_CONV_BWD_DATA,
    DIGA_PROF_CONV_BWD_WEIGHT,
    DIGA_PROF_NORM,
    DIGA_PROF_ELEMENTWISE,
    DIGA_PROF_MIT_GEMM,
    DIGA_PROF_MIT_WGRAD,
    DIGA_PROF_MIT_ATTN_FWD,
    DIGA_PROF_MIT_ATTN_BWD,
    DIGA_PROF_MIT_NORM,
    DIGA_PROF_MIT_DWCONV,
    DIGA_PROF_MIT_MISC,
    DIGA_PROF_NTAGS
};
int diga_prof_enable(int on);
int diga_prof_reset(void);
int diga_prof_query(int tag, int64_t* h_count, double* h_total_ms);
int diga_prof_query_work(int tag, double* h_work);

#if defined(__GNUC__)
#pragma GCC visibility pop
#endif
#ifdef __cplusplus
}
#endif
#endif
```

Measured before the change: 19.63 crops/s.

## Fold downsample BatchNorm apply into residual junction and specialize persistent GEMM

The downsample branch's BatchNorm now only computes statistics and coefficients and skips writing its normalized output. The block's final bn3 then applies those coefficients to the raw residual inside its affine+residual+ReLU kernel, which removes one full read/write pass over the downsample activation. Separately, the persistent GEMM kernel is templated on stats and bias so those branches disappear at compile time, and it skips MMA work for padded row pieces beyond rows_valid. The backward path has to handle a deferred-apply BN, which adds complexity and some correctness risk.

```diff
diff --git a/diga_amd/_lib.py b/diga_amd/_lib.py
--- a/diga_amd/_lib.py
+++ b/diga_amd/_lib.py
@@ -77,6 +77,7 @@
     "diga_norm_workspace_bytes": (SZ, [I64, I64, I64]),
     "diga_bn_fwd": (INT, [P, I64, P, I64, P, I64, P, P, P, P, P, P, P, I64, I64, INT, INT, INT, P, F32, F32, P, SZ, P]),
     "diga_bn_fwd_partials": (INT, [P, I64, P, I64, P, I64, P, P, P, P, P, P, P, I64, I64, INT, INT, P, F32, F32, P, I64, P, SZ, P]),
+    "diga_bn_fwd_partials_resab": (INT, [P, I64, P, I64, P, I64, P, P, P, P, P, P, P, I64, I64, P, F32, F32, P, I64, P, SZ, P]),
     "diga_bn_fwd_records": (INT, [P, I64, P, I64, P, I64, P, P, P, P, P, P, P, I64, I64, INT, INT, P, F32, F32, P, P, I64, P, SZ, P]),
     "diga_bn_bwd": (INT, [P, I64, P, I64, P, I64, P, P, P, P, P, I64, P, I64, I64, I64, INT, INT, P, SZ, P]),
     "diga_bn_bwd_affine": (INT, [P, I64, P, I64, P, I64, P, P, P, P, P, I64, P, P, I64, I64, INT, P, SZ, P]),
diff --git a/diga_amd/config.py b/diga_amd/config.py
--- a/diga_amd/config.py
+++ b/diga_amd/config.py
@@ -39,6 +39,7 @@
     relu_bits: bool = True
     fuse_bwd: bool = True
     junction_chain: bool = True
+    fold_downsample_bn: bool = True
     ddp_bucket_mb: int = 25
     ddp_grad_views: bool = True
     ddp_overlap: bool = True
@@ -74,6 +75,7 @@
         c.relu_bits = _flag("DIGA_RELU_BITS", c.relu_bits)
         c.fuse_bwd = _flag("DIGA_FUSE_BWD", c.fuse_bwd)
         c.junction_chain = _flag("DIGA_JUNCTION_CHAIN", c.junction_chain)
+        c.fold_downsample_bn = _flag("DIGA_FOLD_DOWNSAMPLE_BN", c.fold_downsample_bn)
         c.ddp_bucket_mb = int(e("DIGA_DDP_BUCKET_MB", c.ddp_bucket_mb))
         c.ddp_grad_views = _flag("DIGA_DDP_GRAD_VIEWS", c.ddp_grad_views)
         c.ddp_overlap = _flag("DIGA_DDP_OVERLAP", c.ddp_overlap)
diff --git a/diga_amd/csrc/conv.hip b/diga_amd/csrc/conv.hip
--- a/diga_amd/csrc/conv.hip
+++ b/diga_amd/csrc/conv.hip
@@ -2205,12 +2205,14 @@
     const float* W;
     float* out;
     int M, K, Cout, tiles_m, tiles_n, wb_tiles;
+    int rows_valid;
     int64_t wb_stride;
     int64_t a_ld, out_ld;
     const float* bias;
     float* stats;
 };
 
+template <bool STATS, bool BIAS>
 __global__ __launch_bounds__(768, 3) void gemm_f32_persistent_kernel(GemmArgs g) {
     constexpr int A_BYTES = 256 * 128, B_BYTES = 128 * 128, STAGE = A_BYTES + B_BYTES;
     extern __shared__ __align__(16) unsigned char smem_b[];
@@ -2283,6 +2285,14 @@
     }
 
     const int wm = wv >> 1, wn = wv & 1;
+    const int piece_row = __builtin_amdgcn_readfirstlane(wm * 64);
+    auto piece_live = [&](int it_) {
+#ifdef DIGA_GEMM_ALL_PIECES_LIVE
+        return true;
+#endif
+        const int tile_m = (start + slot + nslots * it_) / g.tiles_n;
+        return (g.wb_tiles > 0 ? tile_m % g.wb_tiles : tile_m) * 256 + piece_row < g.rows_valid;
+    };
     f32x16 acc[2][2];
 #pragma unroll
     for (int i = 0; i < 2; ++i)
@@ -2297,8 +2307,17 @@
 #define DIGA_FOFF(t) ((t) << 5)
 
     __builtin_amdgcn_s_barrier();
-    int cur = 0, it = 0, ks_in_tile = 0;
-    for (int gs = 0; gs < total_steps; ++gs) {
+    int cur = 0;
+    for (int it = 0; it < nmine; ++it) {
+        if (!piece_live(it)) {
+            for (int ks = 0; ks < ksteps; ++ks) {
+                asm volatile("s_waitcnt lgkmcnt(0)" ::: "memory");
+                __builtin_amdgcn_s_barrier();
+                cur = cur == 2 ? 0 : cur + 1;
+            }
+        } else {
+        __builtin_amdgcn_s_waitcnt(0xC07F);
+        for (int ks = 0; ks < ksteps; ++ks) {
         const int sa = cur * STAGE + FA, sb = cur * STAGE + FB;
 #define As_AT(t) (smem_b + (sa ^ DIGA_FOFF(t)))
 #define Bs_AT(t) (smem_b + (sb ^ DIGA_FOFF(t)))
@@ -2333,7 +2352,9 @@
         asm volatile("s_waitcnt lgkmcnt(0)" ::: "memory");
         __builtin_amdgcn_s_barrier();
         cur = cur == 2 ? 0 : cur + 1;
-        if (++ks_in_tile == ksteps) {
+        }
+        }
+        {
             const int t = start + slot + nslots * it;
             const int tile_n = t % g.tiles_n, tile_m = t / g.tiles_n;
             const int row_w = tile_m * 256 + wm * 64;
@@ -2343,8 +2364,8 @@
             const int rows_left = g.M - (row_w + 4 * lh);
 #pragma unroll
             for (int j = 0; j < 2; ++j) {
-                const float bv = g.bias != nullptr ? g.bias[col_w + j * 32] : 0.f;
-                const float sh = __shfl(acc[0][j][0] + bv, li, 64);
+                const float bv = BIAS ? g.bias[col_w + j * 32] : 0.f;
+                const float sh = STATS ? __shfl(BIAS ? acc[0][j][0] + bv : acc[0][j][0], li, 64) : 0.f;
                 float sd = 0.f, sd2 = 0.f;
                 if (row_w + 64 <= g.M) {
 #pragma unroll
@@ -2352,30 +2373,34 @@
 #pragma unroll
                         for (int e = 0; e < 16; ++e) {
                             const int r = i * 32 + (e & 3) + 8 * (e >> 2);
-                            const float v = acc[i][j][e] + bv;
+                            const float v = BIAS ? acc[i][j][e] + bv : acc[i][j][e];
                             __builtin_nontemporal_store(v, DIGA_O_AT(r, j));
-                            const float d = v - sh;
-                            sd += d;
-                            sd2 += d * d;
-                            acc[i][j][e] = 0.f;
-                        }
-                } else {
-#pragma unroll
-                    for (int i = 0; i < 2; ++i)
-#pragma unroll
-                        for (int e = 0; e < 16; ++e) {
-                            const int r = i * 32 + (e & 3) + 8 * (e >> 2);
-                            const float v = acc[i][j][e] + bv;
-                            if (r < rows_left) {
-                                __builtin_nontemporal_store(v, DIGA_O_AT(r, j));
+                            if (STATS) {
                                 const float d = v - sh;
                                 sd += d;
                                 sd2 += d * d;
                             }
                             acc[i][j][e] = 0.f;
                         }
+                } else {
+#pragma unroll
+                    for (int i = 0; i < 2; ++i)
+#pragma unroll
+                        for (int e = 0; e < 16; ++e) {
+                            const int r = i * 32 + (e & 3) + 8 * (e >> 2);
+                            const float v = BIAS ? acc[i][j][e] + bv : acc[i][j][e];
+                            if (r < rows_left) {
+                                __builtin_nontemporal_store(v, DIGA_O_AT(r, j));
+                                if (STATS) {
+                                    const float d = v - sh;
+                                    sd += d;
+                                    sd2 += d * d;
+                                }
+                            }
+                            acc[i][j][e] = 0.f;
+                        }
                 }
-                if (g.stats != nullptr && row_w < g.M) {
+                if (STATS && row_w < g.M) {
                     sd += __shfl_xor(sd, 32, 64);
                     sd2 += __shfl_xor(sd2, 32, 64);
                     if (lh == 0) {
@@ -2386,14 +2411,30 @@
                     }
                 }
             }
-            ks_in_tile = 0;
-            ++it;
-        }
-    }
+        }
+    }
+}
+
+static void launch_gemm_persistent(const GemmArgs& g, hipStream_t st) {
+    const size_t sh = 3 * (256 + 128) * 128;
+#define DIGA_GEMM_P(STATS_, BIAS_)                                                                                                    \
+    do {                                                                                                                              \
+        (void)hipFuncSetAttribute((const void*)gemm_f32_persistent_kernel<STATS_, BIAS_>, hipFuncAttributeMaxDynamicSharedMemorySize, \
+                                  (int)sh);                                                                                           \
+        hipLaunchKernelGGL((gemm_f32_persistent_kernel<STATS_, BIAS_>), dim3(256), dim3(768), sh, st, g);                              \
+    } while (0)
+    if (g.stats != nullptr) {
+        if (g.bias != nullptr) DIGA_GEMM_P(true, true);
+        else DIGA_GEMM_P(true, false);
+    } else {
+        if (g.bias != nullptr) DIGA_GEMM_P(false, true);
+        else DIGA_GEMM_P(false, false);
+    }
+#undef DIGA_GEMM_P
 }
 
 int gemm_batched_f32_dma(const float* A, int64_t rows_per_batch, int batches, int64_t K, const float* W, int64_t Cout,
-                         float* out, hipStream_t st) {
+                         float* out, hipStream_t st, int64_t rows_valid) {
     DIGA_REQUIRE(rows_per_batch > 0 && rows_per_batch % 256 == 0 && K % 32 == 0 && Cout > 0 && Cout % 4 == 0, DIGA_EINVAL,
                  "gemm_batched_f32_dma: rows %% 256, K %% 32, Cout %% 4 required");
     const int64_t M = rows_per_batch * batches;
@@ -2417,8 +2458,8 @@
         g.A = A; g.W = W; g.out = out; g.M = (int)M; g.K = (int)K; g.Cout = (int)Cout;
         g.tiles_m = (int)(M / 256); g.tiles_n = a.tiles_n; g.wb_tiles = a.wb_tiles; g.wb_stride = a.wb_stride;
         g.a_ld = K; g.out_ld = Cout; g.bias = nullptr; g.stats = nullptr;
-        (void)hipFuncSetAttribute((const void*)gemm_f32_persistent_kernel, hipFuncAttributeMaxDynamicSharedMemorySize, (int)sh);
-        hipLaunchKernelGGL(gemm_f32_persistent_kernel, dim3(256), dim3(768), sh, st, g);
+        g.rows_valid = (int)(rows_valid > 0 && rows_valid < rows_per_batch ? rows_valid : rows_per_batch);
+        launch_gemm_persistent(g, st);
         return DIGA_OK;
     }
     (void)hipFuncSetAttribute((const void*)conv_fwd_dma_kernel<false>, hipFuncAttributeMaxDynamicSharedMemorySize, (int)sh);
@@ -2482,10 +2523,8 @@
         GemmArgs g;
         g.A = in; g.W = wgt; g.out = out; g.M = a.M; g.K = (int)Cin; g.Cout = (int)Cout;
         g.tiles_m = (int)ceil_div(a.M, 256); g.tiles_n = (int)(Cout / 128); g.wb_tiles = 0; g.wb_stride = 0;
-        g.a_ld = in_ld; g.out_ld = out_ld; g.bias = bias; g.stats = stats_partial;
-        const size_t shp = 3 * (256 + 128) * 128;
-        (void)hipFuncSetAttribute((const void*)gemm_f32_persistent_kernel, hipFuncAttributeMaxDynamicSharedMemorySize, (int)shp);
-        hipLaunchKernelGGL(gemm_f32_persistent_kernel, dim3(256), dim3(768), shp, st, g);
+        g.a_ld = in_ld; g.out_ld = out_ld; g.bias = bias; g.stats = stats_partial; g.rows_valid = a.M;
+        launch_gemm_persistent(g, st);
         return launch_status("diga_conv2d_nhwc_f32");
     }
     if (a.M >= 256 && Cout >= 256 && R * S * Cin >= 256) {
diff --git a/diga_amd/csrc/norm.hip b/diga_amd/csrc/norm.hip
--- a/diga_amd/csrc/norm.hip
+++ b/diga_amd/csrc/norm.hip
@@ -174,12 +174,13 @@
     lo.y = __builtin_bit_cast(uint32_t, __builtin_convertvector((f2){v.z - h2, v.w - h3}, bf2));
 }
 
-template <bool RES, bool RELU, bool BITS, bool TWIN, bool SEG>
+template <bool RES, bool RELU, bool BITS, bool TWIN, bool SEG, bool RESAB = false>
 __global__ __launch_bounds__(256) void affine_apply_kernel(const float* __restrict__ x, int64_t ld_x, float* __restrict__ y,
                                                            int64_t ld_y, const float* __restrict__ res, int64_t ld_r,
                                                            const float* __restrict__ a, const float* __restrict__ b,
                                                            int64_t ab_seg_stride, int64_t rows_per_seg, int64_t rows,
-                                                           int C, unsigned char* __restrict__ relu_bits) {
+                                                           int C, unsigned char* __restrict__ relu_bits,
+                                                           const float* __restrict__ res_ab = nullptr) {
     const int tq = C >> 2;
     const int tpr = tq < 256 ? tq : 256;
     const int rpb = 256 / tpr;
@@ -191,6 +192,11 @@
         const int c = q * 4;
         float4 av = *reinterpret_cast<const float4*>(a + c);
         float4 bv = b != nullptr ? *reinterpret_cast<const float4*>(b + c) : make_float4(0.f, 0.f, 0.f, 0.f);
+        float4 rav, rbv;
+        if (RESAB) {
+            rav = *reinterpret_cast<const float4*>(res_ab + c);
+            rbv = *reinterpret_cast<const float4*>(res_ab + C + c);
+        }
         int cur_seg = 0;
         for (int r = blockIdx.x * rpb + rl; r < nrows; r += rstep) {
             if (SEG) {
@@ -206,7 +212,11 @@
             o.x = __builtin_fmaf(xv.x, av.x, bv.x); o.y = __builtin_fmaf(xv.y, av.y, bv.y);
             o.z = __builtin_fmaf(xv.z, av.z, bv.z); o.w = __builtin_fmaf(xv.w, av.w, bv.w);
             if (RES) {
-                const float4 rv = ld4s(res + (int64_t)r * ld_r + c);
+                float4 rv = ld4s(res + (int64_t)r * ld_r + c);
+                if (RESAB) {
+                    rv.x = __builtin_fmaf(rv.x, rav.x, rbv.x); rv.y = __builtin_fmaf(rv.y, rav.y, rbv.y);
+                    rv.z = __builtin_fmaf(rv.z, rav.z, rbv.z); rv.w = __builtin_fmaf(rv.w, rav.w, rbv.w);
+                }
                 o.x += rv.x; o.y += rv.y; o.z += rv.z; o.w += rv.w;
             }
             if (RELU) {
@@ -263,6 +273,17 @@
         } else { if (twin_out) DIGA_AFF(false, false, false, true); else DIGA_AFF(false, false, false, false); }
     }
 #undef DIGA_AFF
+}
+
+static void launch_affine_resab(dim3 grid, hipStream_t st, const float* x, int64_t ld_x, float* y, int64_t ld_y, const float* res,
+                                int64_t ld_r, const float* res_ab, const float* a, const float* b, int64_t rows, int C,
+                                unsigned char* relu_bits) {
+    if (relu_bits != nullptr)
+        hipLaunchKernelGGL((affine_apply_kernel<true, true, true, false, false, true>), grid, dim3(256), 0, st, x, ld_x, y, ld_y, res, ld_r,
+                           a, b, (int64_t)0, rows, rows, C, relu_bits, res_ab);
+    else
+        hipLaunchKernelGGL((affine_apply_kernel<true, true, false, false, false, true>), grid, dim3(256), 0, st, x, ld_x, y, ld_y, res, ld_r,
+                           a, b, (int64_t)0, rows, rows, C, relu_bits, res_ab);
 }
 
 __global__ __launch_bounds__(kNormThreads) void bwd_partial_kernel(const float* __restrict__ dy, int64_t ld_dy,
@@ -966,8 +987,10 @@
                                 float* running_var, float* save_mean, float* save_invstd, float* save_ab, int64_t M,
                                 int64_t C, int relu, int y_twin, unsigned char* relu_bits, float momentum, float eps,
                                 const float* partial, int64_t chunk_rows, const float* counts, int64_t n_records,
-                                void* workspace, size_t workspace_bytes, void* stream) {
+                                void* workspace, size_t workspace_bytes, void* stream, const float* res_ab = nullptr) {
     DIGA_REQUIRE(!relu_bits || (relu && C % 32 == 0), DIGA_EINVAL, "%s: relu_bits needs relu and C %% 32 == 0", who);
+    DIGA_REQUIRE(!res_ab || (residual && y && relu && !y_twin && aligned16(res_ab)), DIGA_EINVAL,
+                 "%s: residual coefficients need a residual, an fp32 y and relu", who);
     DIGA_REQUIRE(x && gamma && beta && save_mean && save_invstd && partial && workspace && M > 0, DIGA_EINVAL, "%s: bad argument", who);
     DIGA_REQUIRE(counts ? (n_records > 0 && n_records < (1 << 30)) : chunk_rows > 0, DIGA_EINVAL, "%s: bad chunk_rows / record count", who);
     DIGA_REQUIRE(y || (save_ab && !y_twin), DIGA_EINVAL, "%s: y = null (statistics and coefficients only) needs save_ab", who);
@@ -998,7 +1021,9 @@
     }
     hipLaunchKernelGGL(bn_finalize2_kernel, dim3((unsigned)ceil_div(C, kFinCh)), dim3(256), 0, st, partial, g, gamma, beta,
                        running_mean, running_var, save_mean, save_invstd, ab, momentum, eps, counts);
-    if (y != nullptr)
+    if (y != nullptr && res_ab != nullptr)
+        launch_affine_resab(dim3(ew_blocks(M * C / 4)), st, x, ld_x, y, ld_y, residual, ld_r, res_ab, ab, ab + C, M, (int)C, relu_bits);
+    else if (y != nullptr)
         launch_affine(dim3(ew_blocks(M * C / 4)), st, x, ld_x, y, ld_y, residual, ld_r, ab,
                            ab + C, (int64_t)0, M, M, (int)C, relu, y_twin, relu_bits);
     return launch_status(who);
@@ -1013,6 +1038,18 @@
     return bn_fwd_from_partials("diga_bn_fwd_partials", x, ld_x, y, ld_y, residual, ld_r, gamma, beta, running_mean, running_var, save_mean,
                                 save_invstd, save_ab, M, C, relu, y_twin, relu_bits, momentum, eps, partial, chunk_rows, nullptr, 0,
                                 workspace, workspace_bytes, stream);
+}
+
+extern "C" int diga_bn_fwd_partials_resab(const float* x, int64_t ld_x, float* y, int64_t ld_y, const float* residual,
+                                          int64_t ld_r, const float* residual_ab, const float* gamma, const float* beta,
+                                          float* running_mean, float* running_var, float* save_mean, float* save_invstd,
+                                          int64_t M, int64_t C, unsigned char* relu_bits, float momentum, float eps,
+                                          const float* partial, int64_t chunk_rows, void* workspace, size_t workspace_bytes,
+                                          void* stream) {
+    DIGA_REQUIRE(residual_ab != nullptr, DIGA_EINVAL, "diga_bn_fwd_partials_resab: null residual coefficients");
+    return bn_fwd_from_partials("diga_bn_fwd_partials_resab", x, ld_x, y, ld_y, residual, ld_r, gamma, beta, running_mean, running_var,
+                                save_mean, save_invstd, nullptr, M, C, 1, 0, relu_bits, momentum, eps, partial, chunk_rows, nullptr, 0,
+                                workspace, workspace_bytes, stream, residual_ab);
 }
 
 extern "C" int diga_bn_fwd_records(const float* x, int64_t ld_x, float* y, int64_t ld_y, const float* residual,
diff --git a/diga_amd/csrc/winograd.hip b/diga_amd/csrc/winograd.hip
--- a/diga_amd/csrc/winograd.hip
+++ b/diga_amd/csrc/winograd.hip
@@ -3,7 +3,7 @@
 namespace diga {
 
 int gemm_batched_f32_dma(const float* A, int64_t rows_per_batch, int batches, int64_t K, const float* W, int64_t Cout,
-                         float* out, hipStream_t st);
+                         float* out, hipStream_t st, int64_t rows_valid);
 size_t wgrad_batched_slab_bytes(int64_t rows, int batches, int64_t Cout, int64_t Cin);
 int wgrad_batched_f32_dma(const float* Z, const float* V, float* dU, float* slab, int64_t rows, int batches, int64_t Cout,
                           int64_t Cin, hipStream_t st);
@@ -980,7 +980,7 @@
         hipLaunchKernelGGL(wino_weight_kernel, dim3((unsigned)ceil_div(Cout * (Cin / 4), 256)), dim3(256), 0, st, wgt, U, (int)Cout, (int)Cin,
                            flip);
     launch_input(tile, in, in_ld, tab, V, g.Tp, Cin, H, W, dilation, st, reflect);
-    int rc = gemm_batched_f32_dma(V, g.Tp, P, Cin, U, Cout, Mb, st);
+    int rc = gemm_batched_f32_dma(V, g.Tp, P, Cin, U, Cout, Mb, st, g.T);
     if (rc) return rc;
     if (epi == nullptr && stats != nullptr) {
         if (tile == 6) launch_output_stats_m<6>(Mb, tab, bias, out, out_ld, g, Cout, stats, st);
diff --git a/diga_amd/model/norm.py b/diga_amd/model/norm.py
--- a/diga_amd/model/norm.py
+++ b/diga_amd/model/norm.py
@@ -42,16 +42,23 @@
 
     @staticmethod
     def forward(ctx, x, residual, weight, bias, running_mean, running_var, training, relu, momentum, eps,
-                partials=None, twin_out=False, dx_twin=False, box=None, res_box=None):
+                partials=None, twin_out=False, dx_twin=False, box=None, res_box=None, res_ab=None, defer_apply=None):
         _lib.require_gpu(x)
         xn = nhwc(x.detach())
         n, h, w, c = xn.shape
         m = n * h * w
         rn = None if residual is None else nhwc(residual.detach())
-        y = torch.empty_like(xn)
+        plain_partials = partials is not None and training and not isinstance(partials[1], tuple)
+        if (defer_apply is not None or res_ab is not None) and not plain_partials:
+            raise RuntimeError("DigaBatchNorm2d: the folded downsample BatchNorm needs train-mode statistics from the producing conv")
+        if defer_apply is not None and (relu or residual is not None or twin_out or box is not None):
+            raise RuntimeError("DigaBatchNorm2d: defer_apply is the form of a BatchNorm without ReLU and residual")
+        if res_ab is not None and not (relu and residual is not None and not twin_out):
+            raise RuntimeError("DigaBatchNorm2d: residual coefficients need relu and a residual")
+        y = None if defer_apply is not None else torch.empty_like(xn)
         save_mean = torch.empty(c, dtype=torch.float32, device=xn.device)
         save_invstd = torch.empty_like(save_mean)
-        save_ab = torch.empty(2 * c, dtype=torch.float32, device=xn.device) if (relu and residual is None) else None
+        save_ab = torch.empty(2 * c, dtype=torch.float32, device=xn.device) if ((relu and residual is None) or defer_apply is not None) else None
         ws = _ws(m, 1, c, xn.device)
         bits = None
         if (box is not None and relu and residual is not None and c % 32 == 0 and _relu_bits_enabled()):
@@ -64,6 +71,11 @@
                       _lib.ptr(save_invstd), _lib.ptr(save_ab), m, c, 1 if relu else 0, 1 if twin_out else 0,
                       _lib.ptr(bits), float(momentum), float(eps), _lib.ptr(partials[0]),
                       _lib.C.c_void_p(partials[0].data_ptr() + recs * 3 * c * 4), recs, _lib.ptr(wsr), wsr.numel(), _lib.stream())
+        elif res_ab is not None:
+            _lib.call("diga_bn_fwd_partials_resab", _lib.ptr(xn), c, _lib.ptr(y), c, _lib.ptr(rn), c, _lib.ptr(res_ab), _lib.ptr(weight),
+                      _lib.ptr(bias), _lib.ptr(running_mean), _lib.ptr(running_var), _lib.ptr(save_mean), _lib.ptr(save_invstd), m, c,
+                      _lib.ptr(bits), float(momentum), float(eps), _lib.ptr(partials[0]), int(partials[1]), _lib.ptr(ws), ws.numel(),
+                      _lib.stream())
         elif partials is not None and training:
             _lib.call("diga_bn_fwd_partials", _lib.ptr(xn), c, _lib.ptr(y), c, _lib.ptr(rn), c, _lib.ptr(weight),
                       _lib.ptr(bias), _lib.ptr(running_mean), _lib.ptr(running_var), _lib.ptr(save_mean),
@@ -77,6 +89,13 @@
                       _lib.ptr(save_ab), m, c, 1 if training else 0, 1 if relu else 0, 1 if twin_out else 0,
                       _lib.ptr(bits),
                       float(momentum), float(eps), _lib.ptr(ws), ws.numel(), _lib.stream())
+        if defer_apply is not None:
+            ctx.save_for_backward(xn, None, weight, save_mean, save_invstd, None)
+            ctx.flags = (training, False)
+            ctx.dx_twin = False
+            ctx.box, ctx.res_box = None, None
+            defer_apply["ab"] = save_ab
+            return xn.permute(0, 3, 1, 2)
         ctx.save_for_backward(xn, y if (relu and save_ab is None) else None, weight, save_mean, save_invstd, save_ab)
         ctx.flags = (training, residual is not None)
         ctx.dx_twin = bool(dx_twin and c % 8 == 0)
@@ -104,7 +123,7 @@
                       _lib.ptr(save_mean), _lib.ptr(save_invstd), _lib.ptr(dx), c, _lib.ptr(dgamma), _lib.ptr(dbeta), m, c,
                       1 if training else 0, _lib.ptr(ws), ws.numel(), _lib.stream())
             return (dx.permute(0, 3, 1, 2), None, dgamma if ctx.needs_input_grad[2] else None, dbeta if ctx.needs_input_grad[3] else None,
-                    None, None, None, None, None, None, None, None, None, None, None)
+                    None, None, None, None, None, None, None, None, None, None, None, None, None)
         pre = ctx.box.pop("premasked", None) if ctx.box is not None else None
         if pre is not None and pre[0] == g.data_ptr() and pre[2]._version == pre[4] and ld_g == c and training:
             ws = _lib.workspace(67 * c * 4, xn.device, "norm_kk")
@@ -122,12 +141,12 @@
             ctx.res_box["dres"] = dres
             dres = None
         return (dx.permute(0, 3, 1, 2), None if dres is None else dres.permute(0, 3, 1, 2),
-                dgamma, dbeta, None, None, None, None, None, None, None, None, None, None, None)
+                dgamma, dbeta, None, None, None, None, None, None, None, None, None, None, None, None, None)
 
 
 class DigaBatchNorm2d(nn.BatchNorm2d):
 
-    def forward(self, x, residual=None, relu=False, twin_out=False, dx_twin=False):
+    def forward(self, x, residual=None, relu=False, twin_out=False, dx_twin=False, defer_apply=False):
         if self.weight.requires_grad or self.bias.requires_grad:
             raise RuntimeError("DigaBatchNorm2d implements the frozen-affine BN of the DiGA path; "
                                "set requires_grad=False on weight and bias")
@@ -145,8 +164,13 @@
                 if rb is not None and rb.get("consumer_ready") and "res_claimed" not in rb:
                     rb["res_claimed"] = True
                     res_box = rb
+        res_ab = getattr(residual, "_diga_res_ab", None) if residual is not None else None
+        holder = {} if defer_apply else None
         y = _BnFn.apply(x, residual, self.weight, self.bias, self.running_mean, self.running_var, training, relu,
-                        self.momentum, self.eps, getattr(x, "_diga_bn_partials", None), twin_out, bool(dx_twin), box, res_box)
+                        self.momentum, self.eps, getattr(x, "_diga_bn_partials", None), twin_out, bool(dx_twin), box, res_box,
+                        res_ab, holder)
+        if holder is not None:
+            y._diga_res_ab = holder["ab"]
         if twin_out:
             y._diga_is_twin = True
         if box is not None:
@@ -196,6 +220,10 @@
     return config.active().relu_bits
 
 
+def fold_downsample_bn_enabled():
+    return config.active().fold_downsample_bn
+
+
 def fuse_backward_enabled():
     return config.active().fuse_bwd
 
diff --git a/diga_amd/model/seg_model_noaux.py b/diga_amd/model/seg_model_noaux.py
--- a/diga_amd/model/seg_model_noaux.py
+++ b/diga_amd/model/seg_model_noaux.py
@@ -71,6 +71,12 @@
         y = self.bn2(self.conv2(y, twin_grad=tw2 and grad), relu=True, twin_out=tw3, dx_twin=tw2 and grad)
         if self.downsample is None:
             skip = x
+        elif (dn.fold_downsample_bn_enabled() and len(self.downsample) == 2 and self.training and self.bn3.training
+              and self.downsample[1].training and self.conv3.training and self.downsample[0].training
+              and self.conv3.emit_bn_stats and self.downsample[0].emit_bn_stats and self.conv3.out_channels % 4 == 0
+              and not self.downsample._forward_hooks and not self.downsample[1]._forward_hooks):
+            skip = self.downsample[0](x, chain=chain) if chain is not None else self.downsample[0](x)
+            skip = self.downsample[1](skip, defer_apply=True)
         elif chain is not None:
             skip = self.downsample[1](self.downsample[0](x, chain=chain))
         else:
diff --git a/include/diga_hip.h b/include/diga_hip.h
--- a/include/diga_hip.h
+++ b/include/diga_hip.h
@@ -267,6 +267,12 @@
                          float* save_mean, float* save_invstd, float* save_ab, int64_t M, int64_t C, int relu,
                          int y_twin, unsigned char* relu_bits, float momentum, float eps, const float* partial,
                          int64_t chunk_rows, void* workspace, size_t workspace_bytes, void* stream);
+
+int diga_bn_fwd_partials_resab(const float* x, int64_t ld_x, float* y, int64_t ld_y, const float* residual, int64_t ld_r,
+                               const float* residual_ab, const float* gamma, const float* beta, float* running_mean,
+                               float* running_var, float* save_mean, float* save_invstd, int64_t M, int64_t C,
+                               unsigned char* relu_bits, float momentum, float eps, const float* partial, int64_t chunk_rows,
+                               void* workspace, size_t workspace_bytes, void* stream);
 
 int diga_bn_fwd_records(const float* x, int64_t ld_x, float* y, int64_t ld_y, const float* residual, int64_t ld_r,
                         const float* gamma, const float* beta, float* running_mean, float* running_var,
```

Result: faster. 19.84 crops/s (median of 6 runs) (+1.1%).
